# ChuhanZhou/News_Recommendation_Model

Hardware: AMD Instinct MI355X
Metric: train impressions/sec (higher is better)
Workload: dtype f32

## Files before the change

### include/nrm_hotpath.h

```cpp
#ifndef NRM_HOTPATH_H
#define NRM_HOTPATH_H

#ifdef __cplusplus
extern "C" {
#endif

#define NRM_ABI_VERSION 7
#define NRM_OK 0
#define NRM_EINVAL (-1)
#define NRM_ELAUNCH (-2)

typedef void* nrm_stream_t;

int nrm_abi_version(void);
const char* nrm_last_error(void);
int nrm_build_flags(void);
const char* nrm_source_digest(void);
const char* nrm_build_info(void);


#define NRM_MMA_F32 0
#define NRM_MMA_BF16 1
#define NRM_MMA_BF16X3 2
long nrm_pwattn_packed_floats(int D);
int nrm_pwattn_pack_wp(const float* fc1_weight, int ld, int D, int mma, float* packed, nrm_stream_t stream);
int nrm_pwattn_fwd(const float* t, const float* h, const float* u, const float* v, const float* packed_wp,
                   const float* w2, const float* b2, float* z, float* s,
                   int B, int T, int H, int D, int mma, nrm_stream_t stream);

#define NRM_DZ_F32 0
#define NRM_DZ_HL4 1
int nrm_pwattn_bwd_dz(float* z_inout, const float* ds, const float* w2, float* dw2, float* db2, float* du, float* dv,
                      int B, int T, int H, int D, int dz_format, nrm_stream_t stream);
int nrm_pwattn_bwd_nsplit(int B, int T, int H, int D, int mma);
int nrm_pwattn_bwd_contract(const float* dz, const float* t, const float* h, const float* wp, int ldwp,
                            float* dt, float* dh, float* ws,
                            int B, int T, int H, int D, int passes, int mma, int dz_format, nrm_stream_t stream);
int nrm_pwattn_bwd_rw_supported(int D, int mma);
long nrm_pwattn_bwd_rw_packed_floats(int D, int mma);
int nrm_pwattn_bwd_rw_pack(const float* fc1_weight, int ld, int D, int mma, float* packed, nrm_stream_t stream);
int nrm_pwattn_bwd_rw_dtdh(const float* dz_hl4, const float* t, const float* h, const float* packed, float* dt, float* dh,
                           int B, int T, int H, int D, int mma, nrm_stream_t stream);

int nrm_pwattn_bwd_dp_supported(int D, int H);
long nrm_pwattn_bwd_dp_packed_floats(int D, int H);
int nrm_pwattn_bwd_dp_pack(const float* fc1_weight, int ld, int D, int H, float* packed, nrm_stream_t stream);
int nrm_pwattn_bwd_dp_dtdh(const float* dz, const float* t, const float* h, const float* packed, float* dt, float* dh,
                           int B, int T, int H, int D, nrm_stream_t stream);

#define NRM_EPI_BIAS 0
#define NRM_EPI_GELU 1
#define NRM_EPI_DGELU 2
#define NRM_EPI_MUL 3
long nrm_gemm_packed_floats(int nrows, int ncols, int mma);
int nrm_gemm_nt_bf16_supported(int M, int K, int mma);
int nrm_gemm_pack(const float* src, long row_stride, long col_stride, int nrows, int ncols, float* packed,
                  nrm_stream_t stream);
typedef struct {
    const float* src; const float* src2; float sign2;
    long row_stride, col_stride; int nrows, ncols;
    float* packed;
    int mma;
} nrm_pack_desc;
int nrm_gemm_pack_multi(const nrm_pack_desc* descs, int n, nrm_stream_t stream);
int nrm_gemm_nt(const float* x, int ldx, int M, const float* packed, int N, int K, const float* bias,
                float* y, int ldy, float* z, int ldz, const float* m, int ldm, int epilogue, int mma, nrm_stream_t stream);
int nrm_gemm_tn_nsplit(int ncols_i, int ncols_j, int R, int mma);
int nrm_gemm_tn(const float* A, int lda, int ncols_i, const float* B, int ldb, int ncols_j, int R,
                float* ws, int ldws, float* colsum, float* zero_out, long zero_n, int mma, nrm_stream_t stream);

int nrm_slab_reduce(const float* ws, int nsplit, int nj, int ldws, int ni, float* out, long out_istride, long out_jstride,
                    float* out2, long out2_istride, long out2_jstride, float sign2,
                    const float* vec, float* vec_out, nrm_stream_t stream);
typedef struct nrm_slab_desc {
    const float* ws; int nsplit, nj, ldws, ni;
    float* out; long out_istride, out_jstride;
    float* out2; long out2_istride, out2_jstride; float sign2;
    const float* vec; float* vec_out;
} nrm_slab_desc;
int nrm_slab_reduce_multi(const nrm_slab_desc* descs, int n, nrm_stream_t stream);

int nrm_colreduce(int mode, const float* x, const float* dy, const float* mean, const float* rstd,
                  float* s0, float* s1, int R, int N, int ld, nrm_stream_t stream);
int nrm_bn_finalize(int stage, const float* s, float* out, float* running, int R, int N, float momentum, float eps,
                    nrm_stream_t stream);
int nrm_mul_bwd(const float* dy, int lddy, const float* g, int ldg, const float* e, int lde, float* dg, float* de, int ldo,
                int R, int N, nrm_stream_t stream);
int nrm_bn_apply(const float* x, const float* mean, const float* rstd, const float* gamma, const float* beta,
                 float* y, int R, int N, int ld, nrm_stream_t stream);
int nrm_bn_backward(const float* x, const float* dy, const float* mean, const float* rstd, const float* gamma,
                    const float* s0, const float* s1, const float* add, float* dx, int R, int N, int ld, int training,
                    nrm_stream_t stream);
int nrm_concat_cols(const float* const* srcs, const long* lds, const int* widths, int n, float* out, int ldo, long R,
                    nrm_stream_t stream);

int nrm_pool_bmm(const float* W, long wsb, long wsi, long wsj, const float* X, int ldx, float* out,
                 int B, int I, int J, int D, int accumulate, nrm_stream_t stream);
int nrm_pool_rowdot(const float* g, int ldg, const float* h, float* ds, int B, int T, int H, int D, float* zero_out, int zero_n,
                    nrm_stream_t stream);

int nrm_small_linear_relu_fwd(const void* x, int x_is_f64, const float* weight, const float* bias, float* y, long R, int K, int N, int ldy,
                              nrm_stream_t stream);
int nrm_small_linear_relu_bwd(const void* x, int x_is_f64, const float* weight, const float* bias, const float* dy, int lddy, long R,
                              int K, int N, float* dwb, nrm_stream_t stream);

int nrm_loss_fwd_bwd(const float* out, int out_stride, const void* label, int label_is_f64, const long* user_id, const float* delta,
                     long n_delta, float alpha, int B, int T, float* loss_sum, float* dout, int dout_stride, float* ddelta, int* err,
                     nrm_stream_t stream);

int nrm_adam_step(float* p, float* g, float* m, float* v, long n, float lr, float beta1, float beta2, float eps,
                  float weight_decay, int step, int zero_grad, nrm_stream_t stream);
int nrm_gather_flat(const float* const* srcs, const long* offsets, const long* counts, int n, float* flat, long flat_n,
                    nrm_stream_t stream);
int nrm_adam_step_dev(float* p, float* g, float* m, float* v, long n, float lr, float beta1, float beta2, float eps,
                      float weight_decay, float* state, int zero_grad, nrm_stream_t stream);

int nrm_frontend_fwd(const void* x, int x_is_f64, int nrows, int xcols, int P, int n_sub, int behaviour,
                     const float* cat_tab, int n_cat, int e0, const float* sen_w, const float* sen_b, int e1,
                     const float* type_tab, int n_type, int e2,
                     const float* year_tab, const float* month_tab, const float* day_tab, const float* hour_tab,
                     int n_year, int n_month, int n_day, int n_hour, int e3,
                     float* lab, int ldlab, float* ti, int ldti, int* err, nrm_stream_t stream);
int nrm_frontend_bwd(const void* x, int x_is_f64, int nrows, int xcols, int P, int n_sub, int behaviour,
                     const float* dlab, int lddl, const float* sen_w, const float* sen_b,
                     int n_cat, int e0, int e1, int n_type, int e2, int n_year, int n_month, int n_day, int n_hour, int e3,
                     float* d_cat_tab, float* d_sen_w, float* d_sen_b, float* d_type_tab,
                     float* d_year_tab, float* d_month_tab, float* d_day_tab, float* d_hour_tab, nrm_stream_t stream);

long nrm_frontend_cat_ws_ints(int n_cat, long nrows_total, int n_sub);
int nrm_frontend_cat_grad(const void* x0, int nrows0, int xcols0, const float* dlab0, int lddl0,
                          const void* x1, int nrows1, int xcols1, const float* dlab1, int lddl1, int x_is_f64,
                          int P, int n_sub, int n_cat, int e0, float* d_cat_tab, int* ws, nrm_stream_t stream);

int nrm_row_auc(const float* score, const float* label, const int* len, int B, int T, float* auc, int* top1,
                nrm_stream_t stream);

int nrm_ensemble_rank_max_candidates(void);
int nrm_ensemble_rank(const float* const* logits, const long* row_stride, const long* col_stride, int M, const int* empty,
                      const float* label, int B, int T, float* score, int* rank, int* live, float* metrics, nrm_stream_t stream);

int nrm_compact_gather(const void* x_target, int target_cols, int target_is_f64, const void* x_global, int global_cols, int global_is_f64,
                       const int* cand_off, const int* pad_mult, int B, int T, int trim, int N,
                       void* xt_compact, void* xg_compact, int* flag, nrm_stream_t stream);
int nrm_pwattn_fwd_ragged(const float* t, const float* h, const float* u, const float* v, const float* packed_wp,
                          const float* w2, const float* b2, float* s, const int* cand_imp, const int* cand_off,
                          int B, int N, int max_count, int H, int D, int mma, nrm_stream_t stream);
int nrm_pool_bmm_ragged(const float* s, const float* h, float* out, const int* cand_off, int B, int N, int max_count, int H, int D,
                        nrm_stream_t stream);
int nrm_ensemble_rank_ragged(const float* const* logits, const long* col_stride, int M, const int* cand_off, const int* pad_mult, int N,
                             const float* label, int B, int T, float* score, int* rank, int* live, float* metrics, nrm_stream_t stream);

#ifdef __cplusplus
}
#endif
#endif
```

### news_recommendation_model_amd/csrc/capi.hip

```cpp
#include <stdarg.h>
#include <stdint.h>
#include <stdio.h>
#include <stdlib.h>
#include <vector>

#include "../../include/nrm_hotpath.h"
#include "pwattn.hpp"
#include "gemm.hpp"
#include "head.hpp"
#include "pool_loss.hpp"
#include "frontend.hpp"
#include "scoring.hpp"
#include "compact.hpp"

static thread_local char g_err[512] = "";

static int fail(int code, const char* fmt, ...) {
    va_list ap;
    va_start(ap, fmt);
    vsnprintf(g_err, sizeof(g_err), fmt, ap);
    va_end(ap);
    return code;
}
static int check_hip(hipError_t e, const char* what) {
// ... 211 lines not shown
        if (int rc = check_hip(nrm::bwd_e_launch(p, pl, false, mma, (hipStream_t)stream), "bwd_e pass 2")) return rc;
    }
    return NRM_OK;
}


static bool al16(const void* p) { return ((uintptr_t)p & 15) == 0; }

long nrm_gemm_packed_floats(int nrows, int ncols, int mma) {
    if (nrows <= 0 || ncols <= 0) return 0;
    if (mma == NRM_MMA_BF16 || mma == NRM_MMA_BF16X3)
        return (long)((nrows + 15) / 16) * ((ncols + 31) / 32) * (mma == NRM_MMA_BF16X3 ? 2 : 1) * 256 + 1024;
    const nrm::GemmNtPlan pl = nrm::gemm_nt_plan(nrows);
    return (long)((ncols + 15) / 16) * pl.rows * 16 + 1024;
}

int nrm_gemm_nt_bf16_supported(int M, int K, int mma) { return nrm::gemm_nt_rx_bm(M, K, mma) ? 1 : 0; }

int nrm_gemm_pack(const float* src, long row_stride, long col_stride, int nrows, int ncols, float* packed,
                  nrm_stream_t stream) {
    if (!src || !packed || nrows <= 0 || ncols <= 0) return fail(NRM_EINVAL, "nrm_gemm_pack: bad argument");
    const nrm::GemmNtPlan pl = nrm::gemm_nt_plan(nrows);
    return check_hip(nrm::pack_rows_launch(src, row_stride, col_stride, nrows, ncols, pl.rows, (ncols + 15) / 16, packed,
                                           (hipStream_t)stream), "pack_rows");
}

int nrm_gemm_pack_multi(const nrm_pack_desc* descs, int n, nrm_stream_t stream) {
    if (n < 0 || (n > 0 && !descs)) return fail(NRM_EINVAL, "nrm_gemm_pack_multi: bad argument");
    for (int lo = 0; lo < n; lo += nrm::PACK_MAX) {
        const int m = n - lo < nrm::PACK_MAX ? n - lo : nrm::PACK_MAX;
        nrm::PackTable tab = {};
        long mx = 0;
        for (int i = 0; i < m; ++i) {
            const nrm_pack_desc& d = descs[lo + i];
            if (!d.src || !d.packed || d.nrows <= 0 || d.ncols <= 0) return fail(NRM_EINVAL, "nrm_gemm_pack_multi: entry %d is malformed", lo + i);
            const nrm::GemmNtPlan pl = nrm::gemm_nt_plan(d.nrows);
            nrm::PackEntry& e = tab.e[i];
            e.src = d.src; e.src2 = d.src2; e.dst = d.packed; e.rs = d.row_stride; e.cs = d.col_stride;
            e.nrows = d.nrows; e.ncols = d.ncols; e.rows = pl.rows; e.kchunks = (d.ncols + 15) / 16; e.sign2 = d.sign2; e.fmt = 0;
            if (d.mma == NRM_MMA_BF16 || d.mma == NRM_MMA_BF16X3) {
                e.fmt = d.mma == NRM_MMA_BF16X3 ? 2 : 1; e.rows = (d.nrows + 15) / 16 * 16; e.kchunks = (d.ncols + 31) / 32;
            } else if (d.mma != NRM_MMA_F32) return fail(NRM_EINVAL, "nrm_gemm_pack_multi: entry %d: mma=%d", lo + i, d.mma);
            const long total = e.fmt ? (long)(e.rows / 16) * e.kchunks * 512 : (long)e.kchunks * e.rows * 16;
            if (total > mx) mx = total;
        }
        if (int rc = check_hip(nrm::pack_rows_multi_launch(tab, m, mx, (hipStream_t)stream), "pack_rows_multi")) return rc;
    }
    return NRM_OK;
}

int nrm_gemm_nt(const float* x, int ldx, int M, const float* packed, int N, int K, const float* bias,
                float* y, int ldy, float* z, int ldz, const float* m, int ldm, int epilogue, int mma, nrm_stream_t stream) {
    if (!x || !packed || !y) return fail(NRM_EINVAL, "nrm_gemm_nt: null pointer");
    if (M < 0 || N <= 0 || K <= 0) return fail(NRM_EINVAL, "nrm_gemm_nt: M=%d N=%d K=%d", M, N, K);
    if (ldx % 4 || ldy % 4 || ldx < K || ldy < N || !al16(x) || !al16(y))
        return fail(NRM_EINVAL, "nrm_gemm_nt: ldx=%d ldy=%d must be multiples of 4 covering K=%d / N=%d, rows 16-B aligned", ldx, ldy, K, N);
    if (epilogue != NRM_EPI_BIAS && (!z || ldz % 4 || ldz < N || !al16(z)))
        return fail(NRM_EINVAL, "nrm_gemm_nt: epilogue %d needs z with ldz %% 4 == 0, ldz >= N", epilogue);
    if (epilogue < 0 || epilogue > 3) return fail(NRM_EINVAL, "nrm_gemm_nt: epilogue=%d", epilogue);
    if (epilogue == NRM_EPI_MUL && (!m || ldm % 4 || ldm < N || !al16(m)))
        return fail(NRM_EINVAL, "nrm_gemm_nt: NRM_EPI_MUL needs m with ldm %% 4 == 0, ldm >= N");
    if ((long)256 * (ldx > ldy ? ldx : ldy) * 4 >= (1L << 31)) return fail(NRM_EINVAL, "nrm_gemm_nt: leading dimension too large");
    if (int rc = check_mma("nrm_gemm_nt", mma)) return rc;
    if (mma != NRM_MMA_F32) {
        if (!nrm::gemm_nt_rx_bm(M > 0 ? M : 1, K, mma)) return fail(NRM_EINVAL, "nrm_gemm_nt: K=%d is too wide for the bf16 form (nrm_gemm_nt_bf16_supported)", K);
        nrm::GemmRxParams r = {};
        r.x = x; r.ldx = ldx; r.xcols = ldx; r.wq = packed; r.wq_bytes = (unsigned)(nrm_gemm_packed_floats(N, K, mma) * 4);
        r.bias = bias; r.N = N; r.y = y; r.ldy = ldy;
        r.z = epilogue == NRM_EPI_BIAS ? nullptr : z; r.ldz = epilogue == NRM_EPI_BIAS ? 4 : ldz;
        r.m = epilogue == NRM_EPI_MUL ? m : nullptr; r.ldm = epilogue == NRM_EPI_MUL ? ldm : 4;
        r.M = M; r.K = K; r.k32 = (K + 31) / 32; r.nt16 = (N + 15) / 16;
        return check_hip(nrm::gemm_nt_rx_launch(r, epilogue, mma, (hipStream_t)stream), "gemm_nt_rx");
    }
    const nrm::GemmNtPlan pl = nrm::gemm_nt_plan(N);
    nrm::GemmNtParams p;
    p.x = x; p.ldx = ldx; p.xcols = ldx; p.wp = packed; p.wp_bytes = (unsigned)(nrm_gemm_packed_floats(N, K, NRM_MMA_F32) * 4);
    p.rows = pl.rows; p.bias = bias; p.N = N; p.y = y; p.ldy = ldy;
    p.z = epilogue == NRM_EPI_BIAS ? nullptr : z; p.ldz = epilogue == NRM_EPI_BIAS ? 4 : ldz;
    p.m = epilogue == NRM_EPI_MUL ? m : nullptr; p.ldm = epilogue == NRM_EPI_MUL ? ldm : 4;
    p.M = M; p.K = K; p.kchunks = (K + 15) / 16;
    return check_hip(nrm::gemm_nt_launch(p, pl, epilogue, (hipStream_t)stream), "gemm_nt");
}

static const int kTnWavesBf16 = 1024;
static int tn_waves(int mma = 0) {
    if (const char* e = getenv("NRM_TN_WAVES")) return atoi(e);
    return mma ? kTnWavesBf16 : kTnWaves;
}

int nrm_gemm_tn_nsplit(int ncols_i, int ncols_j, int R, int mma) {
    if (ncols_i <= 0 || ncols_j <= 0 || R <= 0) return 0;
    return nrm::gemm_tn_plan(ncols_i, ncols_j, R, tn_waves(mma), mma).nsplit;
}

int nrm_gemm_tn(const float* A, int lda, int ncols_i, const float* B, int ldb, int ncols_j, int R,
                float* ws, int ldws, float* colsum, float* zero_out, long zero_n, int mma, nrm_stream_t stream) {
    if (!A || !B || !ws) return fail(NRM_EINVAL, "nrm_gemm_tn: null pointer");
    if (ncols_i <= 0 || ncols_j <= 0 || R <= 0 || lda < ncols_i || ldb < ncols_j)
        return fail(NRM_EINVAL, "nrm_gemm_tn: ncols_i=%d ncols_j=%d R=%d lda=%d ldb=%d", ncols_i, ncols_j, R, lda, ldb);
    if (ldws % 4 || ldws < ncols_i || !al16(ws)) return fail(NRM_EINVAL, "nrm_gemm_tn: ldws=%d", ldws);
    if (int rc = check_mma("nrm_gemm_tn", mma)) return rc;
    const nrm::GemmTnPlan pl = nrm::gemm_tn_plan(ncols_i, ncols_j, R, tn_waves(mma), mma);
    if ((long)pl.rps * (lda > ldb ? lda : ldb) * 4 >= (1L << 31)) return fail(NRM_EINVAL, "nrm_gemm_tn: split too large");
    if (mma != NRM_MMA_F32 && (lda % 4 || ldb % 4 || ((uintptr_t)A & 15) || ((uintptr_t)B & 15)))
        return fail(NRM_EINVAL, "nrm_gemm_tn: the bf16 forms read 16-byte row segments (lda, ldb multiples of 4, 16-byte aligned rows)");
    nrm::GemmTnParams p = {};
    p.A = A; p.lda = lda; p.acols = lda; p.B = B; p.ldb = ldb; p.bcols = ldb;
    if (zero_out && (zero_n < 0 || !al16(zero_out))) return fail(NRM_EINVAL, "nrm_gemm_tn: zero_out must be 16-byte aligned, zero_n >= 0");
    p.ws = ws; p.ldws = ldws; p.colsum = colsum; p.R = R; p.ncols_j = ncols_j;
    p.zero_out = zero_out; p.zero_n = zero_out ? zero_n : 0;
    if (mma != NRM_MMA_F32) return check_hip(nrm::gemm_tn_bf16_launch(p, pl, mma, (hipStream_t)stream), "gemm_tn_bf16");
    return check_hip(nrm::gemm_tn_launch(p, pl, (hipStream_t)stream), "gemm_tn");
}

int nrm_slab_reduce(const float* ws, int nsplit, int nj, int ldws, int ni, float* out, long out_istride, long out_jstride,
                    float* out2, long out2_istride, long out2_jstride, float sign2,
                    const float* vec, float* vec_out, nrm_stream_t stream) {
    if (!ws || !out) return fail(NRM_EINVAL, "nrm_slab_reduce: null pointer");
    if (nsplit <= 0 || nj <= 0 || ni <= 0 || ldws < ni) return fail(NRM_EINVAL, "nrm_slab_reduce: nsplit=%d nj=%d ni=%d ldws=%d", nsplit, nj, ni, ldws);
    if ((vec == nullptr) != (vec_out == nullptr)) return fail(NRM_EINVAL, "nrm_slab_reduce: vec and vec_out go together");
    nrm::SlabReduceParams p;
    p.ws = ws; p.nsplit = nsplit; p.nj = nj; p.ldws = ldws; p.ni = ni; p.out = out; p.ors = out_istride; p.ocs = out_jstride;
    p.out2 = out2; p.ors2 = out2_istride; p.ocs2 = out2_jstride; p.sign2 = sign2; p.vec = vec; p.vec_out = vec_out;
    return check_hip(nrm::slab_reduce_launch(p, (hipStream_t)stream), "slab_reduce");
}

int nrm_slab_reduce_multi(const nrm_slab_desc* descs, int n, nrm_stream_t stream) {
    if (n < 0 || (n > 0 && !descs)) return fail(NRM_EINVAL, "nrm_slab_reduce_multi: bad argument");
    if (n == 0) return NRM_OK;
    std::vector<nrm::SlabReduceParams> ps((size_t)n);
    for (int i = 0; i < n; ++i) {
        const nrm_slab_desc& d = descs[i];
        if (!d.ws || !d.out) return fail(NRM_EINVAL, "nrm_slab_reduce_multi: entry %d: null pointer", i);
        if (d.nsplit <= 0 || d.nj <= 0 || d.ni <= 0 || d.ldws < d.ni)
            return fail(NRM_EINVAL, "nrm_slab_reduce_multi: entry %d: nsplit=%d nj=%d ni=%d ldws=%d", i, d.nsplit, d.nj, d.ni, d.ldws);
        if ((d.vec == nullptr) != (d.vec_out == nullptr)) return fail(NRM_EINVAL, "nrm_slab_reduce_multi: entry %d: vec and vec_out go together", i);
        nrm::SlabReduceParams& p = ps[(size_t)i];
        p.ws = d.ws; p.nsplit = d.nsplit; p.nj = d.nj; p.ldws = d.ldws; p.ni = d.ni; p.out = d.out; p.ors = d.out_istride; p.ocs = d.out_jstride;
        p.out2 = d.out2; p.ors2 = d.out2_istride; p.ocs2 = d.out2_jstride; p.sign2 = d.sign2; p.vec = d.vec; p.vec_out = d.vec_out;
    }
    return check_hip(nrm::slab_reduce_multi_launch(ps.data(), n, (hipStream_t)stream), "slab_reduce_multi");
}

static int check_bn(const char* fn, int R, int N, int ld) {
    if (R < 0 || N <= 0 || N % 4 || ld % 4 || ld < N) return fail(NRM_EINVAL, "%s: R=%d N=%d ld=%d (N, ld multiples of 4)", fn, R, N, ld);
    return NRM_OK;
}

int nrm_colreduce(int mode, const float* x, const float* dy, const float* mean, const float* rstd,
                  float* s0, float* s1, int R, int N, int ld, nrm_stream_t stream) {
    if (int rc = check_bn("nrm_colreduce", R, N, ld)) return rc;
    if (!x || !s0 || (mode >= 1 && !mean) || (mode == 2 && (!dy || !rstd || !s1)) || mode < 0 || mode > 2)
        return fail(NRM_EINVAL, "nrm_colreduce: bad argument for mode %d", mode);
    return check_hip(nrm::colred_launch(mode, x, dy, mean, rstd, s0, s1, R, N, ld, (hipStream_t)stream), "colreduce");
}

int nrm_bn_finalize(int stage, const float* s, float* out, float* running, int R, int N, float momentum, float eps,
                    nrm_stream_t stream) {
    if (!s || !out) return fail(NRM_EINVAL, "nrm_bn_finalize: null pointer");
    if ((stage != 0 && stage != 1) || R <= 0 || N <= 0) return fail(NRM_EINVAL, "nrm_bn_finalize: stage=%d R=%d N=%d", stage, R, N);
    return check_hip(nrm::bn_finalize_launch(stage, s, out, running, R, N, momentum, eps, (hipStream_t)stream), "bn_finalize");
}

int nrm_mul_bwd(const float* dy, int lddy, const float* g, int ldg, const float* e, int lde, float* dg, float* de, int ldo,
                int R, int N, nrm_stream_t stream) {
    if (!dy || !g || !e || !dg || !de) return fail(NRM_EINVAL, "nrm_mul_bwd: null pointer");
    if (R < 0 || N <= 0 || N % 4 || lddy % 4 || ldg % 4 || lde % 4 || ldo % 4 || lddy < N || ldg < N || lde < N || ldo < N ||
        !al16(dy) || !al16(g) || !al16(e) || !al16(dg) || !al16(de))
        return fail(NRM_EINVAL, "nrm_mul_bwd: R=%d N=%d (N and leading dimensions multiples of 4, 16-byte aligned rows)", R, N);
    return check_hip(nrm::mul_bwd_launch(dy, g, e, dg, de, R, N, lddy, ldg, lde, ldo, (hipStream_t)stream), "mul_bwd");
}

int nrm_bn_apply(const float* x, const float* mean, const float* rstd, const float* gamma, const float* beta,
                 float* y, int R, int N, int ld, nrm_stream_t stream) {
    if (int rc = check_bn("nrm_bn_apply", R, N, ld)) return rc;
    if (!x || !mean || !rstd || !gamma || !beta || !y) return fail(NRM_EINVAL, "nrm_bn_apply: null pointer");
    return check_hip(nrm::bn_apply_launch(x, mean, rstd, gamma, beta, y, R, N, ld, (hipStream_t)stream), "bn_apply");
}

int nrm_bn_backward(const float* x, const float* dy, const float* mean, const float* rstd, const float* gamma,
                    const float* s0, const float* s1, const float* add, float* dx, int R, int N, int ld, int training,
                    nrm_stream_t stream) {
    if (int rc = check_bn("nrm_bn_backward", R, N, ld)) return rc;
    if (!dy || !rstd || !gamma || !dx || (training && (!x || !mean || !s0 || !s1)))
        return fail(NRM_EINVAL, "nrm_bn_backward: null pointer");
    return check_hip(nrm::bn_bwd_launch(x, dy, mean, rstd, gamma, s0, s1, add, dx, R, N, ld, training, (hipStream_t)stream), "bn_backward");
}


int nrm_concat_cols(const float* const* srcs, const long* lds, const int* widths, int n, float* out, int ldo, long R,
                    nrm_stream_t stream) {
    if (!srcs || !lds || !widths || !out) return fail(NRM_EINVAL, "nrm_concat_cols: null pointer");
    if (n < 1 || n > nrm::CONCAT_MAX || R < 0) return fail(NRM_EINVAL, "nrm_concat_cols: n=%d (1..%d) R=%ld", n, nrm::CONCAT_MAX, R);
    nrm::ConcatTable tab = {};
    int total = 0;
    for (int i = 0; i < n; ++i) {
        if (!srcs[i] || widths[i] <= 0 || lds[i] < widths[i]) return fail(NRM_EINVAL, "nrm_concat_cols: part %d (width %d, ld %ld)", i, widths[i], lds[i]);
        tab.src[i] = srcs[i]; tab.ld[i] = lds[i]; tab.start[i] = total;
        total += widths[i];
    }
    tab.n = n;
    if (ldo < total) return fail(NRM_EINVAL, "nrm_concat_cols: ldo=%d < %d columns", ldo, total);
    return check_hip(nrm::concat_cols_launch(tab, out, R, ldo, total, (hipStream_t)stream), "concat_cols");
}

int nrm_pool_bmm(const float* W, long wsb, long wsi, long wsj, const float* X, int ldx, float* out,
                 int B, int I, int J, int D, int accumulate, nrm_stream_t stream) {
    if (!W || !X || !out) return fail(NRM_EINVAL, "nrm_pool_bmm: null pointer");
    if (B < 0 || I <= 0 || J <= 0 || D <= 0 || D % 4 || B > 65535) return fail(NRM_EINVAL, "nrm_pool_bmm: B=%d I=%d J=%d D=%d", B, I, J, D);
    if (ldx < D || ldx % 4 || !al16(X) || (long)J * ldx * 4 >= (1L << 31))
        return fail(NRM_EINVAL, "nrm_pool_bmm: ldx=%d (>= D, a multiple of 4, X 16-byte aligned, J*ldx*4 < 2^31)", ldx);
    return check_hip(nrm::bmm_rows_launch(W, wsb, wsi, wsj, X, (long)J * ldx, ldx, out, (long)I * D, D, B, I, J, D, accumulate,
                                          (hipStream_t)stream), "pool_bmm");
}

int nrm_pool_bmm_ragged(const float* s, const float* h, float* out, const int* cand_off, int B, int N, int max_count, int H, int D,
                        nrm_stream_t stream) {
    if (!s || !h || !out || !cand_off) return fail(NRM_EINVAL, "nrm_pool_bmm_ragged: null pointer");
    if (B < 0 || N < 0 || max_count < 0 || max_count > N || H <= 0 || D <= 0 || D % 4 || B > 65535)
        return fail(NRM_EINVAL, "nrm_pool_bmm_ragged: B=%d N=%d max_count=%d H=%d D=%d", B, N, max_count, H, D);
    if (!al16(h) || !al16(out) || (long)H * D * 4 >= (1L << 31) || (long)N * H >= (1L << 31))
        return fail(NRM_EINVAL, "nrm_pool_bmm_ragged: h and out must be 16-byte aligned, H*D*4 and N*H below 2^31");
    return check_hip(nrm::bmm_rows_ragged_launch(s, H, h, (long)H * D, D, out, D, cand_off, B, N, max_count, H, D, (hipStream_t)stream), "pool_bmm_ragged");
}

int nrm_pool_rowdot(const float* g, int ldg, const float* h, float* ds, int B, int T, int H, int D, float* zero_out, int zero_n,
                    nrm_stream_t stream) {
    if (!g || !h || !ds) return fail(NRM_EINVAL, "nrm_pool_rowdot: null pointer");
    if (B < 0 || T <= 0 || H <= 0 || D <= 0 || D % 4 || D > 1024 || B > 65535) return fail(NRM_EINVAL, "nrm_pool_rowdot: B=%d T=%d H=%d D=%d", B, T, H, D);
    if (ldg < D || ldg % 4 || !al16(g) || (long)T * ldg * 4 >= (1L << 31))
        return fail(NRM_EINVAL, "nrm_pool_rowdot: ldg=%d (>= D, a multiple of 4, g 16-byte aligned, T*ldg*4 < 2^31)", ldg);
    if (zero_n < 0 || (zero_n > 0 && !zero_out)) return fail(NRM_EINVAL, "nrm_pool_rowdot: zero_n=%d without zero_out", zero_n);
    return check_hip(nrm::rowdot_launch(g, (long)T * ldg, ldg, h, (long)H * D, D, ds, B, T, H, D, zero_out, zero_n, (hipStream_t)stream), "pool_rowdot");
}

int nrm_small_linear_relu_fwd(const void* x, int x_is_f64, const float* weight, const float* bias, float* y, long R, int K, int N, int ldy,
                              nrm_stream_t stream) {
    if (!x || !weight || !y) return fail(NRM_EINVAL, "nrm_small_linear_relu_fwd: null pointer");
    if (R < 0 || K < 1 || K > 4 || N < 1 || N > 8 || ldy < N) return fail(NRM_EINVAL, "nrm_small_linear_relu_fwd: R=%ld K=%d N=%d ldy=%d (K <= 4, N <= 8)", R, K, N, ldy);
    return check_hip(nrm::small_linear_relu_fwd_launch(x, x_is_f64, weight, bias, y, R, K, N, ldy, (hipStream_t)stream), "small_linear_relu_fwd");
}

int nrm_small_linear_relu_bwd(const void* x, int x_is_f64, const float* weight, const float* bias, const float* dy, int lddy, long R,
                              int K, int N, float* dwb, nrm_stream_t stream) {
    if (!x || !weight || !dy || !dwb) return fail(NRM_EINVAL, "nrm_small_linear_relu_bwd: null pointer");
    if (R < 0 || K < 1 || K > 4 || N < 1 || N > 8 || lddy < N) return fail(NRM_EINVAL, "nrm_small_linear_relu_bwd: R=%ld K=%d N=%d lddy=%d (K <= 4, N <= 8)", R, K, N, lddy);
    return check_hip(nrm::small_linear_relu_bwd_launch(x, x_is_f64, weight, bias, dy, lddy, R, K, N, dwb, (hipStream_t)stream), "small_linear_relu_bwd");
}

int nrm_loss_fwd_bwd(const float* out, int out_stride, const void* label, int label_is_f64, const long* user_id, const float* delta,
                     long n_delta, float alpha, int B, int T, float* loss_sum, float* dout, int dout_stride, float* ddelta, int* err,
                     nrm_stream_t stream) {
    if (!out || !label || !user_id || !delta || !loss_sum || !dout || !ddelta || !err) return fail(NRM_EINVAL, "nrm_loss_fwd_bwd: null pointer");
    if (B < 0 || T <= 0 || n_delta < 1 || (long)B * T >= (1L << 29))
        return fail(NRM_EINVAL, "nrm_loss_fwd_bwd: B=%d T=%d n_delta=%ld (T >= 1, n_delta >= 1, B*T < 2^29)", B, T, n_delta);
    if (out_stride < 1 || dout_stride < 1 || (dout_stride == 4 && !al16(dout)))
        return fail(NRM_EINVAL, "nrm_loss_fwd_bwd: out_stride=%d dout_stride=%d (>= 1; dout 16-byte aligned for stride 4)", out_stride, dout_stride);
    return check_hip(nrm::loss_launch(out, out_stride, label, label_is_f64, user_id, delta, n_delta, alpha, B, T, loss_sum, dout, dout_stride,
                                      ddelta, err, (hipStream_t)stream), "loss");
}

int nrm_adam_step(float* p, float* g, float* m, float* v, long n, float lr, float beta1, float beta2, float eps,
                  float weight_decay, int step, int zero_grad, nrm_stream_t stream) {
    if (!p || !g || !m || !v) return fail(NRM_EINVAL, "nrm_adam_step: null pointer");
    if (n < 0 || n % 4 || step < 1 || !al16(p) || !al16(g) || !al16(m) || !al16(v))
        return fail(NRM_EINVAL, "nrm_adam_step: n=%ld step=%d (n %% 4 == 0, step >= 1, 16-byte aligned buffers)", n, step);
    return check_hip(nrm::adam_launch(p, g, m, v, n, lr, beta1, beta2, eps, weight_decay, step, zero_grad, (hipStream_t)stream), "adam");
}

// ... 154 lines not shown
```

### news_recommendation_model_amd/csrc/gemm.hip

```cpp
#include <cstdlib>
#include <type_traits>
#include "common.hpp"
#include "gemm.hpp"
#ifndef NRM_PRIO
#define NRM_PRIO 0
#endif
#ifndef NRM_DIAG_GEMM
#define NRM_DIAG_GEMM 0
#endif

namespace nrm {

__global__ void pack_rows_kernel(const float* __restrict__ src, long rs, long cs, int nrows, int ncols,
                                 int rows, int kchunks, float* __restrict__ packed) {
    const long total = (long)kchunks * rows * 16;
    for (long i = (long)blockIdx.x * blockDim.x + threadIdx.x; i < total; i += (long)gridDim.x * blockDim.x) {
        const int j = (int)(i & 15);
        const long rc = i >> 4;
        const int row = (int)(rc % rows);
        const int c = (int)(rc / rows);
        const int slot = (j >> 2) ^ swz4(row);
        const int col = c * 16 + 4 * slot + (j & 3);
        packed[i] = (row < nrows && col < ncols) ? src[row * rs + col * cs] : 0.0f;
    }
}

__global__ __launch_bounds__(256) void pack_rows_multi_kernel(const PackTable tab) {
    const PackEntry e = tab.e[blockIdx.y];
    if (e.fmt) {
        const int nimg = e.fmt;
        const long total = (long)(e.rows / 16) * e.kchunks * 512;
        __bf16* dst = reinterpret_cast<__bf16*>(e.dst);
        for (long i = (long)blockIdx.x * blockDim.x + threadIdx.x; i < total; i += (long)gridDim.x * blockDim.x) {
            const int j = (int)(i & 31), r16 = (int)((i >> 5) & 15);
            const long tc = i >> 9;
            const int c = (int)(tc % e.kchunks), it = (int)(tc / e.kchunks);
            const int n = 16 * it + r16, k = 32 * c + j;
            float v = 0.0f;
            if (n < e.nrows && k < e.ncols) {
                const long o = n * e.rs + k * e.cs;
                v = e.src[o];
                if (e.src2) v = fmaf(e.sign2, e.src2[o], v);
            }
            const __bf16 hi = (__bf16)v;
            const long o = (tc * nimg) * 512 + r16 * 32 + j;
            dst[o] = hi;
            if (nimg > 1) dst[o + 512] = (__bf16)(v - (float)hi);
        }
        return;
    }
    const long total = (long)e.kchunks * e.rows * 16;
    for (long i = (long)blockIdx.x * blockDim.x + threadIdx.x; i < total; i += (long)gridDim.x * blockDim.x) {
        const int j = (int)(i & 15);
        const long rc = i >> 4;
        const int row = (int)(rc % e.rows);
        const int c = (int)(rc / e.rows);
        const int slot = (j >> 2) ^ swz4(row);
        const int col = c * 16 + 4 * slot + (j & 3);
        float v = 0.0f;
        if (row < e.nrows && col < e.ncols) {
            const long o = row * e.rs + col * e.cs;
            v = e.src[o];
            if (e.src2) v = fmaf(e.sign2, e.src2[o], v);
        }
        e.dst[i] = v;
    }
}

hipError_t pack_rows_multi_launch(const PackTable& tab, int n, long max_total, hipStream_t st) {
    if (n <= 0) return hipSuccess;
    long bx = (max_total + 255) / 256;
    if (bx > 128) bx = 128;
    if (bx < 1) bx = 1;
    hipLaunchKernelGGL(pack_rows_multi_kernel, dim3((unsigned)bx, (unsigned)n), dim3(256), 0, st, tab);
    return hipGetLastError();
}

hipError_t pack_rows_launch(const float* src, long rs, long cs, int nrows, int ncols, int rows, int kchunks,
                            float* packed, hipStream_t st) {
    const long total = (long)kchunks * rows * 16;
    const int blocks = (int)((total + 255) / 256 > 4096 ? 4096 : (total + 255) / 256);
    hipLaunchKernelGGL(pack_rows_kernel, dim3(blocks), dim3(256), 0, st, src, rs, cs, nrows, ncols, rows, kchunks, packed);
    return hipGetLastError();
}

template <int NT, int MT, int EPI, int WPE = 2, int KC = 1>
__global__ __launch_bounds__(256, WPE) void gemm_nt_kernel(const GemmNtParams p) {
#if defined(__HIP_DEVICE_COMPILE__)
    constexpr int BM = 4 * MT * 16;
    constexpr int WROWS = NT * 16;
    constexpr int SUB = (WROWS + BM) * 16;
    constexpr int BUF = KC * SUB;
    __shared__ __attribute__((aligned(16))) float smem[2 * BUF];

    const int tid = threadIdx.x;
    const int lane = tid & 63;
    const int wave = __builtin_amdgcn_readfirstlane(tid >> 6);
    const int r16 = lane & 15, q = lane >> 4;
    const int M = p.M;
    const int m0 = blockIdx.x * BM;
    const int nc = blockIdx.y;
    const int n0 = nc * WROWS;

    constexpr unsigned OOB = 0x80000000u;
    const int rows_here = min(BM, M - m0);
    const __amdgpu_buffer_rsrc_t rs_w = __builtin_amdgcn_make_buffer_rsrc(const_cast<float*>(p.wp), 0, p.wp_bytes, 0x00020000);
    const __amdgpu_buffer_rsrc_t rs_x = __builtin_amdgcn_make_buffer_rsrc(
        const_cast<float*>(p.x) + (size_t)m0 * p.ldx, 0, ((rows_here - 1) * p.ldx + p.xcols) * 4, 0x00020000);
    const __amdgpu_buffer_rsrc_t rs_y = __builtin_amdgcn_make_buffer_rsrc(p.y + (size_t)m0 * p.ldy, 0, rows_here * p.ldy * 4, 0x00020000);
    const __amdgpu_buffer_rsrc_t rs_z = __builtin_amdgcn_make_buffer_rsrc(
        p.z ? p.z + (size_t)m0 * p.ldz : nullptr, 0, p.z ? rows_here * p.ldz * 4 : 0, 0x00020000);
    const __amdgpu_buffer_rsrc_t rs_b = __builtin_amdgcn_make_buffer_rsrc(const_cast<float*>(p.bias), 0, p.bias ? (p.N + 3) / 4 * 16 : 0, 0x00020000);
    const __amdgpu_buffer_rsrc_t rs_m = __builtin_amdgcn_make_buffer_rsrc(
        const_cast<float*>(EPI == EPI_MUL ? p.m + (size_t)m0 * p.ldm : nullptr), 0, EPI == EPI_MUL ? rows_here * p.ldm * 4 : 0, 0x00020000);

    unsigned voff_x[MT];
#pragma unroll
    for (int j = 0; j < MT; ++j) {
        const int rl = (wave * MT + j) * 16 + (lane >> 2);
        const unsigned slot = (unsigned)((lane & 3) ^ swz4(lane >> 2));
        voff_x[j] = rl < rows_here ? (unsigned)(rl * p.ldx + 4 * slot) * 4u : OOB;
    }
    const int rslot = 4 * (q ^ swz4(r16));

    f32x4 acc[NT][MT];
#pragma unroll
    for (int it = 0; it < NT; ++it)
#pragma unroll
        for (int jt = 0; jt < MT; ++jt) acc[it][jt] = f32x4{0.f, 0.f, 0.f, 0.f};

    auto dma_chunk = [&](int c, float* buf) {
        const int wbase = (c * p.rows + n0) * 64;
        for (int pc = wave; pc < NT; pc += 4)
            __builtin_amdgcn_raw_ptr_buffer_load_lds(rs_w, (__attribute__((address_space(3))) void*)(buf + pc * 256),
                                                     16, lane * 16, wbase + pc * 1024, 0, 0);
#pragma unroll
        for (int j = 0; j < MT; ++j)
            __builtin_amdgcn_raw_ptr_buffer_load_lds(rs_x, (__attribute__((address_space(3))) void*)(buf + (WROWS + (wave * MT + j) * 16) * 16),
                                                     16, voff_x[j], c * 64, 0, 0);
    };
    auto dma_stage = [&](int s, float* buf) {
#pragma unroll
        for (int k = 0; k < KC; ++k)
            if (KC == 1 || s * KC + k < p.kchunks) dma_chunk(s * KC + k, buf + k * SUB);
    };
    auto compute = [&](const float* buf, auto full, int ntv, int kleft) {
        constexpr bool FULL = decltype(full)::value;
        const float* Xl = buf + WROWS * 16;
        f32x4 pf[MT];
#pragma unroll
        for (int jt = 0; jt < MT; ++jt) pf[jt] = *reinterpret_cast<const f32x4*>(&Xl[((wave * MT + jt) * 16 + r16) * 16 + rslot]);
        if (kleft < 16) {
            asm volatile("");
            const int kl = kleft - 4 * q;
#pragma unroll
            for (int jt = 0; jt < MT; ++jt)
#pragma unroll
                for (int e = 0; e < 4; ++e) pf[jt][e] = e < kl ? pf[jt][e] : 0.f;
        }
        f32x4 af = *reinterpret_cast<const f32x4*>(&buf[r16 * 16 + rslot]);
#pragma unroll
        for (int it = 0; it < NT; ++it) {
            f32x4 afn = af;
            if (it + 1 < NT) afn = *reinterpret_cast<const f32x4*>(&buf[((it + 1) * 16 + r16) * 16 + rslot]);
            if (FULL || it < ntv) {
#pragma unroll
                for (int j = 0; j < 4; ++j)
#pragma unroll
                    for (int jt = 0; jt < MT; ++jt) acc[it][jt] = mfma16(af[j], pf[jt][j], acc[it][jt]);
            }
            __builtin_amdgcn_sched_barrier(0);
            af = afn;
        }
    };

    const int nt_valid = min(NT, (p.N - n0 + 15) >> 4);
    const int nstages = (p.kchunks + KC - 1) / KC;
    dma_stage(0, smem);
    __syncthreads();
    if (NRM_PRIO) __builtin_amdgcn_s_setprio(NRM_PRIO);
    for (int c = 0; c < nstages; ++c) {
        float* cur = smem + (c & 1) * BUF;
        float* nxt = smem + ((c & 1) ^ 1) * BUF;
        if (c + 1 < nstages && !(NRM_DIAG_GEMM & 4)) dma_stage(c + 1, nxt);
#pragma unroll
        for (int k = 0; k < KC; ++k) {
            if (KC > 1 && c * KC + k >= p.kchunks) break;
            const int kleft = p.K - 16 * (c * KC + k);
            if (nt_valid == NT) compute(cur + k * SUB, std::true_type{}, NT, kleft);
            else compute(cur + k * SUB, std::false_type{}, nt_valid, kleft);
        }
        if (!(NRM_DIAG_GEMM & 1)) __syncthreads();
    }
    if (NRM_PRIO) __builtin_amdgcn_s_setprio(0);
    if (NRM_DIAG_GEMM & 2) return;

#pragma unroll
    for (int it = 0; it < NT; ++it) {
        if (it < nt_valid) {
        const int n = n0 + it * 16 + 4 * q;
        const int nb = (n0 + it * 16) * 4;
        f32x4 bb = f32x4{0.f, 0.f, 0.f, 0.f};
        if (EPI != EPI_DGELU && p.bias) {
            bb = __builtin_bit_cast(f32x4, __builtin_amdgcn_raw_buffer_load_b128(rs_b, 16 * q, nb, 0));
#pragma unroll
            for (int e = 0; e < 4; ++e) bb[e] = n + e < p.N ? bb[e] : 0.f;
        }
#pragma unroll
        for (int jt = 0; jt < MT; ++jt) {
            const int rl = (wave * MT + jt) * 16 + r16;
            f32x4 v = acc[it][jt] + bb;
            if (EPI == EPI_BIAS) {
                if (n < p.ldy) store_b128_guarded(__builtin_bit_cast(u32x4, v), rs_y, (unsigned)(rl * p.ldy + 4 * q) * 4u, nb);
            } else if (EPI == EPI_GELU) {
                if (n < p.ldz) store_b128_guarded(__builtin_bit_cast(u32x4, v), rs_z, (unsigned)(rl * p.ldz + 4 * q) * 4u, nb);
                const f32x4 g = gelu4(v);
                if (n < p.ldy) store_b128_guarded(__builtin_bit_cast(u32x4, g), rs_y, (unsigned)(rl * p.ldy + 4 * q) * 4u, nb);
            } else if (EPI == EPI_MUL) {
                if (n < p.ldz) store_b128_guarded(__builtin_bit_cast(u32x4, v), rs_z, (unsigned)(rl * p.ldz + 4 * q) * 4u, nb);
                f32x4 mm = f32x4{0.f, 0.f, 0.f, 0.f};
                if (n < p.ldm) mm = __builtin_bit_cast(f32x4, __builtin_amdgcn_raw_buffer_load_b128(rs_m, (unsigned)(rl * p.ldm + 4 * q) * 4u, nb, 0));
                if (n < p.ldy) store_b128_guarded(__builtin_bit_cast(u32x4, v * mm), rs_y, (unsigned)(rl * p.ldy + 4 * q) * 4u, nb);
            } else {
                f32x4 zz = f32x4{0.f, 0.f, 0.f, 0.f};
                if (n < p.ldz) zz = __builtin_bit_cast(f32x4, __builtin_amdgcn_raw_buffer_load_b128(rs_z, (unsigned)(rl * p.ldz + 4 * q) * 4u, nb, 0));
                const f32x4 g = gelu_grad4_times(zz, acc[it][jt]);
                if (n < p.ldy) store_b128_guarded(__builtin_bit_cast(u32x4, g), rs_y, (unsigned)(rl * p.ldy + 4 * q) * 4u, nb);
            }
        }
        }
        __builtin_amdgcn_sched_barrier(0);
    }
#endif
}

GemmNtPlan gemm_nt_plan(int N) {
    const int n16 = (N + 15) / 16;
    GemmNtPlan pl;
    if (n16 <= 4) { pl.NT = 4; pl.MT = 4; }
    else {
        const int p13 = (n16 + 12) / 13 * 13, p8 = (n16 + 7) / 8 * 8;
        int best = p13 <= p8 ? p13 : p8;
        if (p13 <= p8) { pl.NT = 13; pl.MT = 1; } else { pl.NT = 8; pl.MT = 3; }
        static const bool narrow = [] { const char* e = getenv("NRM_NT_NARROW"); return !(e && e[0] == '0'); }();
        const int p9 = (n16 + 8) / 9 * 9, p5 = (n16 + 4) / 5 * 5;
        if (narrow && p9 * 10 <= best * 9) { pl.NT = 9; pl.MT = 2; best = p9; }
        if (narrow && p5 * 10 <= best * 9) { pl.NT = 5; pl.MT = 4; best = p5; }
    }
    pl.nchunks = (n16 + pl.NT - 1) / pl.NT;
    pl.rows = pl.nchunks * pl.NT * 16;
    return pl;
}

template <int NT, int MT, int WPE = 2, int KC = 1>
static hipError_t launch_nt(const GemmNtParams& p, const GemmNtPlan& pl, int epi, hipStream_t st) {
    constexpr int BM = 4 * MT * 16;
    const dim3 grid((p.M + BM - 1) / BM, pl.nchunks), block(256);
    if (KC > 1) {
        constexpr int lds = 2 * KC * (NT * 16 + BM) * 16 * 4;
        static_assert(lds <= 160 * 1024, "two stages must fit the CU's LDS");
    }
    switch (epi) {
        case EPI_BIAS:  hipLaunchKernelGGL((gemm_nt_kernel<NT, MT, EPI_BIAS, WPE, KC>), grid, block, 0, st, p); break;
        case EPI_GELU:  hipLaunchKernelGGL((gemm_nt_kernel<NT, MT, EPI_GELU, WPE, KC>), grid, block, 0, st, p); break;
        case EPI_DGELU: hipLaunchKernelGGL((gemm_nt_kernel<NT, MT, EPI_DGELU, WPE, KC>), grid, block, 0, st, p); break;
        case EPI_MUL:   hipLaunchKernelGGL((gemm_nt_kernel<NT, MT, EPI_MUL, WPE, KC>), grid, block, 0, st, p); break;
        default: return hipErrorInvalidValue;
    }
    return hipGetLastError();
}

hipError_t gemm_nt_launch(const GemmNtParams& p, const GemmNtPlan& pl, int epi, hipStream_t st) {
    if (p.M <= 0) return hipSuccess;
    static const bool small_m = [] { const char* e = getenv("NRM_NT_SMALLM"); return !(e && e[0] == '0'); }();
    const long wgs = (long)((p.M + 64 * pl.MT - 1) / (64 * pl.MT)) * pl.nchunks;
    const char* kc_e = getenv("NRM_NT_KC");
    int kc = kc_e ? atoi(kc_e) : 1;
    if (kc != 2 && kc != 4) kc = 1;
    if (p.kchunks < 2 * kc) kc = p.kchunks >= 4 ? 2 : 1;
    if (kc > 1 && (pl.MT == 1 || (small_m && wgs < 512))) {
        if (kc == 4) {
            if (pl.NT == 4) return launch_nt<4, 1, 1, 4>(p, pl, epi, st);
            if (pl.NT == 5) return launch_nt<5, 1, 1, 4>(p, pl, epi, st);
            if (pl.NT == 8) return launch_nt<8, 1, 1, 4>(p, pl, epi, st);
            if (pl.NT == 9) return launch_nt<9, 1, 1, 4>(p, pl, epi, st);
            if (pl.NT == 13) return launch_nt<13, 1, 1, 4>(p, pl, epi, st);
        } else {
            if (pl.NT == 4) return launch_nt<4, 1, 2, 2>(p, pl, epi, st);
            if (pl.NT == 5) return launch_nt<5, 1, 2, 2>(p, pl, epi, st);
            if (pl.NT == 8) return launch_nt<8, 1, 2, 2>(p, pl, epi, st);
            if (pl.NT == 9) return launch_nt<9, 1, 2, 2>(p, pl, epi, st);
            if (pl.NT == 13) return launch_nt<13, 1, 2, 2>(p, pl, epi, st);
        }
    }
    if (small_m && pl.MT > 1 && wgs < 512) {
        if (pl.NT == 4) return launch_nt<4, 1, 4>(p, pl, epi, st);
        if (pl.NT == 5) return launch_nt<5, 1, 4>(p, pl, epi, st);
        if (pl.NT == 8) return launch_nt<8, 1, 4>(p, pl, epi, st);
        if (pl.NT == 9) return launch_nt<9, 1, 4>(p, pl, epi, st);
    }
    if (pl.NT == 4) return launch_nt<4, 4>(p, pl, epi, st);
    if (pl.NT == 5) return launch_nt<5, 4>(p, pl, epi, st);
    if (pl.NT == 8) return launch_nt<8, 3>(p, pl, epi, st);
    if (pl.NT == 9) return launch_nt<9, 2, 3>(p, pl, epi, st);
    static const int use13x2 = [] { const char* e = getenv("NRM_NT_13X2"); return e && e[0] == '1' ? 1 : 0; }();
    if (use13x2) return launch_nt<13, 2>(p, pl, epi, st);
    return launch_nt<13, 1, 4>(p, pl, epi, st);
}

template <int W> __device__ __forceinline__ int tn_col(int t, int r) {
    if (W == 2) return 2 * r + t;
    if (W == 5 && t == 4) return 64 + r;
    if (W == 8 && t >= 4) return 64 + 4 * r + (t - 4);
    return 4 * r + t;
}
#if defined(__HIP_DEVICE_COMPILE__)
template <int W> __device__ __forceinline__ void tn_load(float (&v)[W], const __amdgpu_buffer_rsrc_t rs, unsigned vlo, unsigned vhi, int soff) {
    if constexpr (W == 2) {
        const auto x = __builtin_amdgcn_raw_buffer_load_b64(rs, vlo, soff, 0);
        v[0] = __uint_as_float(x[0]); v[1] = __uint_as_float(x[1]);
    } else {
        const u32x4 x = __builtin_amdgcn_raw_buffer_load_b128(rs, vlo, soff, 0);
#pragma unroll
        for (int e = 0; e < 4; ++e) v[e] = __uint_as_float(x[e]);
        if constexpr (W == 5) v[4] = __uint_as_float(__builtin_amdgcn_raw_buffer_load_b32(rs, vhi, soff, 0));
        if constexpr (W == 8) {
            const u32x4 y = __builtin_amdgcn_raw_buffer_load_b128(rs, vhi, soff, 0);
#pragma unroll
            for (int e = 0; e < 4; ++e) v[4 + e] = __uint_as_float(y[e]);
        }
    }
}
#endif
constexpr int tn_waves_per_simd(int KT, int DT) { return KT * DT <= 16 ? 4 : 3; }

template <int KT, int DT>
__global__ __launch_bounds__(256, tn_waves_per_simd(KT, DT)) void gemm_tn_kernel(const GemmTnParams p) {
#if defined(__HIP_DEVICE_COMPILE__)
    const int tid = threadIdx.x;
    const int lane = tid & 63;
    const int wave = __builtin_amdgcn_readfirstlane(tid >> 6);
    const int r16 = lane & 15, q = lane >> 4;
    const int nblk = gridDim.x * gridDim.y, lin = blockIdx.y * gridDim.x + blockIdx.x;
    const int xq = nblk >> 3, xr = nblk & 7, xcd = lin & 7;
    const int logical = (xcd < xr ? xcd * (xq + 1) : xr * (xq + 1) + (xcd - xr) * xq) + (lin >> 3);
    const int bx = logical % gridDim.x, by = logical / gridDim.x;
    const int ti = bx % p.nti, tj = bx / p.nti;
    const int i0 = ti * (KT * 16), j0 = tj * (DT * 16);
    if (p.zero_out) {
        const long n4 = p.zero_n >> 2;
        const f32x4 z4 = f32x4{0.f, 0.f, 0.f, 0.f};
        for (long i = (long)lin * 256 + tid; i < n4; i += (long)nblk * 256) reinterpret_cast<f32x4*>(p.zero_out)[i] = z4;
        for (long i = (n4 << 2) + (long)lin * 256 + tid; i < p.zero_n; i += (long)nblk * 256) p.zero_out[i] = 0.f;
    }
    const int split = by * 4 + wave;
    if (split >= p.nsplit) return;
    const int r_lo = split * p.rps;
    const int r_hi = min(p.R, r_lo + p.rps);
    const int nrows = r_hi - r_lo;
    const int nsteps = nrows > 0 ? (nrows + 3) >> 2 : 0;

    const __amdgpu_buffer_rsrc_t ra = __builtin_amdgcn_make_buffer_rsrc(
        const_cast<float*>(p.A) + (size_t)r_lo * p.lda, 0, nrows > 0 ? ((nrows - 1) * p.lda + p.acols) * 4 : 0, 0x00020000);
    const __amdgpu_buffer_rsrc_t rb = __builtin_amdgcn_make_buffer_rsrc(
        const_cast<float*>(p.B) + (size_t)r_lo * p.ldb, 0, nrows > 0 ? ((nrows - 1) * p.ldb + p.bcols) * 4 : 0, 0x00020000);
    const unsigned va_lo = (unsigned)(q * p.lda + i0 + tn_col<KT>(0, r16)) * 4u, va_hi = (unsigned)(q * p.lda + i0 + tn_col<KT>(KT - 1, r16) - (KT == 8 ? 3 : 0)) * 4u;
    const unsigned vb_lo = (unsigned)(q * p.ldb + j0 + tn_col<DT>(0, r16)) * 4u, vb_hi = (unsigned)(q * p.ldb + j0 + tn_col<DT>(DT - 1, r16) - (DT == 8 ? 3 : 0)) * 4u;
    const int astep = p.lda * 16, bstep = p.ldb * 16;

    f32x4 C[KT][DT];
    float cs[KT];
#pragma unroll
    for (int it = 0; it < KT; ++it) cs[it] = 0.f;

    float a0[KT], b0[DT], a1[KT], b1[DT], a2[KT], b2[DT], a3[KT], b3[DT];
    auto load_step = [&](float (&a)[KT], float (&b)[DT], int s) {
        tn_load<KT>(a, ra, va_lo, va_hi, s * astep);
        tn_load<DT>(b, rb, vb_lo, vb_hi, s * bstep);
    };
    auto mfma_batch = [&](const float (&a)[KT], const float (&b)[DT]) {
#pragma unroll
        for (int it = 0; it < KT; ++it) {
            cs[it] += a[it];
#pragma unroll
            for (int jt = 0; jt < DT; ++jt) C[it][jt] = mfma16(a[it], b[jt], C[it][jt]);
        }
    };
#pragma unroll
    for (int it = 0; it < KT; ++it)
#pragma unroll
        for (int jt = 0; jt < DT; ++jt) C[it][jt] = f32x4{0.f, 0.f, 0.f, 0.f};
    if (0 < nsteps) load_step(a0, b0, 0);
    if (1 < nsteps) load_step(a1, b1, 1);
    if (2 < nsteps) load_step(a2, b2, 2);
    for (int s = 0; s < nsteps; s += 4) {
        if (NRM_DIAG_GEMM & 8) { mfma_batch(a0, b0); mfma_batch(a1, b1); mfma_batch(a2, b2); mfma_batch(a0, b0); continue; }
        if (s + 3 < nsteps) load_step(a3, b3, s + 3);
        mfma_batch(a0, b0);
        if (s + 1 < nsteps) {
            if (s + 4 < nsteps) load_step(a0, b0, s + 4);
            mfma_batch(a1, b1);
        }
        if (s + 2 < nsteps) {
            if (s + 5 < nsteps) load_step(a1, b1, s + 5);
            mfma_batch(a2, b2);
        }
        if (s + 3 < nsteps) {
            if (s + 6 < nsteps) load_step(a2, b2, s + 6);
            mfma_batch(a3, b3);
        }
    }

    float* wsp = p.ws + (size_t)split * p.ncols_j * p.ldws;
#pragma unroll
    for (int jt = 0; jt < DT; ++jt) {
        const int j = j0 + tn_col<DT>(jt, r16);
        if (j >= p.ncols_j) continue;
        float* row = wsp + (size_t)j * p.ldws + i0;
        if constexpr (KT == 2) {
#pragma unroll
            for (int h = 0; h < 2; ++h) {
                const int ii = 8 * q + 4 * h;
                if (i0 + ii < p.ldws) *reinterpret_cast<f32x4*>(row + ii) = f32x4{C[0][jt][2 * h], C[1][jt][2 * h], C[0][jt][2 * h + 1], C[1][jt][2 * h + 1]};
            }
        } else {
#pragma unroll
            for (int g = 0; g < (KT == 8 ? 2 : 1); ++g)
#pragma unroll
                for (int e = 0; e < 4; ++e) {
                    const int ii = 64 * g + 16 * q + 4 * e;
                    if (i0 + ii < p.ldws)
                        *reinterpret_cast<f32x4*>(row + ii) = f32x4{C[4 * g][jt][e], C[4 * g + 1][jt][e], C[4 * g + 2][jt][e], C[4 * g + 3][jt][e]};
                }
            if constexpr (KT == 5)
                if (i0 + 64 + 4 * q < p.ldws) *reinterpret_cast<f32x4*>(row + 64 + 4 * q) = C[KT - 1][jt];
        }
    }
    if (p.colsum && tj == 0) {
#pragma unroll
        for (int it = 0; it < KT; ++it) {
            const float v = sum_rows4(cs[it]);
            const int i = i0 + tn_col<KT>(it, r16);
            if (q == 0 && i < p.ldws) p.colsum[(size_t)split * p.ldws + i] = v;
        }
    }
#endif
}

static const int kTnShapes[][2] = {{4, 4}, {5, 5}, {2, 8}, {8, 2}, {5, 2}, {2, 5}};

GemmTnPlan gemm_tn_plan(int ncols_i, int ncols_j, int R, int target_waves, int mma) {
    GemmTnPlan pl;
    const int ni16 = (ncols_i + 15) / 16, nj16 = (ncols_j + 15) / 16;
    pl.KT = pl.DT = 4;
    long best = -1;
    static const bool wide = [] { const char* e = getenv("NRM_TN_SHAPES"); return !(e && e[0] == '0'); }();
    for (int k = 0; k < (mma ? 1 : (wide ? 6 : 2)); ++k) {
        const int kt = kTnShapes[k][0], dt = kTnShapes[k][1];
        const long w = (long)((ni16 + kt - 1) / kt) * kt * ((nj16 + dt - 1) / dt) * dt;
        if (best < 0 || w < best) { best = w; pl.KT = kt; pl.DT = dt; }
    }
    pl.nti = (ni16 + pl.KT - 1) / pl.KT;
    pl.ntj = (nj16 + pl.DT - 1) / pl.DT;
    const int tiles = pl.nti * pl.ntj;
    if (target_waves <= 0) target_waves = 1024 * (mma ? 1 : tn_waves_per_simd(pl.KT, pl.DT));
    int ns = target_waves / tiles / 4 * 4;
    if (ns < 4) ns = 4;
    const int max_ns = (R + 127) / 128;
    if (ns > max_ns) ns = max_ns < 1 ? 1 : max_ns;
    pl.rps = ((R + ns - 1) / ns + 3) / 4 * 4;
    if (mma) pl.rps = (pl.rps + 31) / 32 * 32;
    if (pl.rps < 4) pl.rps = 4;
    pl.nsplit = (R + pl.rps - 1) / pl.rps;
    if (pl.nsplit < 1) pl.nsplit = 1;
    return pl;
}

hipError_t gemm_tn_launch(GemmTnParams p, const GemmTnPlan& pl, hipStream_t st) {
    p.nti = pl.nti; p.nsplit = pl.nsplit; p.rps = pl.rps;
    const dim3 grid(pl.nti * pl.ntj, (pl.nsplit + 3) / 4), block(256);
    const int shape = pl.KT * 16 + pl.DT;
    switch (shape) {
        case 4 * 16 + 4: hipLaunchKernelGGL((gemm_tn_kernel<4, 4>), grid, block, 0, st, p); break;
        case 5 * 16 + 5: hipLaunchKernelGGL((gemm_tn_kernel<5, 5>), grid, block, 0, st, p); break;
        case 2 * 16 + 8: hipLaunchKernelGGL((gemm_tn_kernel<2, 8>), grid, block, 0, st, p); break;
        case 8 * 16 + 2: hipLaunchKernelGGL((gemm_tn_kernel<8, 2>), grid, block, 0, st, p); break;
        case 5 * 16 + 2: hipLaunchKernelGGL((gemm_tn_kernel<5, 2>), grid, block, 0, st, p); break;
        case 2 * 16 + 5: hipLaunchKernelGGL((gemm_tn_kernel<2, 5>), grid, block, 0, st, p); break;
        default: return hipErrorInvalidValue;
    }
    return hipGetLastError();
}

__device__ __forceinline__ void slab_reduce_block(const SlabReduceParams& p, int spc, int bx, int by, int nby,
                                                  float (*tile)[129]) {
    const int tx = threadIdx.x, ty = threadIdx.y;
    const int nbi = (p.ni + 127) / 128;
    if (by == nby - 1) {
        if (!p.vec) return;
        const int i = bx * 256 + ty * 32 + tx;
        if (i < p.ni) {
            float a = 0.f;
#pragma unroll 8
            for (int s = 0; s < p.nsplit; ++s) a += p.vec[(size_t)s * p.ldws + i];
            p.vec_out[i] = a;
        }
        return;
    }
    if (bx >= nbi * ((p.nj + 31) / 32)) return;
    const int i0 = (bx % nbi) * 128, j0 = (bx / nbi) * 32;
    const int s_lo = by * spc, s_hi = min(p.nsplit, s_lo + spc);
    const size_t slab = (size_t)p.nj * p.ldws;
    f32x4 a[4];
#pragma unroll
    for (int r = 0; r < 4; ++r) a[r] = f32x4{0.f, 0.f, 0.f, 0.f};
    const int i = i0 + 4 * tx;
    if (i < p.ldws) {
#pragma unroll 4
        for (int s = s_lo; s < s_hi; ++s) {
            const float* src = p.ws + s * slab + (size_t)(j0 + ty) * p.ldws + i;
#pragma unroll
            for (int r = 0; r < 4; ++r)
                if (j0 + ty + 8 * r < p.nj) a[r] += *reinterpret_cast<const f32x4*>(src + (size_t)8 * r * p.ldws);
        }
    }
#pragma unroll
    for (int r = 0; r < 4; ++r)
#pragma unroll
        for (int e = 0; e < 4; ++e) tile[ty + 8 * r][4 * tx + e] = a[r][e];
    __syncthreads();
    const int t = ty * 32 + tx, jj = t & 31;
    const int j = j0 + jj;
    if (j < p.nj) {
        for (int il = t >> 5; il < 128; il += 8) {
            const int ii = i0 + il;
            if (ii >= p.ni) break;
            const float v = tile[jj][il];
            atomicAdd(p.out + ii * p.ors + j * p.ocs, v);
            if (p.out2) atomicAdd(p.out2 + ii * p.ors2 + j * p.ocs2, p.sign2 * v);
        }
    }
}

__global__ __launch_bounds__(256) void slab_reduce_kernel(const SlabReduceParams p, int spc) {
    __shared__ float tile[32][129];
    slab_reduce_block(p, spc, blockIdx.x, blockIdx.y, gridDim.y, tile);
}

__global__ __launch_bounds__(256) void slab_reduce_multi_kernel(const SlabTable tab) {
    __shared__ float tile[32][129];
    int b = blockIdx.x, e = 0;
    while (e + 1 < tab.n && b >= tab.first[e + 1]) ++e;
    b -= tab.first[e];
    slab_reduce_block(tab.e[e], tab.spc[e], b % tab.gx[e], b / tab.gx[e], tab.nchunk[e] + 1, tile);
}

static void slab_plan(const SlabReduceParams& p, int& gx, int& nchunk, int& spc) {
    const int nbi = (p.ni + 127) / 128, nbj = (p.nj + 31) / 32;
    const int tiles = nbi * nbj;
    gx = tiles;
    if (p.vec && (p.ni + 255) / 256 > gx) gx = (p.ni + 255) / 256;
    nchunk = 512 / tiles;
    if (nchunk > 128) nchunk = 128;
    if (nchunk > (p.nsplit + 3) / 4) nchunk = (p.nsplit + 3) / 4;
// ... 36 lines not shown
```

### news_recommendation_model_amd/csrc/gemm.hpp

```cpp
#pragma once
#include <hip/hip_runtime.h>

namespace nrm {

enum { EPI_BIAS = 0, EPI_GELU = 1, EPI_DGELU = 2, EPI_MUL = 3 };

struct GemmNtParams {
    const float* x; int ldx, xcols;
    const float* wp; unsigned wp_bytes;
    int rows;
    const float* bias; int N;
    float* y; int ldy;
    float* z; int ldz;
    const float* m; int ldm;
    int M, K, kchunks;
};
struct GemmNtPlan { int NT, MT, nchunks, rows; };
GemmNtPlan gemm_nt_plan(int N);
hipError_t gemm_nt_launch(const GemmNtParams& p, const GemmNtPlan& pl, int epi, hipStream_t st);
hipError_t pack_rows_launch(const float* src, long rs, long cs, int nrows, int ncols, int rows, int kchunks,
                            float* packed, hipStream_t st);

struct GemmRxParams {
    const float* x; int ldx, xcols;
    const float* wq; unsigned wq_bytes;
    const float* bias; int N;
    float* y; int ldy;
    float* z; int ldz;
    const float* m; int ldm;
    int M, K, k32, nt16;
};
int gemm_bf16_diag_flags();
int gemm_nt_rx_bm(int M, int K, int mma);
hipError_t gemm_nt_rx_launch(const GemmRxParams& p, int epi, int mma, hipStream_t st);

constexpr int PACK_MAX = 36;
struct PackEntry { const float* src; const float* src2; float* dst; long rs, cs; int nrows, ncols, rows, kchunks; float sign2; int fmt; };
struct PackTable { PackEntry e[PACK_MAX]; };
hipError_t pack_rows_multi_launch(const PackTable& tab, int n, long max_total, hipStream_t st);

struct GemmTnParams {
    const float* A; int lda, acols;
    const float* B; int ldb, bcols;
    float* ws; int ldws;
    float* colsum;
    float* zero_out; long zero_n;
    int R, ncols_j;
    int nti, nsplit, rps;
};
struct GemmTnPlan { int KT, DT, nti, ntj, nsplit, rps; };
GemmTnPlan gemm_tn_plan(int ncols_i, int ncols_j, int R, int target_waves, int mma = 0);
hipError_t gemm_tn_launch(GemmTnParams p, const GemmTnPlan& pl, hipStream_t st);
hipError_t gemm_tn_bf16_launch(GemmTnParams p, const GemmTnPlan& pl, int mma, hipStream_t st);

struct SlabReduceParams {
    const float* ws; int nsplit, nj, ldws, ni;
    float* out; long ors, ocs;
    float* out2; long ors2, ocs2; float sign2;
    const float* vec; float* vec_out;
};
hipError_t slab_reduce_launch(const SlabReduceParams& p, hipStream_t st);
constexpr int SLAB_MAX = 24;
struct SlabTable { SlabReduceParams e[SLAB_MAX]; int spc[SLAB_MAX]; int nchunk[SLAB_MAX]; int gx[SLAB_MAX]; int first[SLAB_MAX]; int n; };
hipError_t slab_reduce_multi_launch(const SlabReduceParams* ps, int n, hipStream_t st);
int gemm_diag_flags();

}
```

### news_recommendation_model_amd/csrc/head.hip

```cpp
#include "common.hpp"
#include "head.hpp"

namespace nrm {

template <int MODE>
__global__ __launch_bounds__(256) void colred_kernel(const float* __restrict__ x, const float* __restrict__ dy,
                                                     const float* __restrict__ mean, const float* __restrict__ rstd,
                                                     float* __restrict__ s0, float* __restrict__ s1,
                                                     int R, int N, int ld, int rpb) {
    __shared__ f32x4 red[2][8][32];
    const int tx = threadIdx.x, ty = threadIdx.y;
    const int col = blockIdx.x * 128 + 4 * tx;
    const bool cok = col < N;
    f32x4 a0 = f32x4{0.f, 0.f, 0.f, 0.f}, a1 = a0, mu = a0, rs = a0;
    if (cok && MODE >= 1) mu = *reinterpret_cast<const f32x4*>(mean + col);
    if (cok && MODE == 2) rs = *reinterpret_cast<const f32x4*>(rstd + col);
    const int r_lo = blockIdx.y * rpb, r_hi = min(R, r_lo + rpb);
    if (cok) {
        for (int r = r_lo + ty; r < r_hi; r += 8) {
            const f32x4 xv = *reinterpret_cast<const f32x4*>(x + (size_t)r * ld + col);
            if (MODE == 0) a0 += xv;
            else if (MODE == 1) { const f32x4 d = xv - mu; a0 += d * d; }
            else {
                const f32x4 g = *reinterpret_cast<const f32x4*>(dy + (size_t)r * ld + col);
                a0 += g;
                a1 += g * (xv - mu) * rs;
            }
        }
    }
    red[0][ty][tx] = a0;
    if (MODE == 2) red[1][ty][tx] = a1;
    __syncthreads();
    if (ty == 0 && cok) {
        f32x4 t0 = red[0][0][tx], t1 = red[1][0][tx];
#pragma unroll
        for (int y = 1; y < 8; ++y) { t0 += red[0][y][tx]; if (MODE == 2) t1 += red[1][y][tx]; }
#pragma unroll
        for (int e = 0; e < 4; ++e) {
            atomicAdd(s0 + col + e, t0[e]);
            if (MODE == 2) atomicAdd(s1 + col + e, t1[e]);
        }
    }
}

__global__ __launch_bounds__(256) void bn_apply_kernel(const float* __restrict__ x, const float* __restrict__ mean,
                                                       const float* __restrict__ rstd, const float* __restrict__ gamma,
                                                       const float* __restrict__ beta, float* __restrict__ y,
                                                       long R, int N, int ld) {
    const int n4 = N >> 2;
    const long total = R * n4;
    for (long i = (long)blockIdx.x * blockDim.x + threadIdx.x; i < total; i += (long)gridDim.x * blockDim.x) {
        const long r = i / n4;
        const int col = (int)(i - r * n4) * 4;
        const f32x4 xv = *reinterpret_cast<const f32x4*>(x + r * ld + col);
        const f32x4 mu = *reinterpret_cast<const f32x4*>(mean + col), rs = *reinterpret_cast<const f32x4*>(rstd + col);
        const f32x4 g = *reinterpret_cast<const f32x4*>(gamma + col), b = *reinterpret_cast<const f32x4*>(beta + col);
        *reinterpret_cast<f32x4*>(y + r * ld + col) = (xv - mu) * rs * g + b;
    }
}

__global__ __launch_bounds__(256) void bn_bwd_kernel(const float* __restrict__ x, const float* __restrict__ dy,
                                                     const float* __restrict__ mean, const float* __restrict__ rstd,
                                                     const float* __restrict__ gamma, const float* __restrict__ s0,
                                                     const float* __restrict__ s1, const float* __restrict__ add,
                                                     float* __restrict__ dx, long R, int N, int ld, int training) {
    const int n4 = N >> 2;
    const long total = R * n4;
    const float invR = 1.0f / (float)R;
    for (long i = (long)blockIdx.x * blockDim.x + threadIdx.x; i < total; i += (long)gridDim.x * blockDim.x) {
        const long r = i / n4;
        const int col = (int)(i - r * n4) * 4;
        const f32x4 g = *reinterpret_cast<const f32x4*>(dy + r * ld + col);
        const f32x4 rs = *reinterpret_cast<const f32x4*>(rstd + col), ga = *reinterpret_cast<const f32x4*>(gamma + col);
        f32x4 out;
        if (training) {
            const f32x4 xv = *reinterpret_cast<const f32x4*>(x + r * ld + col);
            const f32x4 mu = *reinterpret_cast<const f32x4*>(mean + col);
            const f32x4 a = *reinterpret_cast<const f32x4*>(s0 + col), b = *reinterpret_cast<const f32x4*>(s1 + col);
            const f32x4 xh = (xv - mu) * rs;
            out = ga * rs * (g - a * invR - xh * b * invR);
        } else {
            out = ga * rs * g;
        }
        if (add) out += *reinterpret_cast<const f32x4*>(add + r * ld + col);
        *reinterpret_cast<f32x4*>(dx + r * ld + col) = out;
    }
}

__global__ __launch_bounds__(256) void bn_finalize_kernel(int stage, const float* __restrict__ s, float* __restrict__ out,
                                                          float* __restrict__ running, int R, int N, float momentum, float eps) {
    const int i = blockIdx.x * blockDim.x + threadIdx.x;
    if (i >= N) return;
    const float v = s[i] / (float)R;
    if (stage == 0) {
        out[i] = v;
        if (running) running[i] = (1.0f - momentum) * running[i] + momentum * v;
    } else {
        out[i] = 1.0f / sqrtf(v + eps);
        if (running) running[i] = (1.0f - momentum) * running[i] + momentum * v * ((float)R / (float)(R > 1 ? R - 1 : 1));
    }
}

hipError_t bn_finalize_launch(int stage, const float* s, float* out, float* running, int R, int N, float momentum, float eps,
                              hipStream_t st) {
    if (N <= 0) return hipSuccess;
    hipLaunchKernelGGL(bn_finalize_kernel, dim3((N + 255) / 256), dim3(256), 0, st, stage, s, out, running, R, N, momentum, eps);
    return hipGetLastError();
}

__global__ __launch_bounds__(256) void mul_bwd_kernel(const float* __restrict__ dy, const float* __restrict__ g,
                                                      const float* __restrict__ e, float* __restrict__ dg,
                                                      float* __restrict__ de, long R, int N, int lddy, int ldg, int lde,
                                                      int ldo) {
    const int n4 = N >> 2;
    const long total = R * n4;
    for (long i = (long)blockIdx.x * blockDim.x + threadIdx.x; i < total; i += (long)gridDim.x * blockDim.x) {
        const long r = i / n4;
        const int col = (int)(i - r * n4) * 4;
        const f32x4 d = *reinterpret_cast<const f32x4*>(dy + r * lddy + col);
        const f32x4 gv = *reinterpret_cast<const f32x4*>(g + r * ldg + col);
        const f32x4 ev = *reinterpret_cast<const f32x4*>(e + r * lde + col);
        *reinterpret_cast<f32x4*>(dg + r * ldo + col) = d * ev;
        *reinterpret_cast<f32x4*>(de + r * ldo + col) = d * gv;
    }
}

hipError_t colred_launch(int mode, const float* x, const float* dy, const float* mean, const float* rstd,
                         float* s0, float* s1, int R, int N, int ld, hipStream_t st) {
    if (R <= 0) return hipSuccess;
    const int rpb = 256;
    const dim3 grid((N + 127) / 128, (R + rpb - 1) / rpb), block(32, 8);
    if (mode == 0) hipLaunchKernelGGL(colred_kernel<0>, grid, block, 0, st, x, dy, mean, rstd, s0, s1, R, N, ld, rpb);
    else if (mode == 1) hipLaunchKernelGGL(colred_kernel<1>, grid, block, 0, st, x, dy, mean, rstd, s0, s1, R, N, ld, rpb);
    else if (mode == 2) hipLaunchKernelGGL(colred_kernel<2>, grid, block, 0, st, x, dy, mean, rstd, s0, s1, R, N, ld, rpb);
    else return hipErrorInvalidValue;
    return hipGetLastError();
}

static int ew_blocks(long total) { long b = (total + 255) / 256; return (int)(b > 4096 ? 4096 : (b < 1 ? 1 : b)); }

hipError_t bn_apply_launch(const float* x, const float* mean, const float* rstd, const float* gamma, const float* beta,
                           float* y, long R, int N, int ld, hipStream_t st) {
    if (R <= 0) return hipSuccess;
    hipLaunchKernelGGL(bn_apply_kernel, dim3(ew_blocks(R * (N >> 2))), dim3(256), 0, st, x, mean, rstd, gamma, beta, y, R, N, ld);
    return hipGetLastError();
}

hipError_t mul_bwd_launch(const float* dy, const float* g, const float* e, float* dg, float* de, long R, int N,
                          int lddy, int ldg, int lde, int ldo, hipStream_t st) {
    if (R <= 0) return hipSuccess;
    hipLaunchKernelGGL(mul_bwd_kernel, dim3(ew_blocks(R * (N >> 2))), dim3(256), 0, st, dy, g, e, dg, de, R, N, lddy, ldg, lde, ldo);
    return hipGetLastError();
}

hipError_t bn_bwd_launch(const float* x, const float* dy, const float* mean, const float* rstd, const float* gamma,
                         const float* s0, const float* s1, const float* add, float* dx, long R, int N, int ld, int training,
                         hipStream_t st) {
    if (R <= 0) return hipSuccess;
    hipLaunchKernelGGL(bn_bwd_kernel, dim3(ew_blocks(R * (N >> 2))), dim3(256), 0, st, x, dy, mean, rstd, gamma, s0, s1, add, dx, R, N, ld, training);
    return hipGetLastError();
}

template <int VEC>
__global__ __launch_bounds__(256) void concat_cols_kernel(const ConcatTable tab, float* __restrict__ out, unsigned R, int ldo, int total) {
    const unsigned tv = (unsigned)(total / VEC);
    const unsigned n = R * tv;
    for (unsigned i = blockIdx.x * blockDim.x + threadIdx.x; i < n; i += gridDim.x * blockDim.x) {
        const unsigned r = i / tv;
        const int c = (int)(i - r * tv) * VEC;
        int k = 0;
#pragma unroll
        for (int j = 1; j < CONCAT_MAX; ++j) k += (j < tab.n && c >= tab.start[j]) ? 1 : 0;
        const float* src = tab.src[k] + (size_t)r * tab.ld[k] + (c - tab.start[k]);
        float* dst = out + (size_t)r * ldo + c;
        if (VEC == 4) *reinterpret_cast<f32x4*>(dst) = *reinterpret_cast<const f32x4*>(src);
        else *dst = *src;
    }
}

hipError_t concat_cols_launch(const ConcatTable& tab, float* out, long R, int ldo, int total, hipStream_t st) {
    if (R <= 0 || total <= 0) return hipSuccess;
    if (R * total >= (1L << 31)) return hipErrorInvalidValue;
    bool vec = (ldo & 3) == 0 && (reinterpret_cast<uintptr_t>(out) & 15) == 0;
    for (int i = 0; i < tab.n; ++i)
        vec = vec && (tab.start[i] & 3) == 0 && (tab.ld[i] & 3) == 0 && (reinterpret_cast<uintptr_t>(tab.src[i]) & 15) == 0;
    vec = vec && (total & 3) == 0;
    if (vec) hipLaunchKernelGGL(concat_cols_kernel<4>, dim3(ew_blocks(R * (total / 4))), dim3(256), 0, st, tab, out, (unsigned)R, ldo, total);
    else     hipLaunchKernelGGL(concat_cols_kernel<1>, dim3(ew_blocks(R * total)), dim3(256), 0, st, tab, out, (unsigned)R, ldo, total);
    return hipGetLastError();
}

constexpr int SL_KMAX = 4, SL_NMAX = 8;

template <typename XT>
__global__ __launch_bounds__(256) void small_linear_relu_fwd_kernel(const XT* __restrict__ x, const float* __restrict__ w,
                                                                    const float* __restrict__ b, float* __restrict__ y,
                                                                    long R, int K, int N, int ldy) {
    const long r = (long)blockIdx.x * 256 + threadIdx.x;
    if (r >= R) return;
    float xk[SL_KMAX];
#pragma unroll
    for (int k = 0; k < SL_KMAX; ++k) xk[k] = k < K ? (float)x[r * K + k] : 0.f;
    float* yr = y + r * ldy;
    for (int n = 0; n < ldy; ++n) {
        float v = 0.f;
        if (n < N) {
            v = b ? b[n] : 0.f;
#pragma unroll
            for (int k = 0; k < SL_KMAX; ++k) if (k < K) v = fmaf(w[n * K + k], xk[k], v);
            v = v <= 0.f ? 0.f : v;
        }
        yr[n] = v;
    }
}

template <typename XT>
__global__ __launch_bounds__(256) void small_linear_relu_bwd_kernel(const XT* __restrict__ x, const float* __restrict__ w,
                                                                    const float* __restrict__ b, const float* __restrict__ dy,
                                                                    int lddy, long R, int K, int N, float* __restrict__ dwb) {
    float acc[SL_NMAX][SL_KMAX + 1];
#pragma unroll
    for (int n = 0; n < SL_NMAX; ++n)
#pragma unroll
        for (int k = 0; k <= SL_KMAX; ++k) acc[n][k] = 0.f;
    for (long r = (long)blockIdx.x * 256 + threadIdx.x; r < R; r += (long)gridDim.x * 256) {
        float xk[SL_KMAX];
#pragma unroll
        for (int k = 0; k < SL_KMAX; ++k) xk[k] = k < K ? (float)x[r * K + k] : 0.f;
#pragma unroll
        for (int n = 0; n < SL_NMAX; ++n) {
            if (n < N) {
                float pre = b ? b[n] : 0.f;
#pragma unroll
                for (int k = 0; k < SL_KMAX; ++k) if (k < K) pre = fmaf(w[n * K + k], xk[k], pre);
                const float g = pre > 0.f ? dy[r * lddy + n] : 0.f;
#pragma unroll
                for (int k = 0; k < SL_KMAX; ++k) acc[n][k] = fmaf(g, xk[k], acc[n][k]);
                acc[n][SL_KMAX] += g;
            }
        }
    }
    __shared__ float part[4][SL_NMAX * (SL_KMAX + 1)];
    const int lane = threadIdx.x & 63, wave = threadIdx.x >> 6;
#pragma unroll
    for (int n = 0; n < SL_NMAX; ++n)
#pragma unroll
        for (int k = 0; k <= SL_KMAX; ++k) {
            const float v = wave_sum64(acc[n][k]);
            if (lane == 0) part[wave][n * (SL_KMAX + 1) + k] = v;
        }
    __syncthreads();
    if (threadIdx.x < SL_NMAX * (SL_KMAX + 1)) {
        const int n = threadIdx.x / (SL_KMAX + 1), k = threadIdx.x - n * (SL_KMAX + 1);
        const float v = part[0][threadIdx.x] + part[1][threadIdx.x] + part[2][threadIdx.x] + part[3][threadIdx.x];
        if (n < N && (k < K || k == SL_KMAX) && v != 0.f) atomicAdd(dwb + (k == SL_KMAX ? N * K + n : n * K + k), v);
    }
}

hipError_t small_linear_relu_fwd_launch(const void* x, int x_is_f64, const float* w, const float* b, float* y, long R, int K, int N,
                                        int ldy, hipStream_t st) {
    if (R <= 0) return hipSuccess;
    if (K < 1 || K > SL_KMAX || N < 1 || N > SL_NMAX || ldy < N) return hipErrorInvalidValue;
    const dim3 grid((unsigned)((R + 255) / 256));
    if (x_is_f64) hipLaunchKernelGGL(small_linear_relu_fwd_kernel<double>, grid, dim3(256), 0, st, (const double*)x, w, b, y, R, K, N, ldy);
    else          hipLaunchKernelGGL(small_linear_relu_fwd_kernel<float>, grid, dim3(256), 0, st, (const float*)x, w, b, y, R, K, N, ldy);
    return hipGetLastError();
}

hipError_t small_linear_relu_bwd_launch(const void* x, int x_is_f64, const float* w, const float* b, const float* dy, int lddy,
                                        long R, int K, int N, float* dwb, hipStream_t st) {
    if (R <= 0) return hipSuccess;
    if (K < 1 || K > SL_KMAX || N < 1 || N > SL_NMAX || lddy < N) return hipErrorInvalidValue;
    long blocks = (R + 255) / 256;
    if (blocks > 256) blocks = 256;
// ... 7 lines not shown
```

### news_recommendation_model_amd/csrc/head.hpp

```cpp
#pragma once
#include <hip/hip_runtime.h>

namespace nrm {
hipError_t colred_launch(int mode, const float* x, const float* dy, const float* mean, const float* rstd,
                         float* s0, float* s1, int R, int N, int ld, hipStream_t st);
hipError_t bn_apply_launch(const float* x, const float* mean, const float* rstd, const float* gamma, const float* beta,
                           float* y, long R, int N, int ld, hipStream_t st);
hipError_t bn_bwd_launch(const float* x, const float* dy, const float* mean, const float* rstd, const float* gamma,
                         const float* s0, const float* s1, const float* add, float* dx, long R, int N, int ld, int training,
                         hipStream_t st);
constexpr int CONCAT_MAX = 8;
struct ConcatTable { const float* src[CONCAT_MAX]; long ld[CONCAT_MAX]; int start[CONCAT_MAX]; int n; };
hipError_t concat_cols_launch(const ConcatTable& tab, float* out, long R, int ldo, int total, hipStream_t st);
hipError_t bn_finalize_launch(int stage, const float* s, float* out, float* running, int R, int N, float momentum, float eps,
                              hipStream_t st);
hipError_t mul_bwd_launch(const float* dy, const float* g, const float* e, float* dg, float* de, long R, int N,
                          int lddy, int ldg, int lde, int ldo, hipStream_t st);
hipError_t small_linear_relu_fwd_launch(const void* x, int x_is_f64, const float* w, const float* b, float* y, long R, int K, int N,
                                        int ldy, hipStream_t st);
hipError_t small_linear_relu_bwd_launch(const void* x, int x_is_f64, const float* w, const float* b, const float* dy, int lddy,
                                        long R, int K, int N, float* dwb, hipStream_t st);
}
```

### news_recommendation_model_amd/modules.py

```python
from __future__ import annotations

import os

import torch
import torch.nn as nn
import torch.nn.functional as F

from . import ops
from .config import Dims, TIME_TABLE_ROWS, model_config

_ACTIVATIONS = {
    "relu": nn.ReLU, "gelu": nn.GELU, "tanh": nn.Tanh, "sigmoid": nn.Sigmoid,
    "leaky_relu": nn.LeakyReLU, "elu": nn.ELU,
}


class MLP(nn.Module):

    def __init__(self, input_dim, output_dim, activation_type="gelu"):
        super().__init__()
        self.fc1 = nn.Linear(input_dim, input_dim // 4)
        self.fc2 = nn.Linear(input_dim // 4, output_dim)
        self.activation_type = activation_type
        self.activation = _ACTIVATIONS.get(str(activation_type).lower(), nn.GELU)()
# ... 96 lines not shown
        ops._require_gpu(x_history, x_target)
        if x_history.shape[0] * x_history.shape[1] == 0 or x_target.shape[1] == 0:
            raise RuntimeError("cannot reshape tensor of 0 elements (empty batch / history / candidate list)")
        sen = self.sentiment_embedding[0]
        lab_h, ti_h, lab_t, ti_t = ops.frontend_pair(
            x_history, x_target, self._dims.n_subcat, self._dims.pca_vector, self.category_embedding[0].weight, sen.weight, sen.bias,
            self.type_embedding[0].weight, self.year_embedding[0].weight, self.month_embedding[0].weight,
            self.day_embedding[0].weight, self.hour_embedding[0].weight)
        lab_h = ops.linear(lab_h, self.w1.weight, self.w1.bias)

        side = ops.branch_stream(lab_t) if self._two_streams(lab_t, lab_h) else None
        if side is not None:
            main = torch.cuda.current_stream()
            side.wait_stream(main)
            ti_t.record_stream(side)
            ti_h.record_stream(side)
            with torch.cuda.stream(side):
                pooled_ti = self._attend_and_pool(self.text_img_attention, ti_t, ti_h)
            pooled_lab = self._attend_and_pool(self.label_attention, lab_t, lab_h)
            main.wait_stream(side)
            pooled_ti.record_stream(main)
        else:
            pooled_lab = self._attend_and_pool(self.label_attention, lab_t, lab_h)
            pooled_ti = self._attend_and_pool(self.text_img_attention, ti_t, ti_h)
        return pooled_lab, pooled_ti, lab_t, ti_t

    @staticmethod
    def _attend_and_pool(attention, t, h):
        mlp = getattr(attention, "mlp", None)
        if type(attention) is PointwiseAttentionExpanded and isinstance(mlp, MLP) and isinstance(mlp.activation, nn.GELU) \
                and mlp.activation.approximate == "none" and t.dim() == 3:
            return ops.attend_and_pool(t, h, mlp.fc1.weight, mlp.fc1.bias, mlp.fc2.weight, mlp.fc2.bias, mma=attention.mma)
        s = attention(t, h)
        return ops.weighted_pool(s.squeeze(-1), h)

    two_streams = None

    def _two_streams(self, t, h):
        return self.uses_two_streams(t.shape[0] * t.shape[1] * h.shape[1] * h.shape[2])

    def uses_two_streams(self, z_elems):
        forced = os.environ.get("NRM_BRANCH_STREAMS")
        if forced is not None:
            return forced == "1"
        if self.two_streams is not None:
            return bool(self.two_streams)
        return z_elems <= ops.BRANCH_STREAMS_MAX_ELEMS


class UserInstantInterestModel(nn.Module):

    def __init__(self, output_dim):
        super().__init__()
        self.output_dim = output_dim
        self.out_fc = nn.Sequential(nn.Linear(3, output_dim), nn.ReLU())

    def forward(self, x_global):
        ops._require_gpu(x_global)
        fc = self.out_fc[0]
        return ops.small_linear_relu(x_global, fc.weight, fc.bias)


class UserModel(nn.Module):

    def __init__(self, user_num=0):
        super().__init__()
        self.invariant_interest_model = UserInvariantInterestModel()
        self.instant_interest_model = UserInstantInterestModel(8)
        width = (sum(self.invariant_interest_model.embed_setting) + model_config["pca_vector"]) * 2 \
            + self.instant_interest_model.output_dim
        self.bn = nn.BatchNorm1d(width)
        self.gate = MLP(width, width)
        self.mlp = MLP(width, width)
        self.out_mlp = MLP(width, 1)
        self.delta = nn.Parameter(torch.zeros(user_num + 1))
        self.bce_loss = nn.BCELoss()
        self.softmax = nn.Softmax(dim=1)

    def forward(self, x_history, x_target, x_global):
        inv = self.invariant_interest_model
        if type(inv) is UserInvariantInterestModel and not (inv._forward_hooks or inv._forward_pre_hooks):
            pooled_lab, pooled_ti, lab_t, ti_t = inv.forward_parts(x_history, x_target)
            eu_L = self.instant_interest_model(x_global)
            e = ops.concat_last((pooled_lab, pooled_ti, eu_L, lab_t, ti_t))
        else:
            eu_H, ec = inv(x_history, x_target)
            eu_L = self.instant_interest_model(x_global)
            e = ops.concat_last((eu_H, eu_L, ec))
        B, T, N = e.shape
        rows = e.reshape(B * T, N)
        g = self.gate
        if isinstance(g.activation, nn.GELU) and g.activation.approximate == "none":
            gated = ops.gate_block(rows, self.bn, g.fc1.weight, g.fc1.bias, g.fc2.weight, g.fc2.bias)
        else:
            gated = g.forward_times(ops.batch_norm(rows, self.bn), rows)
        return self.out_mlp(self.mlp(gated)).reshape(B, T)

    def forward_compact(self, x_history, xt_compact, xg_compact, plan):
        if self.training:
            raise RuntimeError("UserModel.forward_compact is inference only: call .eval() first (training-mode BatchNorm takes its "
                               "statistics over the rows of the launch, and the compact path drops the padded ones)")
        inv = self.invariant_interest_model
        ops._require_gpu(x_history, xt_compact, xg_compact)
        B, H, N = x_history.shape[0], x_history.shape[1], xt_compact.shape[0]
        if plan.B != B or plan.N != N or xg_compact.shape[0] != N:
            raise RuntimeError(f"forward_compact: plan for {plan.B} impressions / {plan.N} rows, got {B} / {N} target and {xg_compact.shape[0]} global rows")
        if B * H == 0 or N == 0:
            raise RuntimeError("cannot reshape tensor of 0 elements (empty batch / history / candidate list)")
        for att in (inv.label_attention, inv.text_img_attention):
            mlp = getattr(att, "mlp", None)
            if not (type(att) is PointwiseAttentionExpanded and isinstance(mlp, MLP) and isinstance(mlp.activation, nn.GELU)
                    and mlp.activation.approximate == "none"):
                raise RuntimeError("forward_compact: the ragged attention implements the reference default (PointwiseAttentionExpanded, exact GELU) only")
        tabs = plan.upload(x_history.device)
        with torch.no_grad():
            sen = inv.sentiment_embedding[0]
            tables = (inv.category_embedding[0].weight, sen.weight, sen.bias, inv.type_embedding[0].weight, inv.year_embedding[0].weight,
                      inv.month_embedding[0].weight, inv.day_embedding[0].weight, inv.hour_embedding[0].weight)
            d = inv._dims
            lab_h, ti_h = ops.frontend(x_history, True, d.n_subcat, d.pca_vector, *tables)
            lab_t, ti_t = ops.frontend(xt_compact.unsqueeze(0), False, d.n_subcat, d.pca_vector, *tables)
            lab_h = ops.linear(lab_h, inv.w1.weight, inv.w1.bias)
            pooled = []
            for att, t, h in ((inv.label_attention, lab_t[0], lab_h), (inv.text_img_attention, ti_t[0], ti_h)):
                m = att.mlp
                pooled.append(ops.attend_pool_ragged(t, h, m.fc1.weight, m.fc1.bias, m.fc2.weight, m.fc2.bias, tabs["cand_imp"],
                                                     tabs["cand_off"], plan.max_count, mma=att.mma))
            eu_L = self.instant_interest_model(xg_compact)
            rows = ops.concat_last((pooled[0], pooled[1], eu_L, lab_t[0], ti_t[0]))
            g = self.gate
            if isinstance(g.activation, nn.GELU) and g.activation.approximate == "none":
                gated = ops.gate_block(rows, self.bn, g.fc1.weight, g.fc1.bias, g.fc2.weight, g.fc2.bias)
            else:
                gated = g.forward_times(ops.batch_norm(rows, self.bn), rows)
            return self.out_mlp(self.mlp(gated)).reshape(N)

    def loss(self, id, out, label, alpha=0.95):
        return ops.softmax_bce_loss(out, self.delta, label, id, alpha)
```

### news_recommendation_model_amd/native.py

```python
from __future__ import annotations

import ctypes
import os
import threading

_HERE = os.path.dirname(os.path.abspath(__file__))
LIB_PATH = os.environ.get("NRM_HOTPATH_LIB") or os.path.join(_HERE, "libnrm_hotpath.so")
ABI_VERSION = 7

_c_fp = ctypes.c_void_p
_c_i, _c_l = ctypes.c_int, ctypes.c_long

SIGNATURES = {
    "nrm_abi_version": (_c_i, []),
    "nrm_last_error": (ctypes.c_char_p, []),
    "nrm_build_flags": (_c_i, []),
    "nrm_source_digest": (ctypes.c_char_p, []),
    "nrm_build_info": (ctypes.c_char_p, []),
    "nrm_pwattn_packed_floats": (_c_l, [_c_i]),
    "nrm_pwattn_pack_wp": (_c_i, [_c_fp, _c_i, _c_i, _c_i, _c_fp, _c_fp]),
    "nrm_pwattn_fwd": (_c_i, [_c_fp] * 9 + [_c_i] * 5 + [_c_fp]),
    "nrm_pwattn_bwd_dz": (_c_i, [_c_fp] * 7 + [_c_i] * 5 + [_c_fp]),
    "nrm_pwattn_bwd_rw_supported": (_c_i, [_c_i, _c_i]),
    "nrm_pwattn_bwd_rw_packed_floats": (_c_l, [_c_i, _c_i]),
    "nrm_pwattn_bwd_rw_pack": (_c_i, [_c_fp, _c_i, _c_i, _c_i, _c_fp, _c_fp]),
    "nrm_pwattn_bwd_rw_dtdh": (_c_i, [_c_fp] * 6 + [_c_i] * 5 + [_c_fp]),
    "nrm_pwattn_bwd_dp_supported": (_c_i, [_c_i, _c_i]),
    "nrm_pwattn_bwd_dp_packed_floats": (_c_l, [_c_i, _c_i]),
    "nrm_pwattn_bwd_dp_pack": (_c_i, [_c_fp, _c_i, _c_i, _c_i, _c_fp, _c_fp]),
    "nrm_pwattn_bwd_dp_dtdh": (_c_i, [_c_fp] * 6 + [_c_i] * 4 + [_c_fp]),
    "nrm_pwattn_bwd_nsplit": (_c_i, [_c_i] * 5),
    "nrm_pwattn_bwd_contract": (_c_i, [_c_fp] * 4 + [_c_i] + [_c_fp] * 3 + [_c_i] * 7 + [_c_fp]),
    "nrm_gemm_packed_floats": (_c_l, [_c_i, _c_i, _c_i]),
    "nrm_gemm_nt_bf16_supported": (_c_i, [_c_i, _c_i, _c_i]),
    "nrm_gemm_pack": (_c_i, [_c_fp, _c_l, _c_l, _c_i, _c_i, _c_fp, _c_fp]),
    "nrm_gemm_nt": (_c_i, [_c_fp, _c_i, _c_i, _c_fp, _c_i, _c_i, _c_fp, _c_fp, _c_i, _c_fp, _c_i, _c_fp, _c_i, _c_i, _c_i, _c_fp]),
    "nrm_slab_reduce": (_c_i, [_c_fp, _c_i, _c_i, _c_i, _c_i, _c_fp, _c_l, _c_l, _c_fp, _c_l, _c_l, ctypes.c_float,
                               _c_fp, _c_fp, _c_fp]),
    "nrm_bn_finalize": (_c_i, [_c_i, _c_fp, _c_fp, _c_fp, _c_i, _c_i, ctypes.c_float, ctypes.c_float, _c_fp]),
    "nrm_mul_bwd": (_c_i, [_c_fp, _c_i, _c_fp, _c_i, _c_fp, _c_i, _c_fp, _c_fp, _c_i, _c_i, _c_i, _c_fp]),
    "nrm_gemm_tn_nsplit": (_c_i, [_c_i, _c_i, _c_i, _c_i]),
    "nrm_gemm_tn": (_c_i, [_c_fp, _c_i, _c_i, _c_fp, _c_i, _c_i, _c_i, _c_fp, _c_i, _c_fp, _c_fp, _c_l, _c_i, _c_fp]),
    "nrm_gemm_pack_multi": (_c_i, [_c_fp, _c_i, _c_fp]),
    "nrm_slab_reduce_multi": (_c_i, [_c_fp, _c_i, _c_fp]),
    "nrm_colreduce": (_c_i, [_c_i] + [_c_fp] * 6 + [_c_i] * 3 + [_c_fp]),
    "nrm_bn_apply": (_c_i, [_c_fp] * 6 + [_c_i] * 3 + [_c_fp]),
    "nrm_bn_backward": (_c_i, [_c_fp] * 9 + [_c_i] * 4 + [_c_fp]),
    "nrm_concat_cols": (_c_i, [_c_fp, _c_fp, _c_fp, _c_i, _c_fp, _c_i, _c_l, _c_fp]),
    "nrm_pool_bmm": (_c_i, [_c_fp, _c_l, _c_l, _c_l, _c_fp, _c_i, _c_fp] + [_c_i] * 5 + [_c_fp]),
    "nrm_pool_rowdot": (_c_i, [_c_fp, _c_i, _c_fp, _c_fp] + [_c_i] * 4 + [_c_fp, _c_i, _c_fp]),
    "nrm_small_linear_relu_fwd": (_c_i, [_c_fp, _c_i, _c_fp, _c_fp, _c_fp, _c_l, _c_i, _c_i, _c_i, _c_fp]),
    "nrm_small_linear_relu_bwd": (_c_i, [_c_fp, _c_i, _c_fp, _c_fp, _c_fp, _c_i, _c_l, _c_i, _c_i, _c_fp, _c_fp]),
    "nrm_loss_fwd_bwd": (_c_i, [_c_fp, _c_i, _c_fp, _c_i, _c_fp, _c_fp, _c_l, ctypes.c_float, _c_i, _c_i, _c_fp, _c_fp, _c_i, _c_fp, _c_fp, _c_fp]),
    "nrm_adam_step": (_c_i, [_c_fp] * 4 + [_c_l] + [ctypes.c_float] * 5 + [_c_i, _c_i, _c_fp]),
    "nrm_adam_step_dev": (_c_i, [_c_fp] * 4 + [_c_l] + [ctypes.c_float] * 5 + [_c_fp, _c_i, _c_fp]),
    "nrm_gather_flat": (_c_i, [_c_fp, _c_fp, _c_fp, _c_i, _c_fp, _c_l, _c_fp]),
    "nrm_row_auc": (_c_i, [_c_fp] * 3 + [_c_i, _c_i] + [_c_fp] * 3),
    "nrm_ensemble_rank_max_candidates": (_c_i, []),
    "nrm_ensemble_rank": (_c_i, [_c_fp] * 3 + [_c_i, _c_fp, _c_fp, _c_i, _c_i] + [_c_fp] * 5),
    "nrm_compact_gather": (_c_i, [_c_fp, _c_i, _c_i, _c_fp, _c_i, _c_i, _c_fp, _c_fp, _c_i, _c_i, _c_i, _c_i, _c_fp, _c_fp, _c_fp, _c_fp]),
    "nrm_pwattn_fwd_ragged": (_c_i, [_c_fp] * 10 + [_c_i] * 6 + [_c_fp]),
    "nrm_pool_bmm_ragged": (_c_i, [_c_fp] * 4 + [_c_i] * 5 + [_c_fp]),
    "nrm_ensemble_rank_ragged": (_c_i, [_c_fp, _c_fp, _c_i, _c_fp, _c_fp, _c_i, _c_fp, _c_i, _c_i] + [_c_fp] * 5),
    "nrm_frontend_fwd": (_c_i, [_c_fp, _c_i, _c_i, _c_i, _c_i, _c_i, _c_i,  _c_fp, _c_i, _c_i,  _c_fp, _c_fp, _c_i,
                                 _c_fp, _c_i, _c_i,  _c_fp, _c_fp, _c_fp, _c_fp,  _c_i, _c_i, _c_i, _c_i, _c_i,
                                 _c_fp, _c_i, _c_fp, _c_i, _c_fp, _c_fp]),
    "nrm_frontend_cat_ws_ints": (_c_l, [_c_i, _c_l, _c_i]),
    "nrm_frontend_cat_grad": (_c_i, [_c_fp, _c_i, _c_i, _c_fp, _c_i] * 2 + [_c_i] * 5 + [_c_fp, _c_fp, _c_fp]),
    "nrm_frontend_bwd": (_c_i, [_c_fp, _c_i, _c_i, _c_i, _c_i, _c_i, _c_i,  _c_fp, _c_i, _c_fp, _c_fp]
                         + [_c_i] * 10 + [_c_fp] * 8 + [_c_fp]),
}



class PackDesc(ctypes.Structure):
    _fields_ = [("src", ctypes.c_void_p), ("src2", ctypes.c_void_p), ("sign2", ctypes.c_float),
                ("row_stride", ctypes.c_long), ("col_stride", ctypes.c_long), ("nrows", ctypes.c_int), ("ncols", ctypes.c_int),
                ("packed", ctypes.c_void_p), ("mma", ctypes.c_int)]


class SlabDesc(ctypes.Structure):
    _fields_ = [("ws", ctypes.c_void_p), ("nsplit", ctypes.c_int), ("nj", ctypes.c_int), ("ldws", ctypes.c_int), ("ni", ctypes.c_int),
                ("out", ctypes.c_void_p), ("out_istride", ctypes.c_long), ("out_jstride", ctypes.c_long),
                ("out2", ctypes.c_void_p), ("out2_istride", ctypes.c_long), ("out2_jstride", ctypes.c_long), ("sign2", ctypes.c_float),
                ("vec", ctypes.c_void_p), ("vec_out", ctypes.c_void_p)]


_lib = None
_lock = threading.Lock()


def load():
    global _lib
    if _lib is not None:
        return _lib
    with _lock:
        if _lib is not None:
            return _lib
        if not os.path.exists(LIB_PATH):
            raise RuntimeError(
                f"{LIB_PATH} is missing: build it with `python -m news_recommendation_model_amd.build` "
                "(hipcc --offload-arch=gfx950). There is no CPU or PyTorch fallback for the hot path.")
        lib = ctypes.CDLL(LIB_PATH)
        for name, (res, args) in SIGNATURES.items():
            fn = getattr(lib, name)
            fn.restype, fn.argtypes = res, args
        if lib.nrm_abi_version() != ABI_VERSION:
            raise RuntimeError(f"ABI mismatch: library {lib.nrm_abi_version()} != binding {ABI_VERSION}; rebuild")
        flags = lib.nrm_build_flags()
        if flags and os.environ.get("NRM_ALLOW_DIAG_LIB") != "1":
            raise RuntimeError(
                f"{LIB_PATH} is a timing-diagnostic build (nrm_build_flags() = {flags:#x}: kernels with parts of their work "
                "removed, results are wrong by construction); set NRM_ALLOW_DIAG_LIB=1 to load it for timing experiments")
        if os.environ.get("NRM_ALLOW_STALE_LIB") != "1" and not os.environ.get("NRM_HOTPATH_LIB"):
            from . import build as _build
            if os.path.isdir(_build.CSRC):
                have, want = lib.nrm_source_digest().decode(), _build.sources_digest()
                if have != want:
                    raise RuntimeError(f"{LIB_PATH} was built from other kernel sources (library {have[:16]}..., sources {want[:16]}...): "
# ... 37 lines not shown
```

### news_recommendation_model_amd/ops.py

```python
from __future__ import annotations

import torch

from . import native

EPI_BIAS, EPI_GELU, EPI_DGELU, EPI_MUL = 0, 1, 2, 3
MMA_F32, MMA_BF16, MMA_BF16X3 = 0, 1, 2
DZ_F32, DZ_HL4 = 0, 1
_MMA_NAMES = {"f32": MMA_F32, "fp32": MMA_F32, "float32": MMA_F32, "bf16": MMA_BF16, "bfloat16": MMA_BF16, "bf16x3": MMA_BF16X3}
_default_mma = MMA_F32


def resolve_mma(mma):
    if mma is None:
        return _default_mma
    if isinstance(mma, str):
        if mma.lower() not in _MMA_NAMES:
            raise ValueError(f"attention arithmetic {mma!r}: expected 'f32', 'bf16' or 'bf16x3'")
        return _MMA_NAMES[mma.lower()]
    if int(mma) not in (MMA_F32, MMA_BF16, MMA_BF16X3):
        raise ValueError(f"attention arithmetic {mma!r}: expected NRM_MMA_F32 (0), NRM_MMA_BF16 (1) or NRM_MMA_BF16X3 (2)")
    return int(mma)


# ... 92 lines not shown
        return ent.buf
    if ent is None:
        ent = _PackEntry()
        ent.buf = torch.empty(lib.nrm_gemm_packed_floats(nrows, ncols, mma), dtype=torch.float32, device=src.device)
        ent.owner, ent.owner_ptr = weakref.ref(owner), owner.data_ptr()
        ent.spec = (src.data_ptr() - owner.data_ptr(), rs, cs, nrows, ncols,
                    (src2.data_ptr() - owner.data_ptr()) if src2 is not None else None, sign2, mma)
        _packs.entries[key] = ent
        weakref.finalize(owner, _packs.entries.pop, key, None)
    d = _pack_desc(src, rs, cs, nrows, ncols, src2, sign2, ent.buf, mma)
    native.call("nrm_gemm_pack_multi", _ctypes_ref(d), 1, native.stream_ptr())
    ent.version, ent.epoch = owner._version, _packs.epoch
    return ent.buf


def _ctypes_ref(desc_or_array):
    import ctypes
    return ctypes.cast(ctypes.pointer(desc_or_array), ctypes.c_void_p)


def repack_persistent(owners=None):
    _packs.epoch += 1
    mine = None if owners is None else {id(o) for o in owners}
    live = []
    for key, ent in list(_packs.entries.items()):
        owner = ent.owner()
        if owner is None or owner.data_ptr() != ent.owner_ptr:
            _packs.entries.pop(key, None)
            continue
        if mine is not None and id(owner) not in mine:
            continue
        live.append((ent, owner))
    if not live:
        return 0
    arr = (native.PackDesc * len(live))(*[_pack_desc_of(ent, owner) for ent, owner in live])
    native.call("nrm_gemm_pack_multi", _ctypes_ref(arr), len(live), native.stream_ptr())
    for ent, owner in live:
        ent.version, ent.epoch = owner._version, _packs.epoch
    return len(live)


def invalidate_packed_weights():
    _packs.entries.clear()
    _packs.epoch += 1
    _packs.generation += 1


def packed_weights_generation():
    return _packs.generation


_flop_meter = None


def flop_meter_start():
    global _flop_meter
    _flop_meter = {"dense": 0.0, "contraction": 0.0, "dense_launches": 0, "contraction_launches": 0}


def flop_meter_stop():
    global _flop_meter
    m, _flop_meter = _flop_meter, None
    return m


def _count_flops(kind, flops):
    if _flop_meter is not None:
        _flop_meter[kind] += float(flops)
        _flop_meter[kind + "_launches"] += 1


import os as _os
_FORCE_F32_GEMM = _os.environ.get("NRM_GEMM_F32") == "1"


def _dense_mma(M, K, mma):
    mma = _default_dense_mma if mma is None else mma
    if _FORCE_F32_GEMM or (mma != MMA_F32 and not native.load().nrm_gemm_nt_bf16_supported(int(M), int(K), int(mma))):
        return MMA_F32
    return mma


def _gemm_nt(x, w_src, row_stride, col_stride, n_out, k_red, bias, epilogue, z=None, m=None, src2=None, sign2=0.0, owner=None,
             mma=None):
    st = native.stream_ptr()
    M = x.shape[0]
    mma = _dense_mma(M, k_red, mma)
    packed = _pack(w_src, row_stride, col_stride, n_out, k_red, src2, sign2, owner, mma)
    ldy = _pad4(n_out)
    y = torch.empty(M, ldy, dtype=torch.float32, device=x.device)
    if epilogue in (EPI_GELU, EPI_MUL):
        z = torch.empty(M, ldy, dtype=torch.float32, device=x.device)
    _count_flops("dense", 2.0 * M * n_out * k_red)
    native.call("nrm_gemm_nt", native.ptr(x), x.stride(0), M, native.ptr(packed), n_out, k_red,
                native.ptr(bias) if bias is not None else None, native.ptr(y), ldy,
                native.ptr(z) if z is not None else None, z.stride(0) if z is not None else 0,
                native.ptr(m) if m is not None else None, m.stride(0) if m is not None else 0, epilogue, mma, st)
    return y[:, :n_out], (z[:, :n_out] if epilogue in (EPI_GELU, EPI_MUL) else None)


def _gemm_tn_slabs(a, b, want_colsum, zero_out=None, mma=None):
    lib = native.load()
    R, ni = a.shape
    nj = b.shape[1]
    mma = _default_dense_mma if mma is None else mma
    if _FORCE_F32_GEMM or (mma != MMA_F32 and (a.stride(0) % 4 or b.stride(0) % 4 or a.data_ptr() % 16 or b.data_ptr() % 16)):
        mma = MMA_F32
    nsplit = lib.nrm_gemm_tn_nsplit(ni, nj, R, mma)
    ldws = _pad4(ni)
    ws = torch.empty(nsplit, nj, ldws, dtype=torch.float32, device=a.device)
    cs = torch.empty(nsplit, ldws, dtype=torch.float32, device=a.device) if want_colsum else None
    _count_flops("dense", 2.0 * R * ni * nj)
    native.call("nrm_gemm_tn", native.ptr(a), a.stride(0), ni, native.ptr(b), b.stride(0), nj, R,
                native.ptr(ws), ldws, native.ptr(cs) if cs is not None else None,
                native.ptr(zero_out) if zero_out is not None else None, zero_out.numel() if zero_out is not None else 0,
                mma, native.stream_ptr())
    return ws, cs, nsplit, ldws


_deferred = {"on": False, "pending": []}


class deferred_slab_reductions:
    def __enter__(self):
        self.prev, _deferred["on"] = _deferred["on"], True
        return self

    def __exit__(self, *exc):
        _deferred["on"] = self.prev
        if exc[0] is not None:
            _deferred["pending"].clear()
        return False


def verify_deferred_targets(params):
    pend = _deferred["pending"]
    if not pend:
        return
    by_ptr = {p.data_ptr(): p for p in params}
    for rec in pend:
        p = by_ptr.get(rec["target"])
        if p is None or not p.requires_grad:
            continue
        if p.grad is None or p.grad.untyped_storage().data_ptr() != rec["keep"][0].data_ptr():
            _deferred["pending"] = []
            _join_wgrad_stream()
            raise RuntimeError(
                "deferred slab reductions: a weight gradient was copied or accumulated before its reduction ran (a weight "
                "used more than once in the graph, a gradient that existed before backward(), a gradient hook, or "
                "create_graph): its values would be wrong. Run this backward outside ops.deferred_slab_reductions() -- "
                "trainer.train_step(..., defer_reductions=False).")


def flush_slab_reductions():
    pend, _deferred["pending"] = _deferred["pending"], []
    _join_wgrad_stream()
    if not pend:
        return
    descs = (native.SlabDesc * len(pend))()
    for d, rec in zip(descs, pend):
        d.ws, d.nsplit, d.nj, d.ldws, d.ni = rec["ws"].data_ptr(), rec["nsplit"], rec["nj"], rec["ldws"], rec["ni"]
        d.out, d.out_istride, d.out_jstride = rec["out"], rec["out_is"], rec["out_js"]
        d.out2, d.out2_istride, d.out2_jstride, d.sign2 = rec["out2"], rec["out2_is"], rec["out2_js"], rec["sign2"]
        if rec["vec"] is not None:
            d.vec, d.vec_out = rec["vec"].data_ptr(), rec["vec_out"]
    native.call("nrm_slab_reduce_multi", descs, len(pend), native.stream_ptr())


def _slab_reduce(ws, nsplit, nj, ldws, ni, out, out_is, out_js, out2=None, out2_is=0, out2_js=0, sign2=0.0,
                 vec=None, vec_out=None, target=None):
    if _deferred["on"]:
        _deferred["pending"].append(dict(
            ws=ws, nsplit=nsplit, nj=nj, ldws=ldws, ni=ni, out=out.data_ptr(), out_is=out_is, out_js=out_js,
            out2=out2.data_ptr() if out2 is not None else None, out2_is=out2_is, out2_js=out2_js, sign2=float(sign2),
            vec=vec, vec_out=vec_out.data_ptr() if vec_out is not None else None,
            target=target.data_ptr() if target is not None else None,
            keep=(out.untyped_storage(), out2.untyped_storage() if out2 is not None else None,
                  vec_out.untyped_storage() if vec_out is not None else None)))
        return
    native.call("nrm_slab_reduce", native.ptr(ws), nsplit, nj, ldws, ni, native.ptr(out), out_is, out_js,
                native.ptr(out2) if out2 is not None else None, out2_is, out2_js, float(sign2),
                native.ptr(vec) if vec is not None else None, native.ptr(vec_out) if vec_out is not None else None,
                native.stream_ptr())


WGRAD_STREAM_MIN_ROWS = 0
_wgrad = {"streams": {}, "used": set()}


class _wgrad_stream:

    def __init__(self, *inputs):
        import os
        forced = os.environ.get("NRM_WGRAD_STREAM")
        self.inputs = inputs
        self.on = _deferred["on"] and forced == "1" and inputs[0].shape[0] >= WGRAD_STREAM_MIN_ROWS

    def __enter__(self):
        if not self.on:
            return False
        dev = self.inputs[0].device
        key = dev.index if dev.index is not None else torch.cuda.current_device()
        side = _wgrad["streams"].get(key)
        if side is None:
            side = _wgrad["streams"][key] = torch.cuda.Stream(device=dev)
        self.main = torch.cuda.current_stream(dev)
        side.wait_stream(self.main)
        for t in self.inputs:
            t.record_stream(side)
        _wgrad["used"].add(key)
        self.ctx = torch.cuda.stream(side)
        self.ctx.__enter__()
        return True

    def __exit__(self, *exc):
        if self.on:
            self.ctx.__exit__(*exc)
        return False


def _join_wgrad_stream():
    for key in list(_wgrad["used"]):
        torch.cuda.current_stream().wait_stream(_wgrad["streams"][key])
    _wgrad["used"].clear()


def _gemm_tn(a, b, want_colsum, target=None, mma=None):
    ni, nj = a.shape[1], b.shape[1]
    ctx = _wgrad_stream(a, b)
    with ctx as side:
        c = torch.empty(ni, nj, dtype=torch.float32, device=a.device)
        ws, cs, nsplit, ldws = _gemm_tn_slabs(a, b, want_colsum, zero_out=c, mma=mma)
        colsum = torch.empty(ni, dtype=torch.float32, device=a.device) if want_colsum else None
        _slab_reduce(ws, nsplit, nj, ldws, ni, c, nj, 1, vec=cs, vec_out=colsum, target=target)
        if side:
            for t in (c, ws, cs, colsum):
                if t is not None:
                    t.record_stream(ctx.main)
    return c, colsum


_LIB = torch.library.Library("nrm", "DEF")


def _op(name, schema, impl, fake):
    _LIB.define(name + schema)
    _LIB.impl(name, impl, "CUDA")
    torch.library.register_fake("nrm::" + name, fake, lib=_LIB)
    return getattr(torch.ops.nrm, name)


def _pwattn_fwd_impl(t, h, w1, b1, w2, b2, save_z, mma):
    _require_gpu(t, h, w1, b1, w2, b2)
    if save_z:
        _chain["end"] = None
    B, T, D = t.shape
    H = h.shape[1]
    if h.shape[0] != B or h.shape[2] != D or tuple(w1.shape) != (D, 4 * D) or D % 4:
        raise RuntimeError(f"pointwise attention: target {tuple(t.shape)}, history {tuple(h.shape)}, "
                           f"fc1 {tuple(w1.shape)} do not agree (feature width must be a multiple of 4)")
    w1_arg = w1
    t, h, w1, b1 = _f32c(t), _f32c(h), _f32c(w1), _f32c(b1)
    w2v, b2 = _f32c(w2).reshape(-1), _f32c(b2).reshape(-1)
    own = w1 if w1 is w1_arg else None
    w_h, w_t, w_d = w1[:, :D], w1[:, D:2 * D], w1[:, 2 * D:3 * D]
    u, _ = _gemm_nt(h.reshape(B * H, D), w_h, 4 * D, 1, D, D, b1, EPI_BIAS, src2=w_d, sign2=-1.0, owner=own, mma=mma)
    v, _ = _gemm_nt(t.reshape(B * T, D), w_t, 4 * D, 1, D, D, None, EPI_BIAS, src2=w_d, sign2=1.0, owner=own, mma=mma)
    st = native.stream_ptr()
    packed = torch.empty(native.load().nrm_pwattn_packed_floats(D), dtype=torch.float32, device=t.device)
    native.call("nrm_pwattn_pack_wp", native.ptr(w1), 4 * D, D, mma, native.ptr(packed), st)
    s = torch.empty(B, T, H, dtype=torch.float32, device=t.device)
    z = torch.empty((B, T, H, D) if save_z else (0,), dtype=torch.float32, device=t.device)
    _count_flops("contraction", 2.0 * B * T * H * D * D)
    native.call("nrm_pwattn_fwd", native.ptr(t), native.ptr(h), native.ptr(u), native.ptr(v),
                native.ptr(packed), native.ptr(w2v), native.ptr(b2),
                native.ptr(z) if save_z else None, native.ptr(s), B, T, H, D, mma, st)
    return s, z


def _pwattn_fwd_fake(t, h, w1, b1, w2, b2, save_z, mma):
    B, T, D = t.shape
    H = h.shape[1]
    return (t.new_empty((B, T, H), dtype=torch.float32),
            t.new_empty((B, T, H, D) if save_z else (0,), dtype=torch.float32))


pwattn_fwd = _op("pwattn_fwd", "(Tensor t, Tensor h, Tensor fc1_weight, Tensor fc1_bias, Tensor fc2_weight, Tensor fc2_bias, "
                 "bool save_z, int mma) -> (Tensor, Tensor)", _pwattn_fwd_impl, _pwattn_fwd_fake)


def _pwattn_bwd_impl(ds, t, h, w1, w2, z, mma, need_dt, need_dh):
    return _attn_bwd_core(ds, t, h, w1, w2, z, mma, need_dt, need_dh)


_chain = {"token": 0, "end": None}


def begin_step():
    _chain["token"] += 1
    _chain["end"] = None


def _note_chain_end():
    ev = torch.cuda.Event()
    ev.record()
    _chain["end"] = (_chain["token"], ev, torch.cuda.current_stream(), torch.cuda.is_current_stream_capturing())


DW_LAST_MIN_ELEMS, DW_LAST_MAX_ELEMS = 200_000_000, 1_000_000_000


def _wait_for_foreign_chain(z_elems):
    import os
    end = _chain["end"]
    forced = os.environ.get("NRM_DW_LAST")
# ... 397 lines not shown
    return (_padded_empty(x, M, K1) if need_dx else f(0), f(N1, K1), f(N1) if has_b1 else f(0), f(N2, K2),
            f(N2) if has_b2 else f(0), (_padded_empty(x, M, N2) if N2 % 4 == 0 else f(M, N2)) if mul is not None else f(0))


mlp_gelu_bwd = _op("mlp_gelu_bwd", "(Tensor dy, Tensor x, Tensor fc1_weight, Tensor fc2_weight, Tensor hidden, Tensor z, "
                   "Tensor pre, Tensor? mul, bool has_b1, bool has_b2, bool need_dx) -> "
                   "(Tensor, Tensor, Tensor, Tensor, Tensor, Tensor)", _mlp_gelu_bwd_impl, _mlp_gelu_bwd_fake)


def _mlp_setup(ctx, inputs, output):
    x, w1, b1, w2, b2, mul = inputs
    y, hidden, z, pre = output
    ctx.set_materialize_grads(False)
    ctx.has_bias = (b1 is not None, b2 is not None)
    ctx.has_mul = mul is not None
    ctx.save_for_backward(x, w1, w2, hidden, z, pre, *((mul,) if mul is not None else ()))


def _mlp_backward(ctx, dy, _dh, _dz, _dpre):
    if dy is None:
        return None, None, None, None, None, None
    saved = ctx.saved_tensors
    x, w1, w2, hidden, z, pre = saved[:6]
    mul = saved[6] if ctx.has_mul else None
    need = ctx.needs_input_grad
    dx, dw1, db1, dw2, db2, dmul = mlp_gelu_bwd(dy, x, w1, w2, hidden, z, pre, mul, ctx.has_bias[0], ctx.has_bias[1], need[0])
    return ((dx if need[0] else None), dw1, (db1 if ctx.has_bias[0] else None), dw2, (db2 if ctx.has_bias[1] else None),
            (dmul if ctx.has_mul else None))


torch.library.register_autograd("nrm::mlp_gelu_fwd", _mlp_backward, setup_context=_mlp_setup, lib=_LIB)


def mlp_gelu(x, fc1_weight, fc1_bias, fc2_weight, fc2_bias, mul=None):
    lead = x.shape[:-1]
    if x.numel() == 0 and x.shape[-1] == fc1_weight.shape[1]:
        out = _degenerate((*lead, fc2_weight.shape[0]), x, fc1_weight, fc1_bias, fc2_weight, fc2_bias)
        return out if mul is None else out * mul
    _require_gpu(x, fc1_weight, fc2_weight)
    m2 = mul.reshape(-1, mul.shape[-1]) if mul is not None else None
    y = mlp_gelu_fwd(x.reshape(-1, x.shape[-1]), fc1_weight, fc1_bias, fc2_weight, fc2_bias, m2)[0]
    return y.reshape(*lead, fc2_weight.shape[0])


def _bn_stats_impl(x, running_mean, running_var, momentum, eps):
    _require_gpu(x, running_mean, running_var)
    x = _rows(x)
    R, N = x.shape
    ld = x.stride(0)
    st = native.stream_ptr()
    dev = x.device
    s = torch.zeros(2, N, dtype=torch.float32, device=dev)
    mean = torch.empty(N, dtype=torch.float32, device=dev)
    rstd = torch.empty(N, dtype=torch.float32, device=dev)
    native.call("nrm_colreduce", 0, native.ptr(x), None, None, None, native.ptr(s[0]), None, R, N, ld, st)
    native.call("nrm_bn_finalize", 0, native.ptr(s[0]), native.ptr(mean), native.ptr(running_mean), R, N, float(momentum), float(eps), st)
    native.call("nrm_colreduce", 1, native.ptr(x), None, native.ptr(mean), None, native.ptr(s[1]), None, R, N, ld, st)
    native.call("nrm_bn_finalize", 1, native.ptr(s[1]), native.ptr(rstd), native.ptr(running_var), R, N, float(momentum), float(eps), st)
    return mean, rstd


batch_norm_stats = _op("batch_norm_stats", "(Tensor x, Tensor(a!) running_mean, Tensor(b!) running_var, float momentum, float eps) -> "
                       "(Tensor, Tensor)", _bn_stats_impl,
                       lambda x, rm, rv, momentum, eps: (x.new_empty((x.shape[1],), dtype=torch.float32),
                                                         x.new_empty((x.shape[1],), dtype=torch.float32)))


def _bn_apply_impl(x, mean, rstd, weight, bias, batch_stats):
    _require_gpu(x, mean, rstd, weight, bias)
    x = _rows(x)
    R, N = x.shape
    ld = x.stride(0)
    w, b = _f32c(weight), _f32c(bias)
    y = torch.empty(R, ld, dtype=torch.float32, device=x.device)
    native.call("nrm_bn_apply", native.ptr(x), native.ptr(mean), native.ptr(rstd), native.ptr(w), native.ptr(b),
                native.ptr(y), R, N, ld, native.stream_ptr())
    return y[:, :N]


batch_norm_apply = _op("batch_norm_apply", "(Tensor x, Tensor mean, Tensor rstd, Tensor weight, Tensor bias, bool batch_stats) -> Tensor",
                       _bn_apply_impl, lambda x, mean, rstd, weight, bias, batch_stats: _padded_empty(x, x.shape[0], x.shape[1]))


def _bn_bwd_impl(dy, x, mean, rstd, weight, training, add=None):
    _require_gpu(dy, x)
    x = _rows(x)
    R, N = x.shape
    ld = x.stride(0)
    st = native.stream_ptr()
    dev = x.device
    if not (dy.dim() == 2 and dy.stride(1) == 1 and dy.stride(0) == ld and dy.dtype == torch.float32
            and dy.data_ptr() % 16 == 0):
        buf = torch.zeros(R, ld, dtype=torch.float32, device=dev)
        buf[:, :N] = dy
        dy = buf[:, :N]
    w = _f32c(weight)
    s0 = torch.zeros(N, dtype=torch.float32, device=dev)
    s1 = torch.zeros(N, dtype=torch.float32, device=dev)
    native.call("nrm_colreduce", 2, native.ptr(x), native.ptr(dy), native.ptr(mean), native.ptr(rstd),
                native.ptr(s0), native.ptr(s1), R, N, ld, st)
    dx = torch.empty(R, ld, dtype=torch.float32, device=dev)
    if add is not None and not (add.dim() == 2 and add.stride(1) == 1 and add.stride(0) == ld and add.dtype == torch.float32
                                and add.data_ptr() % 16 == 0):
        buf = torch.zeros(R, ld, dtype=torch.float32, device=dev)
        buf[:, :N] = add
        add = buf[:, :N]
    native.call("nrm_bn_backward", native.ptr(x), native.ptr(dy), native.ptr(mean), native.ptr(rstd), native.ptr(w),
                native.ptr(s0), native.ptr(s1), native.ptr(add) if add is not None else None, native.ptr(dx), R, N, ld,
                1 if training else 0, st)
    return dx[:, :N], s1, s0


def _bn_bwd_fake(dy, x, mean, rstd, weight, training):
    R, N = x.shape
    return _padded_empty(x, R, N), x.new_empty((N,), dtype=torch.float32), x.new_empty((N,), dtype=torch.float32)


batch_norm_bwd = _op("batch_norm_bwd", "(Tensor dy, Tensor x, Tensor mean, Tensor rstd, Tensor weight, bool training) -> "
                     "(Tensor, Tensor, Tensor)", _bn_bwd_impl, _bn_bwd_fake)


def _bn_setup(ctx, inputs, output):
    x, mean, rstd, weight, bias, batch_stats = inputs
    ctx.batch_stats = batch_stats
    ctx.save_for_backward(x, mean, rstd, weight)


def _bn_backward(ctx, dy):
    x, mean, rstd, weight = ctx.saved_tensors
    dx, dgamma, dbeta = batch_norm_bwd(dy, x, mean, rstd, weight, ctx.batch_stats)
    return dx, None, None, dgamma, dbeta, None


torch.library.register_autograd("nrm::batch_norm_apply", _bn_backward, setup_context=_bn_setup, lib=_LIB)


def batch_norm(x, bn):
    if (x.dim() != 2 or x.shape[1] % 4 or not bn.affine or not bn.track_running_stats or bn.momentum is None):
        return bn(x)
    training = bn.training
    if x.shape[0] <= (1 if training else 0):
        return bn(x)
    _require_gpu(x, bn.weight)
    if training:
        bn.num_batches_tracked.add_(1)
        mean, rstd = batch_norm_stats(x.detach(), bn.running_mean, bn.running_var, float(bn.momentum), float(bn.eps))
    else:
        mean, rstd = bn.running_mean.to(torch.float32), torch.rsqrt(bn.running_var.to(torch.float32) + bn.eps)
    return batch_norm_apply(x, mean, rstd, bn.weight, bn.bias, training)


def _gate_block_fwd_impl(x, mean, rstd, bn_w, bn_b, w1, b1, w2, b2, batch_stats):
    c = _bn_apply_impl(x, mean, rstd, bn_w, bn_b, batch_stats)
    y, hidden, z, pre = _mlp_gelu_fwd_impl(c, w1, b1, w2, b2, x)
    return y, c, hidden, z, pre


def _gate_block_fwd_fake(x, mean, rstd, bn_w, bn_b, w1, b1, w2, b2, batch_stats):
    M, N, N1 = x.shape[0], x.shape[1], w1.shape[0]
    return (_padded_empty(x, M, N), _padded_empty(x, M, N), _padded_empty(x, M, N1), _padded_empty(x, M, N1), _padded_empty(x, M, N))


gate_block_fwd = _op("gate_block_fwd", "(Tensor x, Tensor mean, Tensor rstd, Tensor bn_weight, Tensor bn_bias, Tensor fc1_weight, "
                     "Tensor? fc1_bias, Tensor fc2_weight, Tensor? fc2_bias, bool batch_stats) -> (Tensor, Tensor, Tensor, Tensor, Tensor)",
                     _gate_block_fwd_impl, _gate_block_fwd_fake)


def _gate_block_bwd_impl(dy, x, mean, rstd, bn_w, c, w1, w2, hidden, z, pre, has_b1, has_b2, batch_stats):
    dc, dw1, db1, dw2, db2, dmul = _mlp_gelu_bwd_impl(dy, c, w1, w2, hidden, z, pre, x, has_b1, has_b2, True)
    dx, dgamma, dbeta = _bn_bwd_impl(dc, x, mean, rstd, bn_w, batch_stats, add=dmul)
    return dx, dgamma, dbeta, dw1, db1, dw2, db2


def _gate_block_bwd_fake(dy, x, mean, rstd, bn_w, c, w1, w2, hidden, z, pre, has_b1, has_b2, batch_stats):
    M, N = x.shape
    (N1, K1), (N2, K2) = w1.shape, w2.shape
    f = lambda *shape: x.new_empty(shape, dtype=torch.float32)
    return _padded_empty(x, M, N), f(N), f(N), f(N1, K1), f(N1) if has_b1 else f(0), f(N2, K2), f(N2) if has_b2 else f(0)


gate_block_bwd = _op("gate_block_bwd", "(Tensor dy, Tensor x, Tensor mean, Tensor rstd, Tensor bn_weight, Tensor c, Tensor fc1_weight, "
                     "Tensor fc2_weight, Tensor hidden, Tensor z, Tensor pre, bool has_b1, bool has_b2, bool batch_stats) -> "
                     "(Tensor, Tensor, Tensor, Tensor, Tensor, Tensor, Tensor)", _gate_block_bwd_impl, _gate_block_bwd_fake)


def _gate_block_setup(ctx, inputs, output):
    x, mean, rstd, bn_w, bn_b, w1, b1, w2, b2, batch_stats = inputs
    y, c, hidden, z, pre = output
    ctx.set_materialize_grads(False)
    ctx.flags = (b1 is not None, b2 is not None, batch_stats)
    ctx.save_for_backward(x, mean, rstd, bn_w, c, w1, w2, hidden, z, pre)


def _gate_block_backward(ctx, dy, _dc, _dh, _dz, _dp):
    if dy is None:
        return (None,) * 10
    has_b1, has_b2, batch_stats = ctx.flags
    dx, dgamma, dbeta, dw1, db1, dw2, db2 = gate_block_bwd(dy, *ctx.saved_tensors, has_b1, has_b2, batch_stats)
    return dx, None, None, dgamma, dbeta, dw1, (db1 if has_b1 else None), dw2, (db2 if has_b2 else None), None


torch.library.register_autograd("nrm::gate_block_fwd", _gate_block_backward, setup_context=_gate_block_setup, lib=_LIB)


def gate_block(x, bn, fc1_weight, fc1_bias, fc2_weight, fc2_bias):
    if (x.dim() != 2 or x.shape[1] % 4 or not bn.affine or not bn.track_running_stats or bn.momentum is None
            or x.shape[0] <= (1 if bn.training else 0) or fc2_weight.shape[0] != x.shape[1]):
        return mlp_gelu(batch_norm(x, bn), fc1_weight, fc1_bias, fc2_weight, fc2_bias, mul=x)
    _require_gpu(x, bn.weight, fc1_weight)
    if bn.training:
        bn.num_batches_tracked.add_(1)
        mean, rstd = batch_norm_stats(x.detach(), bn.running_mean, bn.running_var, float(bn.momentum), float(bn.eps))
    else:
        mean, rstd = bn.running_mean.to(torch.float32), torch.rsqrt(bn.running_var.to(torch.float32) + bn.eps)
    return gate_block_fwd(x, mean, rstd, bn.weight, bn.bias, fc1_weight, fc1_bias, fc2_weight, fc2_bias, bn.training)[0]


def _concat_cols_impl(parts):
    import ctypes
    _require_gpu(*parts)
    parts = [p if (p.dtype == torch.float32 and p.dim() == 2 and p.stride(1) == 1) else _f32c(p) for p in parts]
    R = parts[0].shape[0]
    total = sum(p.shape[1] for p in parts)
    if len(parts) > 8 or any(p.shape[0] != R for p in parts):
        return torch.cat(parts, dim=1)
    out = torch.empty(R, _pad4(total), dtype=torch.float32, device=parts[0].device)
    k = len(parts)
    srcs = (ctypes.c_void_p * k)(*[p.data_ptr() for p in parts])
    lds = (ctypes.c_long * k)(*[p.stride(0) if p.shape[0] > 1 else p.shape[1] for p in parts])
    widths = (ctypes.c_int * k)(*[p.shape[1] for p in parts])
    native.call("nrm_concat_cols", srcs, lds, widths, k, native.ptr(out), out.stride(0), R, native.stream_ptr())
    return out[:, :total]


concat_cols_op = _op("concat_cols", "(Tensor[] parts) -> Tensor", _concat_cols_impl,
                     lambda parts: _padded_empty(parts[0], parts[0].shape[0], sum(p.shape[1] for p in parts)))


def _concat_setup(ctx, inputs, output):
    ctx.widths = [p.shape[1] for p in inputs[0]]


def _concat_backward(ctx, g):
    out, c = [], 0
    for w in ctx.widths:
        out.append(g[:, c:c + w])
        c += w
    return (out,)


torch.library.register_autograd("nrm::concat_cols", _concat_backward, setup_context=_concat_setup, lib=_LIB)


def concat_last(parts):
    lead = parts[0].shape[:-1]
    rows = 1
    for d in lead:
        rows *= d
    if rows == 0 or len(parts) > 8:
        return torch.cat(parts, dim=-1)
    _require_gpu(*parts)
    y = concat_cols_op([p.reshape(rows, p.shape[-1]) for p in parts])
    return y.reshape(*lead, y.shape[-1]) if y.is_contiguous() else y.unflatten(0, tuple(lead))


def _pool_fwd_impl(s, h):
    _require_gpu(s, h)
    s, h = _f32c(s), _f32c(h)
    B, T, H = s.shape
    D = h.shape[2]
    out = torch.empty(B, T, D, dtype=torch.float32, device=h.device)
    native.call("nrm_pool_bmm", native.ptr(s), T * H, H, 1, native.ptr(h), D, native.ptr(out), B, T, H, D, 0,
                native.stream_ptr())
    return out


weighted_pool_fwd = _op("weighted_pool_fwd", "(Tensor scores, Tensor history) -> Tensor", _pool_fwd_impl,
                        lambda s, h: s.new_empty((s.shape[0], s.shape[1], h.shape[2]), dtype=torch.float32))


def _pooled_grad_rows(g, B, T, D):
    g = g if g.dtype == torch.float32 else g.to(torch.float32)
    ld = g.stride(1) if T > 1 else (g.stride(0) if B > 1 else D)
    if (g.dim() == 3 and g.stride(2) == 1 and ld >= D and ld % 4 == 0 and (B == 1 or g.stride(0) == T * ld)
            and (T == 1 or g.stride(1) == ld) and g.data_ptr() % 16 == 0 and T * ld * 4 < (1 << 31)):
        return g, ld
    return g.contiguous(), D


def _pool_bwd_impl(g, s, h):
    _require_gpu(g, s, h)
    s, h = _f32c(s), _f32c(h)
    B, T, H = s.shape
    D = h.shape[2]
    g, ldg = _pooled_grad_rows(g, B, T, D)
    st = native.stream_ptr()
    ds = torch.empty(B, T, H, dtype=torch.float32, device=h.device)
    native.call("nrm_pool_rowdot", native.ptr(g), ldg, native.ptr(h), native.ptr(ds), B, T, H, D, None, 0, st)
    dh = torch.empty(B, H, D, dtype=torch.float32, device=h.device)
    native.call("nrm_pool_bmm", native.ptr(s), T * H, 1, H, native.ptr(g), ldg, native.ptr(dh), B, H, T, D, 0, st)
    return ds, dh


weighted_pool_bwd = _op("weighted_pool_bwd", "(Tensor g, Tensor scores, Tensor history) -> (Tensor, Tensor)", _pool_bwd_impl,
                        lambda g, s, h: (s.new_empty(tuple(s.shape), dtype=torch.float32), h.new_empty(tuple(h.shape), dtype=torch.float32)))


def _pool_setup(ctx, inputs, output):
    ctx.save_for_backward(*inputs)


def _pool_backward(ctx, g):
    s, h = ctx.saved_tensors
    return weighted_pool_bwd(g, s, h)


torch.library.register_autograd("nrm::weighted_pool_fwd", _pool_backward, setup_context=_pool_setup, lib=_LIB)


def weighted_pool(scores, history):
    D = history.shape[-1]
    if scores.numel() == 0:
        return _degenerate((scores.shape[0], scores.shape[1], D), scores, history)
    _require_gpu(scores, history)
    if D % 4 == 0:
        return weighted_pool_fwd(scores, history)
    return weighted_pool_fwd(scores, torch.nn.functional.pad(history.to(torch.float32), (0, _pad4(D) - D)))[..., :D]


def _attend_pool_fwd_impl(t, h, w1, b1, w2, b2, save_z, mma):
    s, z = _pwattn_fwd_impl(t, h, w1, b1, w2, b2, save_z, mma)
    return _pool_fwd_impl(s, h), s, z


def _attend_pool_fwd_fake(t, h, w1, b1, w2, b2, save_z, mma):
    s, z = _pwattn_fwd_fake(t, h, w1, b1, w2, b2, save_z, mma)
    return t.new_empty(tuple(t.shape), dtype=torch.float32), s, z


attend_pool_fwd = _op("attend_pool_fwd", "(Tensor t, Tensor h, Tensor fc1_weight, Tensor fc1_bias, Tensor fc2_weight, Tensor fc2_bias, "
                      "bool save_z, int mma) -> (Tensor, Tensor, Tensor)", _attend_pool_fwd_impl, _attend_pool_fwd_fake)


def _attend_pool_bwd_impl(g, t, h, w1, w2, s, z, mma, need_dt, need_dh):
    _require_gpu(g, t, h, w1, w2, s, z)
    B, T, D = t.shape
# ... 487 lines not shown
    own = w1 if w1 is w1_arg else None
    w_h, w_t, w_d = w1[:, :D], w1[:, D:2 * D], w1[:, 2 * D:3 * D]
    u, _ = _gemm_nt(h.reshape(B * H, D), w_h, 4 * D, 1, D, D, b1, EPI_BIAS, src2=w_d, sign2=-1.0, owner=own, mma=mma)
    v, _ = _gemm_nt(t, w_t, 4 * D, 1, D, D, None, EPI_BIAS, src2=w_d, sign2=1.0, owner=own, mma=mma)
    st = native.stream_ptr()
    packed = torch.empty(native.load().nrm_pwattn_packed_floats(D), dtype=torch.float32, device=t.device)
    native.call("nrm_pwattn_pack_wp", native.ptr(w1), 4 * D, D, mma, native.ptr(packed), st)
    _count_flops("contraction", 2.0 * N * H * D * D)
    native.call("nrm_pwattn_fwd_ragged", native.ptr(t), native.ptr(h), native.ptr(u), native.ptr(v), native.ptr(packed), native.ptr(w2v),
                native.ptr(b2), native.ptr(s), native.ptr(cand_imp), native.ptr(cand_off), B, N, int(max_count), H, D, mma, st,
                tag="pwattn_fwd_ragged")
    native.call("nrm_pool_bmm_ragged", native.ptr(s), native.ptr(h), native.ptr(pooled), native.ptr(cand_off), B, N, int(max_count), H, D, st)
    return pooled, s


attend_pool_ragged_fwd = _op("attend_pool_ragged_fwd", "(Tensor t, Tensor h, Tensor fc1_weight, Tensor fc1_bias, Tensor fc2_weight, Tensor fc2_bias, "
                             "Tensor cand_imp, Tensor cand_off, int max_count, int mma) -> (Tensor, Tensor)", _attend_pool_ragged_fwd_impl,
                             lambda t, h, w1, b1, w2, b2, ci, co, mc, mma: (t.new_empty(tuple(t.shape), dtype=torch.float32),
                                                                            t.new_empty((t.shape[0], h.shape[1]), dtype=torch.float32)))


def attend_pool_ragged(target, history, fc1_weight, fc1_bias, fc2_weight, fc2_bias, cand_imp, cand_off, max_count, mma=None):
    D = target.shape[-1]
    args = (target, history, fc1_weight, fc1_bias, fc2_weight, fc2_bias)
    _require_gpu(*args)
    if D % 4:
        P = _pad4(D) - D
        pad = torch.nn.functional.pad
        blocks = [pad(fc1_weight[:, i * D:(i + 1) * D], (0, P, 0, P)) for i in range(4)]
        args = (pad(target.to(torch.float32), (0, P)), pad(history.to(torch.float32), (0, P)), torch.cat(blocks, dim=1),
                pad(fc1_bias, (0, P)), pad(fc2_weight.reshape(1, D), (0, P)), fc2_bias)
    with torch.no_grad():
        return attend_pool_ragged_fwd(*args, cand_imp, cand_off, int(max_count), resolve_mma(mma))[0][:, :D]


def _ensemble_rank_ragged_impl(logits, cand_off, pad_mult, label, T):
    import ctypes
    logits = list(logits)
    _require_gpu(*logits, cand_off, pad_mult, label)
    if not logits or any(x.dim() != 1 or x.shape != logits[0].shape for x in logits):
        raise RuntimeError(f"ensemble_rank_ragged: needs 1 .. 8 logit vectors of one [N] shape, got {[tuple(x.shape) for x in logits]}")
    N, B = logits[0].shape[0], pad_mult.shape[0]
    xs = [x if (x.dtype == torch.float32 and (N <= 1 or x.stride(0) >= 1)) else _f32c(x) for x in logits]
    M, dev = len(xs), xs[0].device
    if tuple(cand_off.shape) != (B + 1,):
        raise RuntimeError(f"ensemble_rank_ragged: cand_off has shape {tuple(cand_off.shape)}, expected ({B + 1},)")
    if label is not None and tuple(label.shape) != (B, T):
        raise RuntimeError(f"ensemble_rank_ragged: label has shape {tuple(label.shape)}, expected ({B}, {T})")
    score = torch.empty(B, T, dtype=torch.float32, device=dev)
    rank = torch.empty(B, T, dtype=torch.int32, device=dev)
    live = torch.empty(B, dtype=torch.int32, device=dev)
    metrics = torch.empty(B if label is not None else 0, 3, dtype=torch.float32, device=dev)
    y = _f32c(label) if label is not None else None
    ptrs = (ctypes.c_void_p * M)(*[x.data_ptr() for x in xs])
    cols = (ctypes.c_long * M)(*[x.stride(0) if N > 1 else 1 for x in xs])
    native.call("nrm_ensemble_rank_ragged", ptrs, cols, M, native.ptr(_tab(cand_off)), native.ptr(_tab(pad_mult)), N,
                native.ptr(y) if y is not None else None, B, int(T), native.ptr(score), native.ptr(rank), native.ptr(live),
                native.ptr(metrics) if y is not None else None, native.stream_ptr())
    return score, rank, live, metrics


def _ensemble_rank_ragged_fake(logits, cand_off, pad_mult, label, T):
    x, B = logits[0], pad_mult.shape[0]
    return (x.new_empty((B, T), dtype=torch.float32), x.new_empty((B, T), dtype=torch.int32), x.new_empty((B,), dtype=torch.int32),
            x.new_empty((B if label is not None else 0, 3), dtype=torch.float32))


ensemble_rank_ragged = _op("ensemble_rank_ragged", "(Tensor[] logits, Tensor cand_off, Tensor pad_mult, Tensor? label, int T) -> "
                           "(Tensor score, Tensor rank, Tensor live, Tensor metrics)", _ensemble_rank_ragged_impl, _ensemble_rank_ragged_fake)


def _adam_step_impl(param, grad, exp_avg, exp_avg_sq, state, lr, beta1, beta2, eps, weight_decay, zero_grad):
    _require_gpu(param, grad, exp_avg, exp_avg_sq, state)
    native.call("nrm_adam_step_dev", native.ptr(param), native.ptr(grad), native.ptr(exp_avg), native.ptr(exp_avg_sq),
                param.numel(), float(lr), float(beta1), float(beta2), float(eps), float(weight_decay), native.ptr(state),
                1 if zero_grad else 0, native.stream_ptr())


adam_step = _op("adam_step", "(Tensor(a!) param, Tensor(b!) grad, Tensor(c!) exp_avg, Tensor(d!) exp_avg_sq, Tensor(e!) state, "
                "float lr, float beta1, float beta2, float eps, float weight_decay, bool zero_grad) -> ()",
                _adam_step_impl, lambda *a: None)

OPS = ("pwattn_fwd", "pwattn_bwd", "linear_fwd", "linear_bwd", "small_linear_relu_fwd", "small_linear_relu_bwd", "mlp_gelu_fwd", "mlp_gelu_bwd", "batch_norm_stats", "batch_norm_apply",
       "batch_norm_bwd", "gate_block_fwd", "gate_block_bwd", "concat_cols",
       "weighted_pool_fwd", "weighted_pool_bwd", "attend_pool_fwd", "attend_pool_bwd", "softmax_bce_loss", "frontend_fwd", "frontend_bwd",
       "frontend_pair_fwd", "frontend_pair_bwd", "row_auc", "ensemble_rank", "compact_gather", "attend_pool_ragged_fwd", "ensemble_rank_ragged",
       "adam_step")
```

Before: 33300.

## Fuse head block: concat with BN stats, gate multiply into GEMM operands

```diff
diff --git a/include/nrm_hotpath.h b/include/nrm_hotpath.h
--- a/include/nrm_hotpath.h
+++ b/include/nrm_hotpath.h
@@ -65,9 +65,13 @@
 int nrm_gemm_pack_multi(const nrm_pack_desc* descs, int n, nrm_stream_t stream);
 int nrm_gemm_nt(const float* x, int ldx, int M, const float* packed, int N, int K, const float* bias,
                 float* y, int ldy, float* z, int ldz, const float* m, int ldm, int epilogue, int mma, nrm_stream_t stream);
+int nrm_gemm_nt_mul(const float* x, int ldx, const float* x2, int ldx2, int M, const float* packed, int N, int K, const float* bias,
+                    float* y, int ldy, float* z, int ldz, int epilogue, nrm_stream_t stream);
 int nrm_gemm_tn_nsplit(int ncols_i, int ncols_j, int R, int mma);
 int nrm_gemm_tn(const float* A, int lda, int ncols_i, const float* B, int ldb, int ncols_j, int R,
                 float* ws, int ldws, float* colsum, float* zero_out, long zero_n, int mma, nrm_stream_t stream);
+int nrm_gemm_tn_mul(const float* A, int lda, const float* A2, int lda2, int ncols_i, const float* B, int ldb, const float* B2, int ldb2,
+                    int ncols_j, int R, float* ws, int ldws, float* colsum, float* zero_out, long zero_n, nrm_stream_t stream);
 
 int nrm_slab_reduce(const float* ws, int nsplit, int nj, int ldws, int ni, float* out, long out_istride, long out_jstride,
                     float* out2, long out2_istride, long out2_jstride, float sign2,
@@ -91,6 +95,14 @@
 int nrm_bn_backward(const float* x, const float* dy, const float* mean, const float* rstd, const float* gamma,
                     const float* s0, const float* s1, const float* add, float* dx, int R, int N, int ld, int training,
                     nrm_stream_t stream);
+int nrm_bn_backward_mul(const float* x, const float* dy, const float* mean, const float* rstd, const float* gamma,
+                        const float* s0, const float* s1, const float* mul_a, const float* mul_b, float* dx, int R, int N, int ld,
+                        int training, nrm_stream_t stream);
+int nrm_bn_stats_blocks(long R);
+int nrm_concat_cols_stats(const float* const* srcs, const long* lds, const int* widths, int n, float* out, int ldo, long R,
+                          float* partials, nrm_stream_t stream);
+int nrm_bn_stats_merge(const float* partials, long R, int N, float* mean, float* rstd, float* running_mean,
+                       float* running_var, float momentum, float eps, nrm_stream_t stream);
 int nrm_concat_cols(const float* const* srcs, const long* lds, const int* widths, int n, float* out, int ldo, long R,
                     nrm_stream_t stream);
 
diff --git a/news_recommendation_model_amd/csrc/capi.hip b/news_recommendation_model_amd/csrc/capi.hip
--- a/news_recommendation_model_amd/csrc/capi.hip
+++ b/news_recommendation_model_amd/csrc/capi.hip
@@ -317,6 +317,28 @@
     return check_hip(nrm::gemm_nt_launch(p, pl, epilogue, (hipStream_t)stream), "gemm_nt");
 }
 
+int nrm_gemm_nt_mul(const float* x, int ldx, const float* x2, int ldx2, int M, const float* packed, int N, int K, const float* bias,
+                    float* y, int ldy, float* z, int ldz, int epilogue, nrm_stream_t stream) {
+    if (!x || !x2 || !packed || !y) return fail(NRM_EINVAL, "nrm_gemm_nt_mul: null pointer");
+    if (M < 0 || N <= 0 || K <= 0) return fail(NRM_EINVAL, "nrm_gemm_nt_mul: M=%d N=%d K=%d", M, N, K);
+    if (ldx % 4 || ldx2 % 4 || ldy % 4 || ldx < K || ldx2 < K || ldy < N || !al16(x) || !al16(x2) || !al16(y))
+        return fail(NRM_EINVAL, "nrm_gemm_nt_mul: ldx=%d ldx2=%d ldy=%d must be multiples of 4 covering K=%d / N=%d, rows 16-B aligned", ldx, ldx2, ldy, K, N);
+    if (epilogue != NRM_EPI_BIAS && epilogue != NRM_EPI_GELU && epilogue != NRM_EPI_DGELU) return fail(NRM_EINVAL, "nrm_gemm_nt_mul: epilogue=%d", epilogue);
+    if (epilogue != NRM_EPI_BIAS && (!z || ldz % 4 || ldz < N || !al16(z)))
+        return fail(NRM_EINVAL, "nrm_gemm_nt_mul: epilogue %d needs z with ldz %% 4 == 0, ldz >= N", epilogue);
+    const int ldmax = ldx > ldy ? (ldx > ldx2 ? ldx : ldx2) : (ldy > ldx2 ? ldy : ldx2);
+    if ((long)256 * ldmax * 4 >= (1L << 31)) return fail(NRM_EINVAL, "nrm_gemm_nt_mul: leading dimension too large");
+    const nrm::GemmNtPlan pl = nrm::gemm_nt_plan(N);
+    nrm::GemmNtParams p;
+    p.x = x; p.ldx = ldx; p.xcols = ldx; p.wp = packed; p.wp_bytes = (unsigned)(nrm_gemm_packed_floats(N, K, NRM_MMA_F32) * 4);
+    p.rows = pl.rows; p.bias = bias; p.N = N; p.y = y; p.ldy = ldy;
+    p.z = epilogue == NRM_EPI_BIAS ? nullptr : z; p.ldz = epilogue == NRM_EPI_BIAS ? 4 : ldz;
+    p.m = nullptr; p.ldm = 4;
+    p.M = M; p.K = K; p.kchunks = (K + 15) / 16;
+    p.x2 = x2; p.ldx2 = ldx2; p.x2cols = ldx2;
+    return check_hip(nrm::gemm_nt_launch(p, pl, epilogue, (hipStream_t)stream), "gemm_nt_mul");
+}
+
 static const int kTnWavesBf16 = 1024;
 static int tn_waves(int mma = 0) {
     if (const char* e = getenv("NRM_TN_WAVES")) return atoi(e);
@@ -348,6 +370,27 @@
     return check_hip(nrm::gemm_tn_launch(p, pl, (hipStream_t)stream), "gemm_tn");
 }
 
+int nrm_gemm_tn_mul(const float* A, int lda, const float* A2, int lda2, int ncols_i, const float* B, int ldb, const float* B2, int ldb2,
+                    int ncols_j, int R, float* ws, int ldws, float* colsum, float* zero_out, long zero_n, nrm_stream_t stream) {
+    if (!A || !B || !ws) return fail(NRM_EINVAL, "nrm_gemm_tn_mul: null pointer");
+    if ((A2 == nullptr) == (B2 == nullptr)) return fail(NRM_EINVAL, "nrm_gemm_tn_mul: exactly one of A2 / B2");
+    if (ncols_i <= 0 || ncols_j <= 0 || R <= 0 || lda < ncols_i || ldb < ncols_j || (A2 && lda2 < ncols_i) || (B2 && ldb2 < ncols_j))
+        return fail(NRM_EINVAL, "nrm_gemm_tn_mul: ncols_i=%d ncols_j=%d R=%d lda=%d ldb=%d lda2=%d ldb2=%d", ncols_i, ncols_j, R, lda, ldb, lda2, ldb2);
+    if (ldws % 4 || ldws < ncols_i || !al16(ws)) return fail(NRM_EINVAL, "nrm_gemm_tn_mul: ldws=%d", ldws);
+    const nrm::GemmTnPlan pl = nrm::gemm_tn_plan(ncols_i, ncols_j, R, tn_waves(0), 0);
+    int ldmax = lda > ldb ? lda : ldb;
+    if (A2 && lda2 > ldmax) ldmax = lda2;
+    if (B2 && ldb2 > ldmax) ldmax = ldb2;
+    if ((long)pl.rps * ldmax * 4 >= (1L << 31)) return fail(NRM_EINVAL, "nrm_gemm_tn_mul: split too large");
+    if (zero_out && (zero_n < 0 || !al16(zero_out))) return fail(NRM_EINVAL, "nrm_gemm_tn_mul: zero_out must be 16-byte aligned, zero_n >= 0");
+    nrm::GemmTnParams p = {};
+    p.A = A; p.lda = lda; p.acols = lda; p.B = B; p.ldb = ldb; p.bcols = ldb;
+    p.A2 = A2; p.lda2 = A2 ? lda2 : 0; p.B2 = B2; p.ldb2 = B2 ? ldb2 : 0;
+    p.ws = ws; p.ldws = ldws; p.colsum = colsum; p.R = R; p.ncols_j = ncols_j;
+    p.zero_out = zero_out; p.zero_n = zero_out ? zero_n : 0;
+    return check_hip(nrm::gemm_tn_launch(p, pl, (hipStream_t)stream), "gemm_tn_mul");
+}
+
 int nrm_slab_reduce(const float* ws, int nsplit, int nj, int ldws, int ni, float* out, long out_istride, long out_jstride,
                     float* out2, long out2_istride, long out2_jstride, float sign2,
                     const float* vec, float* vec_out, nrm_stream_t stream) {
@@ -419,7 +462,45 @@
     if (int rc = check_bn("nrm_bn_backward", R, N, ld)) return rc;
     if (!dy || !rstd || !gamma || !dx || (training && (!x || !mean || !s0 || !s1)))
         return fail(NRM_EINVAL, "nrm_bn_backward: null pointer");
-    return check_hip(nrm::bn_bwd_launch(x, dy, mean, rstd, gamma, s0, s1, add, dx, R, N, ld, training, (hipStream_t)stream), "bn_backward");
+    return check_hip(nrm::bn_bwd_launch(x, dy, mean, rstd, gamma, s0, s1, add, nullptr, nullptr, dx, R, N, ld, training, (hipStream_t)stream), "bn_backward");
+}
+
+int nrm_bn_backward_mul(const float* x, const float* dy, const float* mean, const float* rstd, const float* gamma,
+                        const float* s0, const float* s1, const float* mul_a, const float* mul_b, float* dx, int R, int N, int ld,
+                        int training, nrm_stream_t stream) {
+    if (int rc = check_bn("nrm_bn_backward_mul", R, N, ld)) return rc;
+    if (!dy || !rstd || !gamma || !dx || !mul_a || !mul_b || (training && (!x || !mean || !s0 || !s1)))
+        return fail(NRM_EINVAL, "nrm_bn_backward_mul: null pointer");
+    return check_hip(nrm::bn_bwd_launch(x, dy, mean, rstd, gamma, s0, s1, nullptr, mul_a, mul_b, dx, R, N, ld, training, (hipStream_t)stream),
+                     "bn_backward_mul");
+}
+
+int nrm_bn_stats_blocks(long R) { return R > 0 ? nrm::bn_stats_blocks(R) : 0; }
+
+int nrm_concat_cols_stats(const float* const* srcs, const long* lds, const int* widths, int n, float* out, int ldo, long R,
+                          float* partials, nrm_stream_t stream) {
+    if (!srcs || !lds || !widths || !partials) return fail(NRM_EINVAL, "nrm_concat_cols_stats: null pointer");
+    if (n < 1 || n > nrm::CONCAT_MAX || R < 0 || (!out && n != 1)) return fail(NRM_EINVAL, "nrm_concat_cols_stats: n=%d (1..%d; 1 without out) R=%ld", n, nrm::CONCAT_MAX, R);
+    nrm::ConcatTable tab = {};
+    int total = 0;
+    for (int i = 0; i < n; ++i) {
+        if (!srcs[i] || widths[i] <= 0 || widths[i] % 4 || lds[i] < widths[i] || lds[i] % 4 || !al16(srcs[i]))
+            return fail(NRM_EINVAL, "nrm_concat_cols_stats: part %d (width %d, ld %ld: multiples of 4, 16-byte aligned rows)", i, widths[i], lds[i]);
+        tab.src[i] = srcs[i]; tab.ld[i] = lds[i]; tab.start[i] = total;
+        total += widths[i];
+    }
+    tab.n = n;
+    if (out && (ldo < total || ldo % 4 || !al16(out))) return fail(NRM_EINVAL, "nrm_concat_cols_stats: ldo=%d (>= %d columns, a multiple of 4, 16-byte aligned)", ldo, total);
+    if (!al16(partials)) return fail(NRM_EINVAL, "nrm_concat_cols_stats: partials must be 16-byte aligned");
+    return check_hip(nrm::concat_stats_launch(tab, out, R, ldo, total, partials, (hipStream_t)stream), "concat_cols_stats");
+}
+
+int nrm_bn_stats_merge(const float* partials, long R, int N, float* mean, float* rstd, float* running_mean,
+                       float* running_var, float momentum, float eps, nrm_stream_t stream) {
+    if (!partials || !mean || !rstd) return fail(NRM_EINVAL, "nrm_bn_stats_merge: null pointer");
+    if (R <= 0 || R >= (1L << 31) - 64 || N <= 0) return fail(NRM_EINVAL, "nrm_bn_stats_merge: R=%ld N=%d", R, N);
+    return check_hip(nrm::bn_stats_merge_launch(partials, R, N, mean, rstd, running_mean, running_var, momentum, eps, (hipStream_t)stream),
+                     "bn_stats_merge");
 }
 
 
diff --git a/news_recommendation_model_amd/csrc/gemm.hip b/news_recommendation_model_amd/csrc/gemm.hip
--- a/news_recommendation_model_amd/csrc/gemm.hip
+++ b/news_recommendation_model_amd/csrc/gemm.hip
@@ -84,7 +84,7 @@
     return hipGetLastError();
 }
 
-template <int NT, int MT, int EPI, int WPE = 2, int KC = 1>
+template <int NT, int MT, int EPI, int WPE = 2, int KC = 1, bool X2 = false>
 __global__ __launch_bounds__(256, WPE) void gemm_nt_kernel(const GemmNtParams p) {
 #if defined(__HIP_DEVICE_COMPILE__)
     constexpr int BM = 4 * MT * 16;
@@ -121,6 +121,20 @@
         const unsigned slot = (unsigned)((lane & 3) ^ swz4(lane >> 2));
         voff_x[j] = rl < rows_here ? (unsigned)(rl * p.ldx + 4 * slot) * 4u : OOB;
     }
+    const __amdgpu_buffer_rsrc_t rs_x2 = __builtin_amdgcn_make_buffer_rsrc(
+        const_cast<float*>(X2 ? p.x2 + (size_t)m0 * p.ldx2 : nullptr), 0, X2 ? ((rows_here - 1) * p.ldx2 + p.x2cols) * 4 : 0, 0x00020000);
+    unsigned voff_x2[MT];
+    f32x4 xm[MT], xmn[MT];
+#pragma unroll
+    for (int j = 0; j < MT; ++j) {
+        const int rl = (wave * MT + j) * 16 + (lane & 15);
+        voff_x2[j] = X2 && rl < rows_here ? (unsigned)(rl * p.ldx2 + 4 * (lane >> 4)) * 4u : OOB;
+        xm[j] = xmn[j] = f32x4{0.f, 0.f, 0.f, 0.f};
+    }
+    auto load_x2 = [&](int c, f32x4 (&dst)[MT]) {
+#pragma unroll
+        for (int j = 0; j < MT; ++j) dst[j] = __builtin_bit_cast(f32x4, __builtin_amdgcn_raw_buffer_load_b128(rs_x2, voff_x2[j], c * 64, 0));
+    };
     const int rslot = 4 * (q ^ swz4(r16));
 
     f32x4 acc[NT][MT];
@@ -150,6 +164,10 @@
         f32x4 pf[MT];
 #pragma unroll
         for (int jt = 0; jt < MT; ++jt) pf[jt] = *reinterpret_cast<const f32x4*>(&Xl[((wave * MT + jt) * 16 + r16) * 16 + rslot]);
+        if (X2) {
+#pragma unroll
+            for (int jt = 0; jt < MT; ++jt) pf[jt] = pf[jt] * xm[jt];
+        }
         if (kleft < 16) {
             asm volatile("");
             const int kl = kleft - 4 * q;
@@ -177,18 +195,24 @@
     const int nt_valid = min(NT, (p.N - n0 + 15) >> 4);
     const int nstages = (p.kchunks + KC - 1) / KC;
     dma_stage(0, smem);
+    if (X2) load_x2(0, xm);
     __syncthreads();
     if (NRM_PRIO) __builtin_amdgcn_s_setprio(NRM_PRIO);
     for (int c = 0; c < nstages; ++c) {
         float* cur = smem + (c & 1) * BUF;
         float* nxt = smem + ((c & 1) ^ 1) * BUF;
         if (c + 1 < nstages && !(NRM_DIAG_GEMM & 4)) dma_stage(c + 1, nxt);
+        if (X2 && c + 1 < nstages) load_x2(c + 1, xmn);
 #pragma unroll
         for (int k = 0; k < KC; ++k) {
             if (KC > 1 && c * KC + k >= p.kchunks) break;
             const int kleft = p.K - 16 * (c * KC + k);
             if (nt_valid == NT) compute(cur + k * SUB, std::true_type{}, NT, kleft);
             else compute(cur + k * SUB, std::false_type{}, nt_valid, kleft);
+        }
+        if (X2) {
+#pragma unroll
+            for (int j = 0; j < MT; ++j) xm[j] = xmn[j];
         }
         if (!(NRM_DIAG_GEMM & 1)) __syncthreads();
     }
@@ -252,10 +276,21 @@
     return pl;
 }
 
-template <int NT, int MT, int WPE = 2, int KC = 1>
+template <int NT, int MT, int WPE = 2, int KC = 1, bool X2OK = true>
 static hipError_t launch_nt(const GemmNtParams& p, const GemmNtPlan& pl, int epi, hipStream_t st) {
     constexpr int BM = 4 * MT * 16;
     const dim3 grid((p.M + BM - 1) / BM, pl.nchunks), block(256);
+    if constexpr (KC == 1 && X2OK) {
+        if (p.x2) {
+            switch (epi) {
+                case EPI_BIAS:  hipLaunchKernelGGL((gemm_nt_kernel<NT, MT, EPI_BIAS, WPE, 1, true>), grid, block, 0, st, p); break;
+                case EPI_GELU:  hipLaunchKernelGGL((gemm_nt_kernel<NT, MT, EPI_GELU, WPE, 1, true>), grid, block, 0, st, p); break;
+                case EPI_DGELU: hipLaunchKernelGGL((gemm_nt_kernel<NT, MT, EPI_DGELU, WPE, 1, true>), grid, block, 0, st, p); break;
+                default: return hipErrorInvalidValue;
+            }
+            return hipGetLastError();
+        }
+    } else if (p.x2) return hipErrorInvalidValue;
     if (KC > 1) {
         constexpr int lds = 2 * KC * (NT * 16 + BM) * 16 * 4;
         static_assert(lds <= 160 * 1024, "two stages must fit the CU's LDS");
@@ -278,6 +313,7 @@
     int kc = kc_e ? atoi(kc_e) : 1;
     if (kc != 2 && kc != 4) kc = 1;
     if (p.kchunks < 2 * kc) kc = p.kchunks >= 4 ? 2 : 1;
+    if (p.x2) kc = 1;
     if (kc > 1 && (pl.MT == 1 || (small_m && wgs < 512))) {
         if (kc == 4) {
             if (pl.NT == 4) return launch_nt<4, 1, 1, 4>(p, pl, epi, st);
@@ -302,7 +338,7 @@
     if (pl.NT == 4) return launch_nt<4, 4>(p, pl, epi, st);
     if (pl.NT == 5) return launch_nt<5, 4>(p, pl, epi, st);
     if (pl.NT == 8) return launch_nt<8, 3>(p, pl, epi, st);
-    if (pl.NT == 9) return launch_nt<9, 2, 3>(p, pl, epi, st);
+    if (pl.NT == 9) return p.x2 ? launch_nt<9, 1, 4>(p, pl, epi, st) : launch_nt<9, 2, 3, 1, false>(p, pl, epi, st);
     static const int use13x2 = [] { const char* e = getenv("NRM_NT_13X2"); return e && e[0] == '1' ? 1 : 0; }();
     if (use13x2) return launch_nt<13, 2>(p, pl, epi, st);
     return launch_nt<13, 1, 4>(p, pl, epi, st);
@@ -334,7 +370,8 @@
 #endif
 constexpr int tn_waves_per_simd(int KT, int DT) { return KT * DT <= 16 ? 4 : 3; }
 
-template <int KT, int DT>
+constexpr int tn_mul_sets(int KT, int DT, int MUL) { return MUL == 1 && KT >= 5 && KT * DT >= 16 ? 2 : 3; }
+template <int KT, int DT, int MUL = 0>
 __global__ __launch_bounds__(256, tn_waves_per_simd(KT, DT)) void gemm_tn_kernel(const GemmTnParams p) {
 #if defined(__HIP_DEVICE_COMPILE__)
     const int tid = threadIdx.x;
@@ -390,6 +427,46 @@
     for (int it = 0; it < KT; ++it)
 #pragma unroll
         for (int jt = 0; jt < DT; ++jt) C[it][jt] = f32x4{0.f, 0.f, 0.f, 0.f};
+    if constexpr (MUL != 0) {
+        constexpr int MW = MUL == 1 ? KT : DT;
+        const float* m2 = MUL == 1 ? p.A2 : p.B2;
+        const int ldm = MUL == 1 ? p.lda2 : p.ldb2;
+        const int c0 = MUL == 1 ? i0 : j0;
+        const __amdgpu_buffer_rsrc_t rm = __builtin_amdgcn_make_buffer_rsrc(
+            const_cast<float*>(m2) + (size_t)r_lo * ldm, 0, nrows > 0 ? ((nrows - 1) * ldm + ldm) * 4 : 0, 0x00020000);
+        const unsigned vm_lo = (unsigned)(q * ldm + c0 + tn_col<MW>(0, r16)) * 4u;
+        const unsigned vm_hi = MW == 8 ? vm_lo + 256u : (unsigned)(q * ldm + c0 + tn_col<MW>(MW - 1, r16)) * 4u;
+        const unsigned xa_hi = KT == 8 ? va_lo + 256u : va_hi, xb_hi = DT == 8 ? vb_lo + 256u : vb_hi;
+        const int mstep = ldm * 16;
+        constexpr int NS = tn_mul_sets(KT, DT, MUL);
+        float as[NS][KT], bs[NS][DT], ms[NS][MW];
+        auto load3 = [&](float (&a)[KT], float (&b)[DT], float (&m)[MW], int s) {
+            tn_load<KT>(a, ra, va_lo, xa_hi, s * astep);
+            tn_load<DT>(b, rb, vb_lo, xb_hi, s * bstep);
+            tn_load<MW>(m, rm, vm_lo, vm_hi, s * mstep);
+        };
+        auto mfma3 = [&](float (&a)[KT], float (&b)[DT], const float (&m)[MW]) {
+            {
+#pragma clang fp contract(off)
+#pragma unroll
+                for (int t = 0; t < MW; ++t) { if (MUL == 1) a[t] = a[t] * m[t]; else b[t] = b[t] * m[t]; }
+            }
+            mfma_batch(a, b);
+        };
+#pragma unroll
+        for (int u = 0; u < NS - 1; ++u)
+            if (u < nsteps) load3(as[u], bs[u], ms[u], u);
+        for (int s = 0; s < nsteps; s += NS) {
+#pragma unroll
+            for (int u = 0; u < NS; ++u) {
+                if (s + u < nsteps) {
+                    constexpr int ahead = NS - 1;
+                    if (s + u + ahead < nsteps) load3(as[(u + ahead) % NS], bs[(u + ahead) % NS], ms[(u + ahead) % NS], s + u + ahead);
+                    mfma3(as[u], bs[u], ms[u]);
+                }
+            }
+        }
+    } else {
     if (0 < nsteps) load_step(a0, b0, 0);
     if (1 < nsteps) load_step(a1, b1, 1);
     if (2 < nsteps) load_step(a2, b2, 2);
@@ -409,6 +486,7 @@
             if (s + 6 < nsteps) load_step(a2, b2, s + 6);
             mfma_batch(a3, b3);
         }
+    }
     }
 
     float* wsp = p.ws + (size_t)split * p.ncols_j * p.ldws;
@@ -480,6 +558,20 @@
     p.nti = pl.nti; p.nsplit = pl.nsplit; p.rps = pl.rps;
     const dim3 grid(pl.nti * pl.ntj, (pl.nsplit + 3) / 4), block(256);
     const int shape = pl.KT * 16 + pl.DT;
+    if (p.A2 && p.B2) return hipErrorInvalidValue;
+    if (p.A2 || p.B2) {
+#define NRM_TN_MUL(KT_, DT_)                                                                                     \
+    case KT_ * 16 + DT_:                                                                                         \
+        if (p.A2) hipLaunchKernelGGL((gemm_tn_kernel<KT_, DT_, 1>), grid, block, 0, st, p);                     \
+        else      hipLaunchKernelGGL((gemm_tn_kernel<KT_, DT_, 2>), grid, block, 0, st, p);                     \
+        break;
+        switch (shape) {
+            NRM_TN_MUL(4, 4) NRM_TN_MUL(5, 5) NRM_TN_MUL(2, 8) NRM_TN_MUL(8, 2) NRM_TN_MUL(5, 2) NRM_TN_MUL(2, 5)
+            default: return hipErrorInvalidValue;
+        }
+#undef NRM_TN_MUL
+        return hipGetLastError();
+    }
     switch (shape) {
         case 4 * 16 + 4: hipLaunchKernelGGL((gemm_tn_kernel<4, 4>), grid, block, 0, st, p); break;
         case 5 * 16 + 5: hipLaunchKernelGGL((gemm_tn_kernel<5, 5>), grid, block, 0, st, p); break;
diff --git a/news_recommendation_model_amd/csrc/gemm.hpp b/news_recommendation_model_amd/csrc/gemm.hpp
--- a/news_recommendation_model_amd/csrc/gemm.hpp
+++ b/news_recommendation_model_amd/csrc/gemm.hpp
@@ -14,6 +14,7 @@
     float* z; int ldz;
     const float* m; int ldm;
     int M, K, kchunks;
+    const float* x2 = nullptr; int ldx2 = 4, x2cols = 4;
 };
 struct GemmNtPlan { int NT, MT, nchunks, rows; };
 GemmNtPlan gemm_nt_plan(int N);
@@ -47,6 +48,8 @@
     float* zero_out; long zero_n;
     int R, ncols_j;
     int nti, nsplit, rps;
+    const float* A2; int lda2;
+    const float* B2; int ldb2;
 };
 struct GemmTnPlan { int KT, DT, nti, ntj, nsplit, rps; };
 GemmTnPlan gemm_tn_plan(int ncols_i, int ncols_j, int R, int target_waves, int mma = 0);
diff --git a/news_recommendation_model_amd/csrc/head.hip b/news_recommendation_model_amd/csrc/head.hip
--- a/news_recommendation_model_amd/csrc/head.hip
+++ b/news_recommendation_model_amd/csrc/head.hip
@@ -63,6 +63,7 @@
                                                      const float* __restrict__ mean, const float* __restrict__ rstd,
                                                      const float* __restrict__ gamma, const float* __restrict__ s0,
                                                      const float* __restrict__ s1, const float* __restrict__ add,
+                                                     const float* __restrict__ mul_a, const float* __restrict__ mul_b,
                                                      float* __restrict__ dx, long R, int N, int ld, int training) {
     const int n4 = N >> 2;
     const long total = R * n4;
@@ -83,6 +84,7 @@
             out = ga * rs * g;
         }
         if (add) out += *reinterpret_cast<const f32x4*>(add + r * ld + col);
+        if (mul_a) out += *reinterpret_cast<const f32x4*>(mul_a + r * ld + col) * *reinterpret_cast<const f32x4*>(mul_b + r * ld + col);
         *reinterpret_cast<f32x4*>(dx + r * ld + col) = out;
     }
 }
@@ -154,10 +156,10 @@
 }
 
 hipError_t bn_bwd_launch(const float* x, const float* dy, const float* mean, const float* rstd, const float* gamma,
-                         const float* s0, const float* s1, const float* add, float* dx, long R, int N, int ld, int training,
-                         hipStream_t st) {
-    if (R <= 0) return hipSuccess;
-    hipLaunchKernelGGL(bn_bwd_kernel, dim3(ew_blocks(R * (N >> 2))), dim3(256), 0, st, x, dy, mean, rstd, gamma, s0, s1, add, dx, R, N, ld, training);
+                         const float* s0, const float* s1, const float* add, const float* mul_a, const float* mul_b, float* dx,
+                         long R, int N, int ld, int training, hipStream_t st) {
+    if (R <= 0) return hipSuccess;
+    hipLaunchKernelGGL(bn_bwd_kernel, dim3(ew_blocks(R * (N >> 2))), dim3(256), 0, st, x, dy, mean, rstd, gamma, s0, s1, add, mul_a, mul_b, dx, R, N, ld, training);
     return hipGetLastError();
 }
 
@@ -190,6 +192,122 @@
     return hipGetLastError();
 }
 
+constexpr int STAT_ROWS = 64;
+
+template <bool WRITE>
+__global__ __launch_bounds__(256, 4) void concat_stats_kernel(const ConcatTable tab, float* __restrict__ out, int R, int ldo, int N,
+                                                           float* __restrict__ part, size_t plane) {
+    __shared__ f32x4 red[3][8][32];
+    const int tx = threadIdx.x, ty = threadIdx.y;
+    const bool cok = blockIdx.x * 128 + 4 * tx < N;
+    const int col = cok ? blockIdx.x * 128 + 4 * tx : N - 4;
+    const int r0 = blockIdx.y * STAT_ROWS;
+    const int nb = min(STAT_ROWS, R - r0);
+    const float* src = tab.src[0];
+    long lds = tab.ld[0];
+    int start = 0;
+#pragma unroll
+    for (int j = 1; j < CONCAT_MAX; ++j)
+        if (j < tab.n && col >= tab.start[j]) { src = tab.src[j]; lds = tab.ld[j]; start = tab.start[j]; }
+    src += col - start;
+    f32x4 v[8];
+    f32x4 a = f32x4{0.f, 0.f, 0.f, 0.f};
+#pragma unroll
+    for (int i = 0; i < 8; ++i) {
+        const int r = r0 + ty + 8 * i;
+        const f32x4 t = *reinterpret_cast<const f32x4*>(src + (size_t)min(r, R - 1) * lds);
+        if (WRITE && cok && r < R) *reinterpret_cast<f32x4*>(out + (size_t)r * ldo + col) = t;
+#pragma unroll
+        for (int e = 0; e < 4; ++e) v[i][e] = r < R ? t[e] : 0.f;
+        a += v[i];
+    }
+    red[0][ty][tx] = a;
+    __syncthreads();
+    f32x4 mu = red[0][0][tx];
+#pragma unroll
+    for (int y = 1; y < 8; ++y) mu += red[0][y][tx];
+    const float inv = 1.0f / (float)nb;
+    mu = mu * f32x4{inv, inv, inv, inv};
+    f32x4 m2 = f32x4{0.f, 0.f, 0.f, 0.f}, rs = m2;
+#pragma unroll
+    for (int i = 0; i < 8; ++i) {
+        if (r0 + ty + 8 * i < R) { const f32x4 d = v[i] - mu; m2 += d * d; rs += d; }
+    }
+    red[1][ty][tx] = m2;
+    red[2][ty][tx] = rs;
+    __syncthreads();
+    if (ty == 0 && cok) {
+        f32x4 t = red[1][0][tx], u = red[2][0][tx];
+#pragma unroll
+        for (int y = 1; y < 8; ++y) { t += red[1][y][tx]; u += red[2][y][tx]; }
+        float* dst = part + (size_t)blockIdx.y * N + col;
+        *reinterpret_cast<f32x4*>(dst) = mu;
+        *reinterpret_cast<f32x4*>(dst + plane) = t;
+        *reinterpret_cast<f32x4*>(dst + 2 * plane) = u;
+    }
+}
+
+__global__ __launch_bounds__(256) void bn_stats_merge_kernel(const float* __restrict__ pmean, size_t plane, int nblk,
+                                                             int R, int N, float* __restrict__ mean, float* __restrict__ rstd,
+                                                             float* __restrict__ running_mean, float* __restrict__ running_var,
+                                                             float momentum, float eps) {
+    __shared__ float red[8][33];
+    const int tx = threadIdx.x, ty = threadIdx.y;
+    const int col = blockIdx.x * 32 + tx;
+    const bool cok = col < N;
+    float a = 0.f;
+    if (cok)
+        for (int b = ty; b < nblk; b += 8)
+            a += (float)min(STAT_ROWS, R - b * STAT_ROWS) * pmean[(size_t)b * N + col] + pmean[(size_t)b * N + col + 2 * plane];
+    red[ty][tx] = a;
+    __syncthreads();
+    float mu = red[0][tx];
+#pragma unroll
+    for (int y = 1; y < 8; ++y) mu += red[y][tx];
+    mu = mu / (float)R;
+    __syncthreads();
+    a = 0.f;
+    if (cok)
+        for (int b = ty; b < nblk; b += 8) {
+            const size_t o = (size_t)b * N + col;
+            const float d = pmean[o] - mu;
+            a += pmean[o + plane] + (float)min(STAT_ROWS, R - b * STAT_ROWS) * d * d + 2.0f * d * pmean[o + 2 * plane];
+        }
+    red[ty][tx] = a;
+    __syncthreads();
+    if (ty == 0 && cok) {
+        float m2 = red[0][tx];
+#pragma unroll
+        for (int y = 1; y < 8; ++y) m2 += red[y][tx];
+        m2 = m2 < 0.f ? 0.f : m2;
+        const float var = m2 / (float)R;
+        mean[col] = mu;
+        rstd[col] = 1.0f / sqrtf(var + eps);
+        if (running_mean) running_mean[col] = (1.0f - momentum) * running_mean[col] + momentum * mu;
+        if (running_var) running_var[col] = (1.0f - momentum) * running_var[col] + momentum * var * ((float)R / (float)(R > 1 ? R - 1 : 1));
+    }
+}
+
+int bn_stats_blocks(long R) { return (int)((R + STAT_ROWS - 1) / STAT_ROWS); }
+
+hipError_t concat_stats_launch(const ConcatTable& tab, float* out, long R, int ldo, int total, float* part, hipStream_t st) {
+    if (R <= 0 || total <= 0) return hipSuccess;
+    if (R >= (1L << 31) - STAT_ROWS || bn_stats_blocks(R) > 65535) return hipErrorInvalidValue;
+    const dim3 grid((total + 127) / 128, bn_stats_blocks(R)), block(32, 8);
+    const size_t plane = (size_t)bn_stats_blocks(R) * total;
+    if (out) hipLaunchKernelGGL(concat_stats_kernel<true>, grid, block, 0, st, tab, out, (int)R, ldo, total, part, plane);
+    else     hipLaunchKernelGGL(concat_stats_kernel<false>, grid, block, 0, st, tab, out, (int)R, ldo, total, part, plane);
+    return hipGetLastError();
+}
+
+hipError_t bn_stats_merge_launch(const float* part, long R, int N, float* mean, float* rstd, float* running_mean,
+                                 float* running_var, float momentum, float eps, hipStream_t st) {
+    if (N <= 0 || R <= 0) return hipSuccess;
+    hipLaunchKernelGGL(bn_stats_merge_kernel, dim3((N + 31) / 32), dim3(32, 8), 0, st, part, (size_t)bn_stats_blocks(R) * N, bn_stats_blocks(R), (int)R, N, mean, rstd,
+                       running_mean, running_var, momentum, eps);
+    return hipGetLastError();
+}
+
 constexpr int SL_KMAX = 4, SL_NMAX = 8;
 
 template <typename XT>
diff --git a/news_recommendation_model_amd/csrc/head.hpp b/news_recommendation_model_amd/csrc/head.hpp
--- a/news_recommendation_model_amd/csrc/head.hpp
+++ b/news_recommendation_model_amd/csrc/head.hpp
@@ -7,11 +7,15 @@
 hipError_t bn_apply_launch(const float* x, const float* mean, const float* rstd, const float* gamma, const float* beta,
                            float* y, long R, int N, int ld, hipStream_t st);
 hipError_t bn_bwd_launch(const float* x, const float* dy, const float* mean, const float* rstd, const float* gamma,
-                         const float* s0, const float* s1, const float* add, float* dx, long R, int N, int ld, int training,
-                         hipStream_t st);
+                         const float* s0, const float* s1, const float* add, const float* mul_a, const float* mul_b, float* dx,
+                         long R, int N, int ld, int training, hipStream_t st);
 constexpr int CONCAT_MAX = 8;
 struct ConcatTable { const float* src[CONCAT_MAX]; long ld[CONCAT_MAX]; int start[CONCAT_MAX]; int n; };
 hipError_t concat_cols_launch(const ConcatTable& tab, float* out, long R, int ldo, int total, hipStream_t st);
+int bn_stats_blocks(long R);
+hipError_t concat_stats_launch(const ConcatTable& tab, float* out, long R, int ldo, int total, float* part, hipStream_t st);
+hipError_t bn_stats_merge_launch(const float* part, long R, int N, float* mean, float* rstd, float* running_mean,
+                                 float* running_var, float momentum, float eps, hipStream_t st);
 hipError_t bn_finalize_launch(int stage, const float* s, float* out, float* running, int R, int N, float momentum, float eps,
                               hipStream_t st);
 hipError_t mul_bwd_launch(const float* dy, const float* g, const float* e, float* dg, float* de, long R, int N,
diff --git a/news_recommendation_model_amd/modules.py b/news_recommendation_model_amd/modules.py
--- a/news_recommendation_model_amd/modules.py
+++ b/news_recommendation_model_amd/modules.py
@@ -202,11 +202,15 @@
         if type(inv) is UserInvariantInterestModel and not (inv._forward_hooks or inv._forward_pre_hooks):
             pooled_lab, pooled_ti, lab_t, ti_t = inv.forward_parts(x_history, x_target)
             eu_L = self.instant_interest_model(x_global)
-            e = ops.concat_last((pooled_lab, pooled_ti, eu_L, lab_t, ti_t))
+            parts = (pooled_lab, pooled_ti, eu_L, lab_t, ti_t)
         else:
             eu_H, ec = inv(x_history, x_target)
             eu_L = self.instant_interest_model(x_global)
-            e = ops.concat_last((eu_H, eu_L, ec))
+            parts = (eu_H, eu_L, ec)
+        if self._head_is_one_block() and parts[0].dim() == 3 and parts[0].shape[0] * parts[0].shape[1] > 0:
+            B, T = parts[0].shape[:2]
+            return self.out_mlp(self._head_block([p.reshape(B * T, p.shape[-1]) for p in parts])).reshape(B, T)
+        e = ops.concat_last(parts)
         B, T, N = e.shape
         rows = e.reshape(B * T, N)
         g = self.gate
@@ -215,6 +219,17 @@
         else:
             gated = g.forward_times(ops.batch_norm(rows, self.bn), rows)
         return self.out_mlp(self.mlp(gated)).reshape(B, T)
+
+    def _head_is_one_block(self):
+        def plain(m):
+            return (type(m) is MLP and isinstance(m.activation, nn.GELU) and m.activation.approximate == "none"
+                    and not (m._forward_hooks or m._forward_pre_hooks))
+        return plain(self.gate) and plain(self.mlp) and type(self.bn) is nn.BatchNorm1d and not (self.bn._forward_hooks or self.bn._forward_pre_hooks)
+
+    def _head_block(self, parts):
+        g, m = self.gate, self.mlp
+        return ops.head_block(parts, self.bn, g.fc1.weight, g.fc1.bias, g.fc2.weight, g.fc2.bias,
+                              m.fc1.weight, m.fc1.bias, m.fc2.weight, m.fc2.bias)
 
     def forward_compact(self, x_history, xt_compact, xg_compact, plan):
         if self.training:
@@ -247,6 +262,8 @@
                 pooled.append(ops.attend_pool_ragged(t, h, m.fc1.weight, m.fc1.bias, m.fc2.weight, m.fc2.bias, tabs["cand_imp"],
                                                      tabs["cand_off"], plan.max_count, mma=att.mma))
             eu_L = self.instant_interest_model(xg_compact)
+            if self._head_is_one_block():
+                return self.out_mlp(self._head_block([pooled[0], pooled[1], eu_L, lab_t[0], ti_t[0]])).reshape(N)
             rows = ops.concat_last((pooled[0], pooled[1], eu_L, lab_t[0], ti_t[0]))
             g = self.gate
             if isinstance(g.activation, nn.GELU) and g.activation.approximate == "none":
diff --git a/news_recommendation_model_amd/native.py b/news_recommendation_model_amd/native.py
--- a/news_recommendation_model_amd/native.py
+++ b/news_recommendation_model_amd/native.py
@@ -35,6 +35,12 @@
     "nrm_gemm_nt_bf16_supported": (_c_i, [_c_i, _c_i, _c_i]),
     "nrm_gemm_pack": (_c_i, [_c_fp, _c_l, _c_l, _c_i, _c_i, _c_fp, _c_fp]),
     "nrm_gemm_nt": (_c_i, [_c_fp, _c_i, _c_i, _c_fp, _c_i, _c_i, _c_fp, _c_fp, _c_i, _c_fp, _c_i, _c_fp, _c_i, _c_i, _c_i, _c_fp]),
+    "nrm_gemm_nt_mul": (_c_i, [_c_fp, _c_i, _c_fp, _c_i, _c_i, _c_fp, _c_i, _c_i, _c_fp, _c_fp, _c_i, _c_fp, _c_i, _c_i, _c_fp]),
+    "nrm_gemm_tn_mul": (_c_i, [_c_fp, _c_i, _c_fp, _c_i, _c_i, _c_fp, _c_i, _c_fp, _c_i, _c_i, _c_i, _c_fp, _c_i, _c_fp, _c_fp, _c_l, _c_fp]),
+    "nrm_bn_backward_mul": (_c_i, [_c_fp] * 10 + [_c_i] * 4 + [_c_fp]),
+    "nrm_bn_stats_blocks": (_c_i, [_c_l]),
+    "nrm_concat_cols_stats": (_c_i, [_c_fp, _c_fp, _c_fp, _c_i, _c_fp, _c_i, _c_l, _c_fp, _c_fp]),
+    "nrm_bn_stats_merge": (_c_i, [_c_fp, _c_l, _c_i, _c_fp, _c_fp, _c_fp, _c_fp, ctypes.c_float, ctypes.c_float, _c_fp]),
     "nrm_slab_reduce": (_c_i, [_c_fp, _c_i, _c_i, _c_i, _c_i, _c_fp, _c_l, _c_l, _c_fp, _c_l, _c_l, ctypes.c_float,
                                _c_fp, _c_fp, _c_fp]),
     "nrm_bn_finalize": (_c_i, [_c_i, _c_fp, _c_fp, _c_fp, _c_i, _c_i, ctypes.c_float, ctypes.c_float, _c_fp]),
diff --git a/news_recommendation_model_amd/ops.py b/news_recommendation_model_amd/ops.py
--- a/news_recommendation_model_amd/ops.py
+++ b/news_recommendation_model_amd/ops.py
@@ -198,16 +198,21 @@
 
 
 def _gemm_nt(x, w_src, row_stride, col_stride, n_out, k_red, bias, epilogue, z=None, m=None, src2=None, sign2=0.0, owner=None,
-             mma=None):
+             mma=None, x2=None):
     st = native.stream_ptr()
     M = x.shape[0]
-    mma = _dense_mma(M, k_red, mma)
+    mma = MMA_F32 if x2 is not None else _dense_mma(M, k_red, mma)
     packed = _pack(w_src, row_stride, col_stride, n_out, k_red, src2, sign2, owner, mma)
     ldy = _pad4(n_out)
     y = torch.empty(M, ldy, dtype=torch.float32, device=x.device)
     if epilogue in (EPI_GELU, EPI_MUL):
         z = torch.empty(M, ldy, dtype=torch.float32, device=x.device)
     _count_flops("dense", 2.0 * M * n_out * k_red)
+    if x2 is not None:
+        native.call("nrm_gemm_nt_mul", native.ptr(x), x.stride(0), native.ptr(x2), x2.stride(0), M, native.ptr(packed), n_out, k_red,
+                    native.ptr(bias) if bias is not None else None, native.ptr(y), ldy,
+                    native.ptr(z) if z is not None else None, z.stride(0) if z is not None else 0, epilogue, st)
+        return y[:, :n_out], (z[:, :n_out] if epilogue == EPI_GELU else None)
     native.call("nrm_gemm_nt", native.ptr(x), x.stride(0), M, native.ptr(packed), n_out, k_red,
                 native.ptr(bias) if bias is not None else None, native.ptr(y), ldy,
                 native.ptr(z) if z is not None else None, z.stride(0) if z is not None else 0,
@@ -215,11 +220,13 @@
     return y[:, :n_out], (z[:, :n_out] if epilogue in (EPI_GELU, EPI_MUL) else None)
 
 
-def _gemm_tn_slabs(a, b, want_colsum, zero_out=None, mma=None):
+def _gemm_tn_slabs(a, b, want_colsum, zero_out=None, mma=None, a2=None, b2=None):
     lib = native.load()
     R, ni = a.shape
     nj = b.shape[1]
     mma = _default_dense_mma if mma is None else mma
+    if a2 is not None or b2 is not None:
+        mma = MMA_F32
     if _FORCE_F32_GEMM or (mma != MMA_F32 and (a.stride(0) % 4 or b.stride(0) % 4 or a.data_ptr() % 16 or b.data_ptr() % 16)):
         mma = MMA_F32
     nsplit = lib.nrm_gemm_tn_nsplit(ni, nj, R, mma)
@@ -227,6 +234,13 @@
     ws = torch.empty(nsplit, nj, ldws, dtype=torch.float32, device=a.device)
     cs = torch.empty(nsplit, ldws, dtype=torch.float32, device=a.device) if want_colsum else None
     _count_flops("dense", 2.0 * R * ni * nj)
+    if a2 is not None or b2 is not None:
+        native.call("nrm_gemm_tn_mul", native.ptr(a), a.stride(0), native.ptr(a2) if a2 is not None else None,
+                    a2.stride(0) if a2 is not None else 0, ni, native.ptr(b), b.stride(0), native.ptr(b2) if b2 is not None else None,
+                    b2.stride(0) if b2 is not None else 0, nj, R, native.ptr(ws), ldws, native.ptr(cs) if cs is not None else None,
+                    native.ptr(zero_out) if zero_out is not None else None, zero_out.numel() if zero_out is not None else 0,
+                    native.stream_ptr())
+        return ws, cs, nsplit, ldws
     native.call("nrm_gemm_tn", native.ptr(a), a.stride(0), ni, native.ptr(b), b.stride(0), nj, R,
                 native.ptr(ws), ldws, native.ptr(cs) if cs is not None else None,
                 native.ptr(zero_out) if zero_out is not None else None, zero_out.numel() if zero_out is not None else 0,
@@ -341,12 +355,12 @@
     _wgrad["used"].clear()
 
 
-def _gemm_tn(a, b, want_colsum, target=None, mma=None):
+def _gemm_tn(a, b, want_colsum, target=None, mma=None, a2=None, b2=None):
     ni, nj = a.shape[1], b.shape[1]
-    ctx = _wgrad_stream(a, b)
+    ctx = _wgrad_stream(a, b, *[t for t in (a2, b2) if t is not None])
     with ctx as side:
         c = torch.empty(ni, nj, dtype=torch.float32, device=a.device)
-        ws, cs, nsplit, ldws = _gemm_tn_slabs(a, b, want_colsum, zero_out=c, mma=mma)
+        ws, cs, nsplit, ldws = _gemm_tn_slabs(a, b, want_colsum, zero_out=c, mma=mma, a2=a2, b2=b2)
         colsum = torch.empty(ni, dtype=torch.float32, device=a.device) if want_colsum else None
         _slab_reduce(ws, nsplit, nj, ldws, ni, c, nj, 1, vec=cs, vec_out=colsum, target=target)
         if side:
@@ -910,7 +924,7 @@
                        _bn_apply_impl, lambda x, mean, rstd, weight, bias, batch_stats: _padded_empty(x, x.shape[0], x.shape[1]))
 
 
-def _bn_bwd_impl(dy, x, mean, rstd, weight, training, add=None):
+def _bn_bwd_impl(dy, x, mean, rstd, weight, training, add=None, mul=None):
     _require_gpu(dy, x)
     x = _rows(x)
     R, N = x.shape
@@ -933,6 +947,18 @@
         buf = torch.zeros(R, ld, dtype=torch.float32, device=dev)
         buf[:, :N] = add
         add = buf[:, :N]
+    if mul is not None:
+        ok = all(t.dim() == 2 and t.stride(1) == 1 and t.stride(0) == ld and t.dtype == torch.float32 and t.data_ptr() % 16 == 0
+                 for t in mul)
+        if not ok:
+            buf = torch.zeros(R, ld, dtype=torch.float32, device=dev)
+            buf[:, :N] = mul[0] * mul[1]
+            add, mul = buf[:, :N], None
+    if mul is not None:
+        native.call("nrm_bn_backward_mul", native.ptr(x), native.ptr(dy), native.ptr(mean), native.ptr(rstd), native.ptr(w),
+                    native.ptr(s0), native.ptr(s1), native.ptr(mul[0]), native.ptr(mul[1]), native.ptr(dx), R, N, ld,
+                    1 if training else 0, st)
+        return dx[:, :N], s1, s0
     native.call("nrm_bn_backward", native.ptr(x), native.ptr(dy), native.ptr(mean), native.ptr(rstd), native.ptr(w),
                 native.ptr(s0), native.ptr(s1), native.ptr(add) if add is not None else None, native.ptr(dx), R, N, ld,
                 1 if training else 0, st)
@@ -1090,6 +1116,207 @@
     _require_gpu(*parts)
     y = concat_cols_op([p.reshape(rows, p.shape[-1]) for p in parts])
     return y.reshape(*lead, y.shape[-1]) if y.is_contiguous() else y.unflatten(0, tuple(lead))
+
+
+def head_chain_forced():
+    return _os.environ.get("NRM_HEAD_CHAIN") == "1"
+
+
+def _mlp_shapes_ok(x_cols, w1, w2, n_out=None):
+    return (w1.dim() == 2 and w2.dim() == 2 and w1.shape[1] == x_cols and w2.shape[1] == w1.shape[0]
+            and (n_out is None or w2.shape[0] == n_out))
+
+
+def _head_block_fwd_impl(x, mean, rstd, bn_w, bn_b, gw1, gb1, gw2, gb2, mw1, mb1, mw2, mb2, batch_stats):
+    _require_gpu(x, mean, rstd, bn_w, gw1, gw2, mw1, mw2)
+    x = _rows(x)
+    M, N = x.shape
+    own = lambda w: (lambda c: (c, c if c is w else None))(_f32c(w))
+    (gw1, go1), (gw2, go2), (mw1, mo1), (mw2, mo2) = own(gw1), own(gw2), own(mw1), own(mw2)
+    bias = lambda b: _f32c(b) if b is not None else None
+    if not (_mlp_shapes_ok(N, gw1, gw2, N) and _mlp_shapes_ok(N, mw1, mw2)):
+        raise RuntimeError(f"head block: gate {tuple(gw1.shape)} / {tuple(gw2.shape)} and mlp {tuple(mw1.shape)} / {tuple(mw2.shape)} "
+                           f"do not fit rows of {N} features")
+    c = _bn_apply_impl(x, mean, rstd, bn_w, bn_b, batch_stats)
+    g_hidden, g_z = _gemm_nt(c, gw1, N, 1, gw1.shape[0], N, bias(gb1), EPI_GELU, owner=go1)
+    pre, _ = _gemm_nt(g_hidden, gw2, gw2.shape[1], 1, N, gw2.shape[1], bias(gb2), EPI_BIAS, owner=go2)
+    m_hidden, m_z = _gemm_nt(pre, mw1, N, 1, mw1.shape[0], N, bias(mb1), EPI_GELU, owner=mo1, x2=x)
+    out, _ = _gemm_nt(m_hidden, mw2, mw2.shape[1], 1, mw2.shape[0], mw2.shape[1], bias(mb2), EPI_BIAS, owner=mo2)
+    return out, c, g_hidden, g_z, pre, m_hidden, m_z
+
+
+def _head_block_fwd_fake(x, mean, rstd, bn_w, bn_b, gw1, gb1, gw2, gb2, mw1, mb1, mw2, mb2, batch_stats):
+    M, N = x.shape
+    pe = lambda n: _padded_empty(x, M, n)
+    return pe(mw2.shape[0]), pe(N), pe(gw1.shape[0]), pe(gw1.shape[0]), pe(N), pe(mw1.shape[0]), pe(mw1.shape[0])
+
+
+head_block_fwd = _op("head_block_fwd", "(Tensor x, Tensor mean, Tensor rstd, Tensor bn_weight, Tensor bn_bias, Tensor gate_fc1_weight, "
+                     "Tensor? gate_fc1_bias, Tensor gate_fc2_weight, Tensor? gate_fc2_bias, Tensor mlp_fc1_weight, Tensor? mlp_fc1_bias, "
+                     "Tensor mlp_fc2_weight, Tensor? mlp_fc2_bias, bool batch_stats) -> "
+                     "(Tensor, Tensor, Tensor, Tensor, Tensor, Tensor, Tensor)", _head_block_fwd_impl, _head_block_fwd_fake)
+
+
+def _head_block_bwd_impl(dout, x, mean, rstd, bn_w, c, gw1, gw2, g_hidden, g_z, pre, mw1, mw2, m_hidden, m_z,
+                         has_gb1, has_gb2, has_mb1, has_mb2, batch_stats):
+    _require_gpu(dout, x)
+    x = _rows(x)
+    M, N = x.shape
+    pg1, pg2, pm1, pm2 = gw1, gw2, mw1, mw2
+    own = lambda w: (lambda cc: (cc, cc if cc is w else None))(_f32c(w))
+    (gw1, go1), (gw2, go2), (mw1, mo1), (mw2, mo2) = own(gw1), own(gw2), own(mw1), own(mw2)
+    dout = _rows(dout)
+    dmw2, dmb2 = _gemm_tn(dout, m_hidden, has_mb2, target=pm2)
+    dmz, _ = _gemm_nt(dout, mw2, 1, mw2.shape[1], mw2.shape[1], mw2.shape[0], None, EPI_DGELU, z=m_z, owner=mo2)
+    dmw1, dmb1 = _gemm_tn(dmz, pre, has_mb1, target=pm1, b2=x)
+    dy = _gemm_nt(dmz, mw1, 1, N, N, mw1.shape[0], None, EPI_BIAS, owner=mo1)[0]
+    dgw2, dgb2 = _gemm_tn(dy, g_hidden, has_gb2, target=pg2, a2=x)
+    dgz, _ = _gemm_nt(dy, gw2, 1, gw2.shape[1], gw2.shape[1], N, None, EPI_DGELU, z=g_z, owner=go2, x2=x)
+    dgw1, dgb1 = _gemm_tn(dgz, c, has_gb1, target=pg1)
+    dc = _gemm_nt(dgz, gw1, 1, N, N, gw1.shape[0], None, EPI_BIAS, owner=go1)[0]
+    dx, dgamma, dbeta = _bn_bwd_impl(dc, x, mean, rstd, bn_w, batch_stats, mul=(dy, pre))
+    e = lambda: torch.empty((0,), dtype=torch.float32, device=x.device)
+    return (dx, dgamma, dbeta, dgw1, (dgb1 if has_gb1 else e()), dgw2, (dgb2 if has_gb2 else e()),
+            dmw1, (dmb1 if has_mb1 else e()), dmw2, (dmb2 if has_mb2 else e()))
+
+
+def _head_block_bwd_fake(dout, x, mean, rstd, bn_w, c, gw1, gw2, g_hidden, g_z, pre, mw1, mw2, m_hidden, m_z,
+                         has_gb1, has_gb2, has_mb1, has_mb2, batch_stats):
+    M, N = x.shape
+    f = lambda *shape: x.new_empty(shape, dtype=torch.float32)
+    v = lambda has, n: f(n) if has else f(0)
+    return (_padded_empty(x, M, N), f(N), f(N), f(*gw1.shape), v(has_gb1, gw1.shape[0]), f(*gw2.shape), v(has_gb2, gw2.shape[0]),
+            f(*mw1.shape), v(has_mb1, mw1.shape[0]), f(*mw2.shape), v(has_mb2, mw2.shape[0]))
+
+
+head_block_bwd = _op("head_block_bwd", "(Tensor dout, Tensor x, Tensor mean, Tensor rstd, Tensor bn_weight, Tensor c, Tensor gate_fc1_weight, "
+                     "Tensor gate_fc2_weight, Tensor gate_hidden, Tensor gate_z, Tensor pre, Tensor mlp_fc1_weight, Tensor mlp_fc2_weight, "
+                     "Tensor mlp_hidden, Tensor mlp_z, bool has_gb1, bool has_gb2, bool has_mb1, bool has_mb2, bool batch_stats) -> "
+                     "(Tensor, Tensor, Tensor, Tensor, Tensor, Tensor, Tensor, Tensor, Tensor, Tensor, Tensor)",
+                     _head_block_bwd_impl, _head_block_bwd_fake)
+
+
+def _head_block_setup(ctx, inputs, output):
+    x, mean, rstd, bn_w, bn_b, gw1, gb1, gw2, gb2, mw1, mb1, mw2, mb2, batch_stats = inputs
+    out, c, g_hidden, g_z, pre, m_hidden, m_z = output
+    ctx.set_materialize_grads(False)
+    ctx.flags = (gb1 is not None, gb2 is not None, mb1 is not None, mb2 is not None, batch_stats)
+    ctx.save_for_backward(x, mean, rstd, bn_w, c, gw1, gw2, g_hidden, g_z, pre, mw1, mw2, m_hidden, m_z)
+
+
+def _head_block_backward(ctx, dout, *_unused):
+    if dout is None:
+        return (None,) * 14
+    b = ctx.flags
+    dx, dgamma, dbeta, dgw1, dgb1, dgw2, dgb2, dmw1, dmb1, dmw2, dmb2 = head_block_bwd(dout, *ctx.saved_tensors, *b)
+    return (dx, None, None, dgamma, dbeta, dgw1, (dgb1 if b[0] else None), dgw2, (dgb2 if b[1] else None),
+            dmw1, (dmb1 if b[2] else None), dmw2, (dmb2 if b[3] else None), None)
+
+
+torch.library.register_autograd("nrm::head_block_fwd", _head_block_backward, setup_context=_head_block_setup, lib=_LIB)
+
+
+def _vec4_rows(t):
+    return (t.dtype == torch.float32 and t.dim() == 2 and t.stride(1) == 1 and t.shape[1] % 4 == 0 and t.data_ptr() % 16 == 0
+            and (t.shape[0] <= 1 or t.stride(0) % 4 == 0))
+
+
+def _partial_stats(parts, write):
+    import ctypes
+    _require_gpu(*parts)
+    R = parts[0].shape[0]
+    total = sum(p.shape[1] for p in parts)
+    if not write:
+        parts = [_rows(parts[0])]
+    if not (1 <= len(parts) <= 8 and all(p.shape[0] == R for p in parts) and all(_vec4_rows(p) for p in parts) and R >= 1):
+        raise RuntimeError("concat_cols_stats: up to 8 fp32 row blocks whose widths, leading dimensions and addresses are multiples of 4 floats")
+    lib = native.load()
+    nblk = lib.nrm_bn_stats_blocks(R)
+    dev = parts[0].device
+    part = torch.empty(3, nblk, total, dtype=torch.float32, device=dev)
+    k = len(parts)
+    out = torch.empty(R, total, dtype=torch.float32, device=dev) if write else None
+    srcs = (ctypes.c_void_p * k)(*[p.data_ptr() for p in parts])
+    lds = (ctypes.c_long * k)(*[p.stride(0) if p.shape[0] > 1 else _pad4(p.shape[1]) for p in parts])
+    widths = (ctypes.c_int * k)(*[p.shape[1] for p in parts])
+    native.call("nrm_concat_cols_stats", srcs, lds, widths, k, native.ptr(out) if out is not None else None,
+                out.stride(0) if out is not None else 0, R, native.ptr(part), native.stream_ptr())
+    return out, part
+
+
+def _concat_cols_stats_impl(parts):
+    return _partial_stats(list(parts), True)
+
+
+def _concat_cols_stats_fake(parts):
+    R, total = parts[0].shape[0], sum(p.shape[1] for p in parts)
+    nblk = (R + 63) // 64
+    return parts[0].new_empty((R, total), dtype=torch.float32), parts[0].new_empty((3, nblk, total), dtype=torch.float32)
+
+
+concat_cols_stats_op = _op("concat_cols_stats", "(Tensor[] parts) -> (Tensor, Tensor)", _concat_cols_stats_impl, _concat_cols_stats_fake)
+
+
+def _concat_stats_backward(ctx, g, _gp):
+    return _concat_backward(ctx, g)
+
+
+torch.library.register_autograd("nrm::concat_cols_stats", _concat_stats_backward,
+                                setup_context=lambda ctx, inputs, output: _concat_setup(ctx, inputs, output), lib=_LIB)
+
+
+def _bn_stats_merge_impl(part, rows, running_mean, running_var, momentum, eps):
+    _require_gpu(part, running_mean, running_var)
+    if not (part.dim() == 3 and part.is_contiguous() and part.dtype == torch.float32 and part.shape[0] == 3
+            and part.shape[1] == native.load().nrm_bn_stats_blocks(int(rows))):
+        raise RuntimeError("batch_norm_stats_merge: partials must be the contiguous [3, blocks, N] tensor of concat_cols_stats")
+    N = part.shape[2]
+    mean = torch.empty(N, dtype=torch.float32, device=part.device)
+    rstd = torch.empty(N, dtype=torch.float32, device=part.device)
+    native.call("nrm_bn_stats_merge", native.ptr(part), int(rows), N, native.ptr(mean), native.ptr(rstd),
+                native.ptr(running_mean), native.ptr(running_var), float(momentum), float(eps), native.stream_ptr())
+    return mean, rstd
+
+
+batch_norm_stats_merge = _op("batch_norm_stats_merge", "(Tensor partials, int rows, Tensor(a!) running_mean, Tensor(b!) running_var, "
+                             "float momentum, float eps) -> (Tensor, Tensor)", _bn_stats_merge_impl,
+                             lambda part, rows, rm, rv, momentum, eps: (part.new_empty((part.shape[2],)), part.new_empty((part.shape[2],))))
+
+
+batch_norm_partial_stats = _op("batch_norm_partial_stats", "(Tensor x) -> Tensor", lambda x: _partial_stats([x], False)[1],
+                               lambda x: x.new_empty((3, (x.shape[0] + 63) // 64, x.shape[1]), dtype=torch.float32))
+
+
+def batch_norm_stats_oneread(x, running_mean, running_var, momentum, eps):
+    return batch_norm_stats_merge(batch_norm_partial_stats(x.detach()), x.shape[0], running_mean, running_var, float(momentum), float(eps))
+
+
+def head_block(parts, bn, gate_fc1_weight, gate_fc1_bias, gate_fc2_weight, gate_fc2_bias,
+               mlp_fc1_weight, mlp_fc1_bias, mlp_fc2_weight, mlp_fc2_bias):
+    parts = list(parts)
+    R, N = parts[0].shape[0], sum(p.shape[1] for p in parts)
+    fused = (not head_chain_forced() and (_default_dense_mma == MMA_F32 or _FORCE_F32_GEMM) and N % 4 == 0 and bn.affine
+             and bn.track_running_stats and bn.momentum is not None and R > (1 if bn.training else 0) and len(parts) <= 8
+             and all(p.dim() == 2 and p.shape[0] == R for p in parts)
+             and _mlp_shapes_ok(N, gate_fc1_weight, gate_fc2_weight, N) and _mlp_shapes_ok(N, mlp_fc1_weight, mlp_fc2_weight))
+    if not fused:
+        rows = parts[0] if len(parts) == 1 else concat_cols_op(parts) if (R and len(parts) <= 8) else torch.cat(parts, dim=1)
+        gated = gate_block(rows, bn, gate_fc1_weight, gate_fc1_bias, gate_fc2_weight, gate_fc2_bias)
+        return mlp_gelu(gated, mlp_fc1_weight, mlp_fc1_bias, mlp_fc2_weight, mlp_fc2_bias)
+    _require_gpu(*parts, bn.weight, gate_fc1_weight, mlp_fc1_weight)
+    if bn.training:
+        bn.num_batches_tracked.add_(1)
+        if len(parts) > 1 and all(_vec4_rows(p) for p in parts):
+            rows, part = concat_cols_stats_op(parts)
+            mean, rstd = batch_norm_stats_merge(part, R, bn.running_mean, bn.running_var, float(bn.momentum), float(bn.eps))
+        else:
+            rows = parts[0] if len(parts) == 1 else concat_cols_op(parts)
+            mean, rstd = batch_norm_stats_oneread(rows.detach(), bn.running_mean, bn.running_var, float(bn.momentum), float(bn.eps))
+    else:
+        rows = parts[0] if len(parts) == 1 else concat_cols_op(parts)
+        mean, rstd = bn.running_mean.to(torch.float32), torch.rsqrt(bn.running_var.to(torch.float32) + bn.eps)
+    return head_block_fwd(rows, mean, rstd, bn.weight, bn.bias, gate_fc1_weight, gate_fc1_bias, gate_fc2_weight, gate_fc2_bias,
+                          mlp_fc1_weight, mlp_fc1_bias, mlp_fc2_weight, mlp_fc2_bias, bn.training)[0]
 
 
 def _pool_fwd_impl(s, h):
@@ -1743,7 +1970,8 @@
                 _adam_step_impl, lambda *a: None)
 
 OPS = ("pwattn_fwd", "pwattn_bwd", "linear_fwd", "linear_bwd", "small_linear_relu_fwd", "small_linear_relu_bwd", "mlp_gelu_fwd", "mlp_gelu_bwd", "batch_norm_stats", "batch_norm_apply",
-       "batch_norm_bwd", "gate_block_fwd", "gate_block_bwd", "concat_cols",
+       "batch_norm_bwd", "gate_block_fwd", "gate_block_bwd", "concat_cols", "head_block_fwd", "head_block_bwd", "concat_cols_stats",
+       "batch_norm_stats_merge", "batch_norm_partial_stats",
        "weighted_pool_fwd", "weighted_pool_bwd", "attend_pool_fwd", "attend_pool_bwd", "softmax_bce_loss", "frontend_fwd", "frontend_bwd",
        "frontend_pair_fwd", "frontend_pair_bwd", "row_auc", "ensemble_rank", "compact_gather", "attend_pool_ragged_fwd", "ensemble_rank_ragged",
        "adam_step")
```

Result: no change. 33180 (-0.3%).
